# shockless/asr-transformer

Measured on AMD Instinct MI355X. Metric: encoder+decoder frames/sec/GPU at d_model=512 T=1000; 1->8 GPU scaling, higher is better.
Workload: dtype bf16; 1 GPU; c3: 12+12 layers d_model=512 h=8 ff=2048, B=64/GPU, T=1000 (T'=249), L=64, V=250; bf16 train step fwd+CE+bwd+AdamW, dropout 0.1; model=speech-transformer, global_batch=64, seq_len=1000, parallelism=dp1

## Files before the change

### asr-transformer_amd/asrx/blocks.py

```python
import bisect
import math

import torch

from . import kernels as K
from .kernels import MaskSpec


class FreshGrads:

    def __init__(self, store, params):
        self.grad = store.grad
        self.base = store.grad.data_ptr()
        ent = sorted((store.offset(p), p.numel()) for p in params)
        self.offs = [o for o, _ in ent]
        self.live = dict(ent)

    def take(self, gw):
        if not self.live:
            return False
        a = (gw.data_ptr() - self.base) // 4
        rows, cols = (gw.shape[0], gw.shape[1]) if gw.dim() == 2 else (1, gw.numel())
        ld = gw.stride(0) if gw.dim() == 2 else cols
        b = a + (rows - 1) * ld + cols
        i = bisect.bisect_left(self.offs, a)
        if i > 0 and self.offs[i - 1] + self.live.get(self.offs[i - 1], 0) > a:
            i -= 1
        hit = []
        while i < len(self.offs) and self.offs[i] < b:
            o = self.offs[i]
            if o in self.live:
                hit.append(o)
            i += 1
        if not hit:
            return False
        full = (ld == cols and (gw.dim() < 2 or gw.stride(1) == 1) and hit[0] == a
                and sum(self.live[o] for o in hit) == b - a)
        for o in hit:
            n = self.live.pop(o)
            if not full:
                self.grad[o:o + n].zero_()
        return full

    def drain(self, params=None, store=None):
        offs = list(self.live) if params is None else [store.offset(p) for p in params if store.offset(p) in self.live]
        for o in offs:
            self.grad[o:o + self.live.pop(o)].zero_()


class Ctx:

    def __init__(self, store, cd, train, p_drop, seeds, attn_impl="fused"):
        self.store = store
        self.cd = cd
        self.train = train
        self.p = p_drop if train else 0.0
        self.seeds = seeds
        self.attn_impl = attn_impl
        self.wq = None
        self.lnq = None
        self.fresh = None
        self.adam = None
        self.adam_cover = []
        self._gwritten = set()

    def W(self, p):
        return self.store.w16(p) if self.cd == torch.bfloat16 else self.store.w32(p)

    def G(self, p):
        return self.store.g(p)

    def seed(self):
        return self.seeds.next() if self.p > 0 else 0

    def wgrad(self, dy, x, gw, gb=None):
        if self.wq is not None and K.wgrad_groupable(dy, x, gw):
            self.wq.append((dy, x, gw, gb))
        else:
            first = self.fresh is not None and self.fresh.take(gw)
            self._note_writes(gw, gb)
            K.linear_wgrad(dy, x, gw, bias_grad=gb, beta=0.0 if first else 1.0)

    def _note_writes(self, *ts):
        cov = {o for o, _ in self.adam_cover}
        base = self.store.grad.data_ptr()
        for t in ts:
            if t is not None:
                assert (t.data_ptr() - base) // 4 not in cov, "asrx: write to a gradient after its fused AdamW"
                self._gwritten.add(t.data_ptr())

    def _adam_safe(self, q0):
        seen = set()
        for _, _, gw, gb in q0:
            for t in (gw, gb):
                if t is None:
                    continue
                if t.data_ptr() in seen or t.data_ptr() in self._gwritten:
                    return False
                seen.add(t.data_ptr())
        return True

    def _issue_wgrads(self, q):
        if self.fresh is None:
            for _, _, gw, gb in q:
                self._note_writes(gw, gb)
            K.linear_wgrad_grouped(q)
            return
        q0, q1 = [], []
        for it in q:
            (q0 if self.fresh.take(it[2]) else q1).append(it)
        adam = self.adam if not q1 and self._adam_safe(q0) else None
        for _, _, gw, gb in q0 + q1:
            self._note_writes(gw, gb)
        kname = K.linear_wgrad_grouped(q0, beta=0.0, adam=adam)
        if adam is not None and kname in K.GROUPED_FUSED_KERNELS:
            base = self.store.grad.data_ptr()
            for _, _, gw, gb in q0:
                for t in (gw, gb):
                    if t is not None:
                        self.adam_cover.append(((t.data_ptr() - base) // 4, t.numel()))
        K.linear_wgrad_grouped(q1)

    def defer_wgrad(self):
        if self.cd == torch.bfloat16 and self.wq is None:
            self.wq, self.lnq = [], []
            return True
        return False

    def flush_wgrad(self):
        q, self.wq = self.wq, None
        lq, self.lnq = self.lnq, None
        self._issue_wgrads(q or [])
        K.reduce_rows_grouped(lq or [])


class Seeds:
    def __init__(self, base):
        self.base = base
        self.i = 0

    def next(self):
        self.i += 1
        x = (self.base * 0x9E3779B97F4A7C15 + self.i * 0xBF58476D1CE4E5B9) & ((1 << 64) - 1)
        return x ^ (x >> 31)




def _empty(shape, dtype, like):
    return torch.empty(shape, dtype=dtype, device=like.device)


def as_dtype(t, dtype):
    if t.dtype == dtype:
        return t.contiguous()
    out = _empty(t.shape, dtype, t)
    K.cast(t.contiguous(), out)
    return out


def drop_bwd_c(C, g, seed):
    dy_c = _empty(g.shape, C.cd, g)
    if C.p > 0:
        K.ewise(K.EW_DROPOUT, g, dy_c, p=C.p, seed=seed)
    else:
        K.cast(g, dy_c)
    return dy_c



def ln_fwd(C, x, ln, out_dtype=None):
    y = _empty(x.shape, out_dtype or C.cd, x)
    mean, rstd = K.layernorm_fwd(x, ln.weight.data, ln.bias.data, y)
    return y, mean, rstd


def ln_grad_buf(C, ln):
    gw, gb = C.G(ln.weight), C.G(ln.bias)
    if gb.data_ptr() == gw.data_ptr() + 4 * gw.numel():
        return C.store.grad[C.store.offset(ln.weight):C.store.offset(ln.weight) + 2 * gw.numel()], None
    tmp = torch.zeros(2 * gw.numel(), device=gw.device, dtype=torch.float32)
    return tmp, (gw, gb)


def ln_bwd(C, x, dy, ln, mean, rstd, dres=None, drop_out=None, drop_seed=0, drop_p=0.0):
    buf, split = ln_grad_buf(C, ln)
# ... 261 lines not shown
    d = dy.shape[1]
    dmid_c = _empty(dy.shape, C.cd, dy)
    dmid = ffn_bwd(C, Sf, dy, dy_c, dx_c_out=dmid_c, dx_c_p=C.p, dx_c_seed=Sa["sd"])
    return self_attn_bwd(C, Sa, dmid, dmid_c, dx_c_out=dx_c_out, dx_c_p=dx_c_p, dx_c_seed=dx_c_seed)


def dec_layer_fwd(C, x, layer, B, L, H, spec, kv, kv_ld, Te, group=1, xspec=None):
    x1, Sa = self_attn_fwd(C, x, layer._norm1, layer._mask_attention, B, L, H, spec)
    x2, Sc = cross_attn_fwd(C, x1, layer._norm2, layer._cross_attention, kv, kv_ld, B, L, Te, H, group, xspec)
    x3, Sf = ffn_fwd(C, x2, layer._norm3, layer._feedforward)
    return x3, (Sa, Sc, Sf)


def dec_layer_bwd(C, S, dy, dy_c, dkv, dx_c_out, dx_c_p=0.0, dx_c_seed=0):
    Sa, Sc, Sf = S
    d2_c = _empty(dy.shape, C.cd, dy)
    d2 = ffn_bwd(C, Sf, dy, dy_c, dx_c_out=d2_c, dx_c_p=C.p, dx_c_seed=Sc["sd"])
    d1_c = _empty(dy.shape, C.cd, dy)
    d1 = cross_attn_bwd(C, Sc, d2, d2_c, dkv, dx_c_out=d1_c, dx_c_p=C.p, dx_c_seed=Sa["sd"])
    return self_attn_bwd(C, Sa, d1, d1_c, dx_c_out=dx_c_out, dx_c_p=dx_c_p, dx_c_seed=dx_c_seed)



def frontend_fwd(C, spectrum, conv1, conv2):
    B, _, F, T = spectrum.shape
    F1, T1 = (F - 3) // 2 + 1, (T - 3) // 2 + 1
    F2, T2 = (F1 - 3) // 2 + 1, (T1 - 3) // 2 + 1
    x = spectrum.contiguous().float()
    y1 = _empty((B, F1, T1, 64), C.cd, x)
    y1m = torch.empty((B, F1, T1, 8), dtype=torch.uint8, device=x.device) if C.cd == torch.bfloat16 else None
    K.conv1_fwd(x, conv1.weight.data.reshape(64, 9).contiguous(), conv1.bias.data, y1, mask=y1m)
    feats = _empty((B * T2, F2 * 64), C.cd, x)
    if C.cd == torch.bfloat16:
        K.conv2_fwd(y1, C.W(conv2.weight), conv2.bias.data, feats)
        cols = None
    else:
        cols = _empty((B * T2 * F2, 576), C.cd, x)
        K.im2col_conv2(y1, cols)
        K.gemm(cols, C.W(conv2.weight), feats, B * T2 * F2, 64, 576, lda=576, ldb=576, ldc=64,
               bias=conv2.bias.data, relu=True)
    return feats, dict(x=x, y1=y1, y1m=y1m, cols=cols, feats=feats, dims=(B, F, T, F1, T1, F2, T2))


def frontend_bwd(C, S, dfeats_c, conv1, conv2):
    B, F, T, F1, T1, F2, T2 = S["dims"]
    M2 = B * T2 * F2
    dy2 = dfeats_c.view(M2, 64)
    cols = S["cols"]
    G = C.G
    if cols is None:
        gw = G(conv2.weight)
        if C.fresh is not None:
            C.fresh.take(gw)
        K.conv2_wgrad(dy2, S["y1"], gw, G(conv2.bias))
    else:
        C.wgrad(dy2, cols, G(conv2.weight), G(conv2.bias))
    if cols is None and K.conv_bwd_implicit_fits(T):
        K.conv_bwd_implicit(dy2, C.W(conv2.weight), S["y1m"], S["x"], G(conv1.weight).view(64, 9), G(conv1.bias))
        return
    dcols = _empty((M2, 576), C.cd, dy2)
    K.linear_dgrad(dy2, C.W(conv2.weight), dcols)
    K.conv1_bwd_fused(dcols, S["y1"], S["x"], G(conv1.weight).view(64, 9), G(conv1.bias))
```

### asr-transformer_amd/asrx/kernels.py

```python
import ctypes
import os
import math
from typing import NamedTuple, Optional

import torch

from ._lib import (BF16, BITS, CONSTS, CTC_MAX_TARGET, CTC_MEAN, CTC_SUM, ED_CROSS, ED_GROUP, ED_PAIRS, F32,
                   MAX_ROWSUM_GROUPS, AttnDesc, GemmDesc, GemmGroupDev, RowsumGroup, call)

_U64 = (1 << 64) - 1


_raw_stream = torch._C._cuda_getCurrentRawStream
_cur_dev = torch._C._cuda_getDevice


def stream():
    return _raw_stream(_cur_dev())


def code(t):
    if t.dtype == torch.bfloat16:
        return BF16
    if t.dtype == torch.float32:
# ... 367 lines not shown
        seen, nb = set(), 0
        for dy, x, gw, gb in items:
            for t in (dy, x):
                if t.data_ptr() not in seen:
                    seen.add(t.data_ptr())
                    nb += t.shape[0] * t.shape[1] * t.element_size()
            for t in (gw, gb):
                if t is not None:
                    nb += t.numel() * 4 * (2 if beta == 1.0 else 1) + (26 * t.numel() if fused else 0)
        probe.alg_bytes[kname] = nb
    if probe is not None and probe.active and probe.log is not None:
        probe.log.append((kname, len(items), 0,
                          sum(it[0].shape[0] * it[0].shape[1] * it[1].shape[1] for it in items), 1, 1))
    if probe is not None and probe.active:
        timed_launch(kname, flops, launch)
    else:
        launch()
    return kname


def colsum(x, out, *, accumulate=True, rows=None, cols=None, ld=None):
    _cuda(x, out)
    rows = x.shape[0] if rows is None else rows
    cols = x.shape[1] if cols is None else cols
    ld = x.stride(0) if ld is None else ld
    nblocks = max(1, min(512, (rows + 63) // 64))
    part = torch.empty(nblocks * cols, device=x.device, dtype=torch.float32)
    call("asrx_reduce_rows", code(x), x.data_ptr(), rows, cols, ld, out.data_ptr(), int(accumulate),
         part.data_ptr(), nblocks, stream())



def layernorm_fwd(x, gamma, beta, y, eps=1e-5):
    _cuda(x, gamma, beta, y)
    rows, d = x.shape
    mean = torch.empty(rows, device=x.device, dtype=torch.float32)
    rstd = torch.empty(rows, device=x.device, dtype=torch.float32)
    call("asrx_layernorm_fwd", code(x), x.data_ptr(), code(y), y.data_ptr(), gamma.data_ptr(), beta.data_ptr(),
         mean.data_ptr(), rstd.data_ptr(), rows, d, eps, stream())
    return mean, rstd


def reduce_rows_grouped(items):
    for c0 in range(0, len(items), MAX_ROWSUM_GROUPS):
        chunk = items[c0:c0 + MAX_ROWSUM_GROUPS]
        arr = (RowsumGroup * len(chunk))()
        for gr, (src, out, acc) in zip(arr, chunk):
            _cuda(src, out)
            gr.in_, gr.rows, gr.cols = src.data_ptr(), src.shape[0], src.shape[1]
            gr.out, gr.accumulate = out.data_ptr(), int(acc)
        call("asrx_reduce_rows_grouped", arr, len(chunk), stream())


LN_BWD_BLOCKS = 512
LN_BWD512_WAVES = 8


def layernorm_bwd(x, dy, gamma, mean, rstd, dgb, *, dres=None, dx_drop=None, dropout_p=0.0, seed=0, defer=None):
    _cuda(x, dy, gamma, mean, rstd, dgb)
    rows, d = x.shape
    dx = torch.empty(rows, d, device=x.device, dtype=torch.float32)
    wpb = LN_BWD512_WAVES if d == 512 else 4
    nblocks = max(1, min(LN_BWD_BLOCKS * 4 // wpb, (rows + 2 * wpb - 1) // (2 * wpb)))
    part = torch.empty(nblocks * 2 * d, device=x.device, dtype=torch.float32)
    call("asrx_layernorm_bwd", code(x), x.data_ptr(), code(dy), dy.data_ptr(), gamma.data_ptr(), mean.data_ptr(),
         rstd.data_ptr(), _p(dres), dx.data_ptr(), _p(dx_drop), code(dx_drop) if dx_drop is not None else 0,
         dropout_p, seed & _U64, part.data_ptr(), nblocks, rows, d, stream())
    if defer is not None:
        defer.append((part.view(nblocks, 2 * d), dgb, True))
        return dx
    part2 = torch.empty(max(1, (nblocks + 63) // 64) * 2 * d, device=x.device, dtype=torch.float32)
    call("asrx_reduce_rows", F32, part.data_ptr(), nblocks, 2 * d, 2 * d, dgb.data_ptr(), 1, part2.data_ptr(),
         max(1, (nblocks + 63) // 64), stream())
    return dx



class MaskSpec:

    def __init__(self, mode=0, causal=False, kvalid=None, qvalid=None, valid_bstride=0, dense=None,
                 strides=(0, 0, 0)):
        self.mode, self.causal = mode, causal
        self.kvalid, self.qvalid, self.valid_bstride = kvalid, qvalid, valid_bstride
        self.dense, self.strides = dense, strides

    @staticmethod
    def decoder(mask):
        valid = (mask >= 1).to(torch.uint8).contiguous()
        return MaskSpec(1, True, valid, valid, valid.stride(0))

    @staticmethod
    def keys(valid):
        assert valid.dtype == torch.uint8 and valid.dim() == 2 and valid.stride(1) == 1
        return MaskSpec(1, False, valid, None, valid.stride(0))

    @staticmethod
    def from_attention_mask(m, B, Lq, Lk):
        if m is None:
            return MaskSpec()
        mb = m.gt(0).to(torch.uint8)
        while mb.dim() < 3:
            mb = mb.unsqueeze(0)
        mb = mb.expand(B, Lq, Lk)
        return MaskSpec(2, dense=mb, strides=tuple(mb.stride()))


# ... 447 lines not shown

def conv1_fwd(x, w, b, y1, mask=None):
    _cuda(x, w, b, y1, mask)
    B, _, F, T = x.shape
    call("asrx_conv1_fwd", x.data_ptr(), B, F, T, w.data_ptr(), b.data_ptr(), y1.data_ptr(), code(y1), _p(mask),
         stream())


def im2col_conv2(y1, cols):
    _cuda(y1, cols)
    B, F1, T1, _ = y1.shape
    assert y1.dtype == cols.dtype
    call("asrx_im2col_conv2", code(y1), y1.data_ptr(), B, F1, T1, cols.data_ptr(), stream())


def col2im_conv2(dcols, y1, dy1):
    _cuda(dcols, y1, dy1)
    B, F1, T1, _ = y1.shape
    call("asrx_col2im_conv2", code(dcols), dcols.data_ptr(), code(y1), y1.data_ptr(), B, F1, T1, dy1.data_ptr(),
         stream())


def conv2_fwd(y1, w2, bias, out):
    _cuda(y1, w2, bias, out)
    B, F1, T1, _ = y1.shape
    call("asrx_conv2_fwd", y1.data_ptr(), w2.data_ptr(), bias.data_ptr(), out.data_ptr(), B, F1, T1, stream())


def conv2_wgrad(dy2, y1, dw, db, splitk=256):
    _cuda(dy2, y1, dw, db)
    B, F1, T1, _ = y1.shape
    ws = torch.empty(splitk * 64 * 576, device=dy2.device, dtype=torch.float32)
    rws = torch.empty(splitk * 64, device=dy2.device, dtype=torch.float32) if db is not None else None
    call("asrx_conv2_wgrad", dy2.data_ptr(), y1.data_ptr(), B, F1, T1, dw.data_ptr(), _p(db), ws.data_ptr(),
         ws.numel(), _p(rws), splitk, stream())


CONV_BWD_MAXT1 = 1024
CONV_BWD_MAXLDS = 80 * 1024


def conv_bwd_implicit_fits(T):
    T1 = (T - 3) // 2 + 1
    return T1 <= CONV_BWD_MAXT1 and 6 * 64 * 64 * 2 + ((T1 * 8 + 15) & ~15) + 12 * T <= CONV_BWD_MAXLDS


def conv_bwd_implicit(dy2, w2, y1_mask, x, dw, db):
    _cuda(dy2, w2, y1_mask, x, dw, db)
    B, _, F, T = x.shape
    nblocks = max(2, min(512, B * y1_mask.shape[1]))
    part = torch.empty((nblocks + 128) * 640, device=x.device, dtype=torch.float32)
    call("asrx_conv_bwd_implicit", dy2.data_ptr(), w2.data_ptr(), y1_mask.data_ptr(), x.data_ptr(), B, F, T,
         part.data_ptr(), nblocks, dw.data_ptr(), db.data_ptr(), stream())


def conv1_bwd_w(x, dy1, dw, db):
    _cuda(x, dy1, dw, db)
    B, _, F, T = x.shape
    nblocks = 512
    part = torch.empty((nblocks + 128) * 640, device=x.device, dtype=torch.float32)
    call("asrx_conv1_bwd_w", x.data_ptr(), dy1.data_ptr(), B, F, T, part.data_ptr(), nblocks, dw.data_ptr(),
         db.data_ptr(), stream())


def conv1_bwd_fused(dcols, y1, x, dw, db):
    _cuda(dcols, y1, x, dw, db)
    B, _, F, T = x.shape
    nblocks = (B * y1.shape[1] * 8 + 3) // 4
    part = torch.empty((nblocks + 128) * 640, device=x.device, dtype=torch.float32)
    call("asrx_conv1_bwd_fused", code(dcols), dcols.data_ptr(), code(y1), y1.data_ptr(), x.data_ptr(), B, F, T,
         part.data_ptr(), nblocks, dw.data_ptr(), db.data_ptr(), stream())


def embed_fwd(tok, table, pe, out, L, dropout_p=0.0, seed=0):
    _cuda(tok, table, pe, out)
    call("asrx_embed_fwd", tok.data_ptr(), tok.numel(), L, table.data_ptr(), table.shape[1], pe.data_ptr(),
         dropout_p, seed & _U64, out.data_ptr(), stream())


def embed_bwd(tok, dout, dtable, L, pad_id, dropout_p=0.0, seed=0):
    _cuda(tok, dout, dtable)
    call("asrx_embed_bwd", tok.data_ptr(), tok.numel(), L, dout.data_ptr(), dtable.shape[1], dtable.shape[0],
         pad_id, dropout_p, seed & _U64, dtable.data_ptr(), stream())


CE_OLD_MAXLD = 1024


def xent_workspace_elems(rows):
    from ._lib import lib
    n = lib().asrx_xent_workspace_elems(rows)
    if n < 0:
        raise RuntimeError(f"asrx: no cross-entropy workspace for {rows} rows")
    return n


def cross_entropy(logits, V, target, ignore_index=-100, grad_scale=1.0, want_grad=True, want_argmax=False,
                  label_smoothing=0.0, grad_dtype=torch.bfloat16, want_stats=False, strided=False):
    _cuda(logits, target)
    rows, ld = logits.shape
    if strided:
        assert logits.dtype == torch.float32 and logits.stride(1) == 1 and V <= ld, \
            "asrx: cross_entropy(strided=True) needs fp32 rows of unit column stride"
        if rows > 1:
            ld = logits.stride(0)
            assert ld >= logits.shape[1], "asrx: cross_entropy(strided=True): overlapping rows"
# ... 239 lines not shown
    cross = mode == "cross"
    call("asrx_edit_distance", hyp.data_ptr(), hyp.stride(0), hyp.shape[1], _p(hyp_lengths),
         None if cross else ref.data_ptr(), 0 if cross else ref.stride(0), 0 if cross else ref.shape[1],
         None if cross else _p(ref_lengths), N, code, W, None if mode == "pairs" else _p(n_hyp), *_drop_ids(drop),
         -1 if stop is None else int(stop), dist.data_ptr(), _p(cnt), stream())
    return dist, cnt


def mbr_rank(dist, score, B, W, scale=1.0, n_hyp=None):
    _cuda(dist, score, n_hyp)
    assert dist.dtype == torch.int32 and dist.numel() == B * W * W and dist.is_contiguous()
    assert score.dtype == torch.float32 and score.numel() == B * W and score.is_contiguous()
    _check_n_hyp(n_hyp, B)
    risk = torch.empty(B, W, dtype=torch.float32, device=dist.device)
    order = torch.empty(B, W, dtype=torch.int32, device=dist.device)
    call("asrx_mbr_rank", dist.data_ptr(), score.data_ptr(), _p(n_hyp), B, W, float(scale), risk.data_ptr(),
         order.data_ptr(), stream())
    return risk, order


def adam(p, g, m, v, p_bf16, lr, beta1, beta2, eps, weight_decay, step, grad_scale=1.0, decoupled=False, hyp=None):
    _cuda(p, g, m, v, p_bf16, hyp)
    bc1 = 1.0 - beta1 ** step
    bc2 = 1.0 - beta2 ** step
    call("asrx_adam", p.data_ptr(), g.data_ptr(), m.data_ptr(), v.data_ptr(), _p(p_bf16), p.numel(), lr, beta1,
         beta2, eps, weight_decay, bc1, bc2, grad_scale, int(decoupled), _p(hyp), stream())


def adam_desc(p, m, v, p_bf16, g, lr, beta1, beta2, eps, weight_decay, step, grad_scale=1.0, decoupled=False,
              hyp=None):
    from ._lib import AdamDesc
    _cuda(p, m, v, p_bf16, g, hyp)
    d = AdamDesc()
    d.p, d.m, d.v, d.p_bf16, d.g_base, d.hyp = p.data_ptr(), m.data_ptr(), v.data_ptr(), _p(p_bf16), g.data_ptr(), _p(hyp)
    d.lr, d.beta1, d.beta2, d.eps, d.weight_decay = lr, beta1, beta2, eps, weight_decay
    d.bias_corr1, d.bias_corr2 = 1.0 - beta1 ** step, 1.0 - beta2 ** step
    d.grad_scale, d.decoupled = grad_scale, int(decoupled)
    return d


def adam_spans(p, g, m, v, p_bf16, spans, lr, beta1, beta2, eps, weight_decay, step, grad_scale=1.0, decoupled=False,
               hyp=None):
    _cuda(p, g, m, v, p_bf16, spans, hyp)
    call("asrx_adam_spans", p.data_ptr(), g.data_ptr(), m.data_ptr(), v.data_ptr(), _p(p_bf16), spans.data_ptr(),
         spans.shape[0], lr, beta1, beta2, eps, weight_decay, 1.0 - beta1 ** step, 1.0 - beta2 ** step, grad_scale,
         int(decoupled), _p(hyp), stream())


def adam_hyper(hyp, lr, beta1, beta2, step):
    import numpy as np
    upload(hyp, np.array([lr, 1.0 - beta1 ** step, 1.0 - beta2 ** step], dtype=np.float32))


TUNE_KEYS = {k: CONSTS["ASRX_TUNE_" + k.upper()] for k in ("softmax_u", "ln_rw", "ln_pf", "ln_bpc")}


def set_tuning(name, value):
    call("asrx_set_tuning", TUNE_KEYS[name], int(value))


def set_seed_offset(offset):
    call("asrx_set_seed_offset", int(offset) & _U64, stream())
```

### asr-transformer_amd/asrx/train.py

```python
import os

import torch

from . import kernels as K
from .augment import rank_seed
from .blocks import FreshGrads
from .dist import GradAllReduce
from .functions import get_store, key_spec, make_ctx, model_backward, model_forward, pad_lengths

FRESH_GRADS = os.environ.get("ASRX_FRESH_GRADS", "1") == "1"
GRAPH = os.environ.get("ASRX_GRAPH", "1") == "1"
GRAPH_WARMUP = 2
EARLY_ADAM = os.environ.get("ASRX_DP_EARLY_ADAM", "0") == "1"
FUSED_ADAM = os.environ.get("ASRX_FUSED_ADAM", "1") == "1"
ADAM_SPAN = 8192
ZERO_SPAN = 16384


def _aligned_spans(spans, n, q=4):
    out = []
    for a, b in sorted(spans):
        a, b = -(-a // q) * q, min(n, b) // q * q
        if b <= a:
            continue
# ... 199 lines not shown
                                                                   logits[i].shape[1]), device=logits[i].device)),
                                          dim=0)
            logits = torch.stack(logits, dim=0)
            preds.append(pred.to("cpu"))
            targets.append(text.to("cpu"))
            loss = loss_function(logits.transpose(1, 2), text)
            total += loss.item()
    return {"Val Loss": total / max(1, len(data_loader))}, preds[-1][-1]


class Trainer:

    def __init__(self, model, lr=1e-4, betas=(0.9, 0.98), eps=1e-9, weight_decay=0.0, decoupled=True,
                 ignore_index=-100, group=None, bucket_mb=64, allreduce_fn=None, graph=None, wire=None, preds=False,
                 ctc_weight=0.0, bos_token_id=1, spec_augment=None, label_smoothing=0.0):
        self.model = model
        self.label_smoothing = float(label_smoothing)
        if not 0.0 <= self.label_smoothing < 1.0:
            raise ValueError(f"label_smoothing {label_smoothing} outside [0, 1)")
        self.last_stats = None
        self.spec_augment = spec_augment
        self._aug_buf = None
        self.ctc_weight = float(ctc_weight)
        if not 0.0 <= self.ctc_weight < 1.0:
            raise ValueError(f"ctc_weight {ctc_weight} outside [0, 1)")
        head = getattr(model, "ctc_head", None)
        if self.ctc_weight > 0 and head is None:
            raise ValueError("ctc_weight > 0 needs a model with a CTC head: Transformer(..., ctc=True)")
        self._ctc_drop = [int(bos_token_id), int(model.decoder._eos_token_id)]
        if model.decoder.pad_token_id is not None:
            self._ctc_drop.append(int(model.decoder.pad_token_id))
        idle_head = list(head.parameters()) if head is not None and self.ctc_weight == 0 else []
        self.store = get_store(model)
        self.m = torch.zeros_like(self.store.flat)
        self.v = torch.zeros_like(self.store.flat)
        self.lr, self.betas, self.eps, self.wd, self.decoupled = lr, betas, eps, weight_decay, decoupled
        self.ignore_index = ignore_index
        self.step_count = 0
        self.reducer = GradAllReduce(self.store.grad, group=group, bucket_mb=bucket_mb, allreduce_fn=allreduce_fn,
                                     wire=wire)
        self.store.refresh_shadow(force=True)
        self._wonly = [p for p in wgrad_only_params(model) if not any(p is q for q in idle_head)] if FRESH_GRADS else []
        self.graph = GRAPH if graph is None else bool(graph)
        self._cap = None
        self._caps = {}
        self._eager_keys = set()
        self._hyp = torch.zeros(3, dtype=torch.float32, device=self.store.flat.device)
        self.ar_events = None
        self._adam_side = None
        self.want_preds = bool(preds)
        self.last_preds = None
        self._cover = None
        self._rspans = {}
        self._fuse_next = False
        self._frozen = sorted((self.store.offset(p), p.numel()) for p in unused_params(model) + idle_head
                              if self.store.owns(p))
        if self._wonly:
            n, spans, pos = self.store.grad.numel(), [], 0
            for o, k in sorted((self.store.offset(p), p.numel()) for p in self._wonly):
                if o > pos:
                    spans.append((pos, o))
                pos = max(pos, o + k)
            if pos < n:
                spans.append((pos, n))
            spans = [(c, min(c + ZERO_SPAN, b)) for a, b in spans for c in range(a, b, ZERO_SPAN)]
            self._zero_spans = torch.tensor(spans, dtype=torch.int64).reshape(-1, 2).to(self.store.grad.device)

    def _fused_adam_ok(self):
        return FUSED_ADAM and not self.reducer.active and self.model.precision == "bf16" and bool(self._wonly)

    def _residual_spans(self, cover):
        key = tuple(sorted(cover))
        tab = self._rspans.get(key)
        if tab is None:
            pieces = residual_pieces(self.store.flat.numel(), sorted(key + tuple(self._frozen)))
            tab = torch.tensor(pieces, dtype=torch.int64).reshape(-1, 2).to(self.store.flat.device)
            self._rspans[key] = tab
        return tab

    def forward_backward(self, spectrum, text, mask, ready=None, capture=False, input_text=None, input_lengths=None):
        model = self.model
        C = make_ctx(model, model.decoder.p)
        inp = text if input_text is None else input_text
        lam = self.ctc_weight
        from .model import subsampled
        enc_len, enc_spec = key_spec(pad_lengths(model, input_lengths), spectrum.shape[0],
                                     subsampled(spectrum.shape[-1]), self.store.flat.device, 2)
        if (text.is_cuda and text.dtype == torch.int64 and inp.dtype == torch.int64 and mask.dtype == torch.float32
                and text.stride(1) == 1 and inp.stride(1) == 1 and mask.stride(1) == 1):
            B, L = text.shape[0], text.shape[1] - 1
            dec_in, tgt, valid = K.step_tokens(text, inp, mask)
            spec = K.MaskSpec(1, True, valid, valid, valid.stride(0))
            logits, S = model_forward(C, model, spectrum, dec_in.view(B, L), None, spec=spec, ctc=lam > 0,
                                      enc_spec=enc_spec)
        else:
            logits, S = model_forward(C, model, spectrum, inp[:, :-1], mask[:, :-1], ctc=lam > 0, enc_spec=enc_spec)
            tgt = text[:, 1:].reshape(-1).contiguous()
        V = model.decoder._classifier.V
        if self.label_smoothing > 0 or logits.shape[1] > K.CE_OLD_MAXLD:
            loss, dl, am, self.last_stats = K.cross_entropy(
                logits, V, tgt, ignore_index=self.ignore_index, grad_scale=1.0 - lam, want_argmax=self.want_preds,
                label_smoothing=self.label_smoothing, grad_dtype=C.cd, want_stats=True)
        else:
            loss, dl, am = K.cross_entropy(logits, V, tgt, ignore_index=self.ignore_index, grad_scale=1.0 - lam,
                                           want_argmax=self.want_preds)
            self.last_stats = None
        self.last_preds = am
        dctc = None
        if lam > 0:
            dev = logits.device
            tt = text.to(device=dev, dtype=torch.int64)
            ctc_tgt, ctc_len = K.ctc_targets(tt if tt.stride(1) == 1 else tt.contiguous(),
                                             mask.to(device=dev, dtype=torch.float32).contiguous(), self._ctc_drop,
                                             model.ctc_blank)
            cl = S["ctc_logits"]
            Tp = cl.shape[0] // text.shape[0]
            loss, _, dctc = K.ctc_loss(cl, model.ctc_head.V, Tp, ctc_tgt, ctc_len, input_lengths=enc_len,
                                       max_target_len=min(ctc_tgt.shape[1], 255), blank=model.ctc_blank,
                                       reduction="mean", zero_infinity=True, grad_scale=lam, grad_dtype=C.cd,
                                       loss_add=loss, loss_add_scale=1.0 - lam, loss_scale=lam)
        if self._wonly and C.cd == torch.bfloat16 and all(p.grad is not None for p in self.store.params):
            K.zero_spans(self.store.grad, self._zero_spans)
            C.fresh = FreshGrads(self.store, self._wonly)
        else:
            self.store.grad.zero_()
        self._cover = None
        if self._fuse_next and C.fresh is not None:
            sh = self.store.shadow
            C.adam = K.adam_desc(self.store.flat, self.m, self.v, sh, self.store.grad, self.lr, self.betas[0],
                                 self.betas[1], self.eps, self.wd, max(1, self.step_count + 1),
                                 grad_scale=1.0 / self.reducer.world, decoupled=self.decoupled, hyp=self._hyp)
        if ready is None and not capture and self.reducer.active:
            ready = self.reducer.ready
        model_backward(C, model, S, dl.to(C.cd) if dl.dtype != C.cd else dl, ready=ready, dctc_c=dctc)
        if C.fresh is not None:
            C.fresh.drain()
            C.fresh = None
        if C.adam is not None and C.adam_cover:
            self._cover = list(C.adam_cover)
        return loss

    def _adam(self, hyp=None, span=None):
        if span is None and self._cover is not None:
            sh = self.store.shadow
            K.adam_spans(self.store.flat, self.store.grad, self.m, self.v, sh, self._residual_spans(self._cover),
                         self.lr, self.betas[0], self.betas[1], self.eps, self.wd, max(1, self.step_count),
                         grad_scale=1.0 / self.reducer.world, decoupled=self.decoupled, hyp=hyp)
            return
        a0, b0 = span if span is not None else (0, self.store.flat.numel())
        for a, b in _minus(a0, b0, self._frozen, align=4):
            sh = self.store.shadow[a:b] if self.store.shadow is not None else None
            K.adam(self.store.flat[a:b], self.store.grad[a:b], self.m[a:b], self.v[a:b], sh, self.lr, self.betas[0],
                   self.betas[1], self.eps, self.wd, max(1, self.step_count), grad_scale=1.0 / self.reducer.world,
                   decoupled=self.decoupled, hyp=hyp)

    def _reduce_and_adam(self, hyp=None):
        red = self.reducer
        n = self.store.flat.numel()
        early = []
        if EARLY_ADAM and red.active and red.allreduce_fn is None and red.wire == "fp32" and red._issued:
            early = _aligned_spans(red._issued, n)
        if not early:
            self._finish()
            self._adam(hyp)
            return
        dev = self.store.flat.device
        if self._adam_side is None:
            self._adam_side = torch.cuda.Stream(device=dev)
        side, main = self._adam_side, torch.cuda.current_stream(dev)
        works = list(red._works)
        with torch.cuda.stream(side):
            for w in works:
                w.wait()
            for sp in early:
                self._adam(hyp, sp)
        self._finish()
        for sp in _complement(early, n):
            self._adam(hyp, sp)
        main.wait_stream(side)

    def _aug_seed(self):
        return rank_seed(self.spec_augment.seed, reducer_rank(self.reducer))

    def _augment(self, spectrum, out, input_lengths, n):
        if out is None:
            out = self._aug_buf
            if out is None or out.shape != spectrum.shape or out.device != spectrum.device:
                out = self._aug_buf = torch.empty(tuple(spectrum.shape), dtype=torch.float32, device=spectrum.device)
        return self.spec_augment.augment(spectrum, out=out, lengths=input_lengths, step=n, seed=self._aug_seed())

    def step(self, spectrum, text, mask, input_text=None, input_lengths=None):
        if input_text is None:
            input_text = text
        lens = pad_lengths(self.model, input_lengths, self.store.flat.device)
        if self.graph and self.model.precision == "bf16":
# ... 16 lines not shown
        self.step_count += 1
        self._reduce_and_adam(self._hyp)
        self.store.mark_shadow_fresh()
        return loss

    def _finish(self):
        if self.ar_events is not None and self.reducer.active:
            e0, e1 = torch.cuda.Event(enable_timing=True), torch.cuda.Event(enable_timing=True)
            e0.record()
            self.reducer.finish()
            e1.record()
            self.ar_events.append((e0, e1))
        else:
            self.reducer.finish()

    @staticmethod
    def _key(*xs):
        return tuple((tuple(x.shape), x.dtype) for x in xs)

    def _capture(self, spectrum, text, mask, input_text, lens=None):
        dev = self.store.flat.device
        ins = tuple(x.to(dev).clone() for x in (spectrum, text, mask, input_text))
        if lens is not None:
            ins += (lens.clone(),)
        torch.cuda.synchronize(dev)
        pool = torch.cuda.graph_pool_handle()
        side = torch.cuda.Stream(device=dev)
        side.wait_stream(torch.cuda.current_stream(dev))
        with torch.cuda.stream(side):
            seg = _Segments(pool)
            K.CAPTURE = seg
            self._fuse_next = self._fused_adam_ok()
            try:
                loss = self.forward_backward(*ins[:3], ready=seg if self.reducer.active else None, capture=True,
                                             input_text=ins[3], input_lengths=ins[4] if lens is not None else None)
                if not self.reducer.active:
                    self._adam(self._hyp)
            finally:
                self._fuse_next = False
                K.CAPTURE = None
                seg.close()
        torch.cuda.current_stream(dev).wait_stream(side)
        torch.cuda.synchronize(dev)
        self._cap = (seg, ins, loss, self.last_preds, self.last_stats)

    def _replay(self, spectrum, text, mask, input_text, input_lengths=None, lens=None):
        seg, ins, loss, preds, stats = self._cap
        aug = self.spec_augment is not None
        if aug and ins[0].data_ptr() == spectrum.data_ptr():
            raise ValueError("Trainer.step: the spectrogram is the captured input buffer itself; the augmenter does not "
                             "work in place, pass a tensor of your own")
        self.last_preds, self.last_stats = preds, stats
        srcs = (spectrum, text, mask, input_text) + ((lens,) if lens is not None else ())
        for i, (dst, src) in enumerate(zip(ins, srcs)):
            if i == 0 and aug:
                self._augment(src, dst, input_lengths, self.step_count + 1)
            elif dst.data_ptr() != src.data_ptr():
                dst.copy_(src, non_blocking=True)
        self.step_count += 1
        K.set_seed_offset(self.step_count)
        K.adam_hyper(self._hyp, self.lr, self.betas[0], self.betas[1], self.step_count)
        seg.replay(self.reducer)
        if self.reducer.active:
            self._reduce_and_adam(self._hyp)
        self.store.mark_shadow_fresh()
        return loss
```

### asr-transformer_amd/csrc/common.h

```cpp
#pragma once
#include <hip/hip_runtime.h>
#include <stdint.h>

#include "../../include/asrx.h"

typedef uint16_t bf16_t;
typedef short s4_t __attribute__((ext_vector_type(4)));
typedef short s8_t __attribute__((ext_vector_type(8)));
typedef float f4_t __attribute__((ext_vector_type(4)));
typedef unsigned int v2u_t __attribute__((ext_vector_type(2)));
typedef unsigned int v4u_t __attribute__((ext_vector_type(4)));

#define ASRX_DEV __device__ __forceinline__

ASRX_DEV float bf2f(bf16_t v) { return __uint_as_float(((uint32_t)v) << 16); }

typedef float f2_t __attribute__((ext_vector_type(2)));
typedef __bf16 bf2_t __attribute__((ext_vector_type(2)));
ASRX_DEV bf16_t f2bf(float f) { return __builtin_bit_cast(bf16_t, (__bf16)f); }
ASRX_DEV uint32_t pack2bf(float a, float b) {
  return __builtin_bit_cast(uint32_t, __builtin_convertvector((f2_t){a, b}, bf2_t));
}

ASRX_DEV float adam_pin(float x) {
// ... 4 lines not shown
                         float bc1, float rbc2, float gs, int decoupled) {
  float gr = adam_pin(g * gs);
  float pv = p;
  if (decoupled) pv = adam_pin(pv * __builtin_fmaf(-lr, wd, 1.f));
  else gr = __builtin_fmaf(wd, pv, gr);
  m = __builtin_fmaf(b1, m, adam_pin((1.f - b1) * gr));
  v = __builtin_fmaf(b2, v, adam_pin(adam_pin((1.f - b2) * gr) * gr));
  const float denom = __builtin_fmaf(sqrtf(v), rbc2, eps);
  pv -= adam_pin(adam_pin(lr / bc1) * m) / denom;
  p = pv;
  return pv;
}

struct AdamFused {
  float* p; float* m; float* v; bf16_t* pb; const float* g0; const float* hyp;
  float lr, b1, b2, eps, wd, bc1, rbc2, gs; int decoupled;
};
ASRX_DEV void adam_hyp(const AdamFused& a, float& lr, float& bc1, float& rbc2) {
  lr = a.lr; bc1 = a.bc1; rbc2 = a.rbc2;
  if (a.hyp) { lr = a.hyp[0]; bc1 = a.hyp[1]; rbc2 = 1.f / sqrtf(a.hyp[2]); }
}
ASRX_DEV void adam_apply4(const AdamFused& a, const float* ga, f4_t g4, float lr, float bc1, float rbc2) {
  const int64_t off = ga - a.g0;
  f4_t p4 = *(const f4_t*)(a.p + off), m4 = *(const f4_t*)(a.m + off), v4 = *(const f4_t*)(a.v + off);
#pragma unroll
  for (int k = 0; k < 4; ++k) {
    float pe = p4[k], me = m4[k], ve = v4[k];
    adam_elem(g4[k], pe, me, ve, lr, a.b1, a.b2, a.eps, a.wd, bc1, rbc2, a.gs, a.decoupled);
    p4[k] = pe;
    m4[k] = me;
    v4[k] = ve;
  }
  *(f4_t*)(a.p + off) = p4;
  *(f4_t*)(a.m + off) = m4;
  *(f4_t*)(a.v + off) = v4;
  if (a.pb) {
    typedef uint32_t au2_t __attribute__((ext_vector_type(2)));
    au2_t u;
    u.x = pack2bf(p4[0], p4[1]);
    u.y = pack2bf(p4[2], p4[3]);
    *(au2_t*)(a.pb + off) = u;
  }
}
ASRX_DEV void adam_apply1(const AdamFused& a, const float* ga, float g, float lr, float bc1, float rbc2) {
  const int64_t off = ga - a.g0;
  float p = a.p[off], m = a.m[off], v = a.v[off];
  adam_elem(g, p, m, v, lr, a.b1, a.b2, a.eps, a.wd, bc1, rbc2, a.gs, a.decoupled);
  a.p[off] = p;
  a.m[off] = m;
  a.v[off] = v;
  if (a.pb) a.pb[off] = f2bf(p);
}

ASRX_DEV float exp2_raw(float x) { return __builtin_amdgcn_exp2f(x); }

ASRX_DEV uint32_t rng_hash(uint64_t seed, uint32_t pidx) {
  uint32_t x = pidx ^ (uint32_t)seed;
  x ^= x >> 16;
  x *= 0x7feb352dU;
  x ^= x >> 15;
  x = x * 0x846ca68bU + (uint32_t)(seed >> 32);
  x ^= x >> 16;
  return x;
}

static __device__ uint64_t g_seed_offset;
ASRX_DEV uint64_t seed_at(uint64_t seed, uint64_t o) {
  if (o == 0) return seed;
  uint64_t z = o * 0x9E3779B97F4A7C15ull;
  z = (z ^ (z >> 30)) * 0xBF58476D1CE4E5B9ull;
  z = (z ^ (z >> 27)) * 0x94D049BB133111EBull;
  return seed ^ z ^ (z >> 31);
}
ASRX_DEV uint64_t seed_eff(uint64_t seed) { return seed_at(seed, g_seed_offset); }
#define ASRX_SEED_OFFSET_SETTER(tu)                                                                 \
  uint64_t* asrx_seed_offset_addr_##tu() {                                                          \
    void* p = nullptr;                                                                              \
    return hipGetSymbolAddress(&p, HIP_SYMBOL(g_seed_offset)) == hipSuccess ? (uint64_t*)p : nullptr; \
  }
uint64_t* asrx_seed_offset_addr_gemm();
uint64_t* asrx_seed_offset_addr_attention();
uint64_t* asrx_seed_offset_addr_norm();
uint64_t* asrx_seed_offset_addr_softmax();
uint64_t* asrx_seed_offset_addr_frontend();
uint64_t* asrx_seed_offset_addr_gemm_ws();

ASRX_DEV uint32_t rng_half(uint32_t h, uint32_t which) { return which ? (h >> 16) : (h & 0xffffu); }

ASRX_DEV bool rng_keep(uint64_t seed, uint32_t idx, uint32_t threshold) {
  return rng_half(rng_hash(seed, idx >> 1), idx & 1u) >= threshold;
}

ASRX_DEV uint32_t attn_pair(int64_t bh, int lq, int lk, int q, int key) {
  return (uint32_t)((bh * ((lq + 1) >> 1) + (q >> 1)) * (int64_t)lk + key);
}

ASRX_DEV bool attn_keep(uint64_t seed, int64_t bh, int lq, int lk, int q, int key, uint32_t threshold) {
  return rng_half(rng_hash(seed, attn_pair(bh, lq, lk, q, key)), q & 1) >= threshold;
}

static inline uint32_t drop_threshold(float p) {
  if (p <= 0.f) return 0u;
  if (p >= 1.f) return 65536u;
  return (uint32_t)((double)p * 65536.0 + 0.5);
}

// ... 62 lines not shown
```

### asr-transformer_amd/csrc/frontend.hip

```cpp
#include <algorithm>
#include <cstring>

#include "common.h"
#include "gemm_common.h"

namespace {

constexpr int C1 = 64;

template <typename OT>
__global__ __launch_bounds__(256) void conv1_fwd_row_kernel(const float* __restrict__ x, int F, int T, int F1,
                                                            int T1, const float* __restrict__ w,
                                                            const float* __restrict__ bias, OT* __restrict__ y,
                                                            uint8_t* __restrict__ mask) {
  __shared__ __attribute__((aligned(16))) float sw[C1 * 9 + C1];
  for (int i = threadIdx.x; i < C1 * 10; i += 256) sw[i] = i < C1 * 9 ? w[i] : bias[i - C1 * 9];
  __syncthreads();
  const int cg = threadIdx.x & 7, ps = threadIdx.x >> 3;
  const int row = blockIdx.x, b = row / F1, f1 = row % F1;
  float wr[8][9], br[8];
#pragma unroll
  for (int q = 0; q < 18; ++q) {
    const f4_t v = *(const f4_t*)(sw + cg * 72 + 4 * q);
#pragma unroll
    for (int e = 0; e < 4; ++e) wr[(4 * q + e) / 9][(4 * q + e) % 9] = v[e];
  }
#pragma unroll
  for (int i = 0; i < 8; ++i) br[i] = sw[C1 * 9 + cg * 8 + i];
  extern __shared__ float sx[];
  const float* xr = x + ((int64_t)b * F + 2 * f1) * T;
  for (int i = threadIdx.x; i < 3 * T; i += 256) sx[i] = xr[(int64_t)(i / T) * T + i % T];
  __syncthreads();
  OT* yr = y + (int64_t)row * T1 * C1 + cg * 8;
  for (int t1 = ps; t1 < T1; t1 += 32) {
    float in[9];
#pragma unroll
    for (int kh = 0; kh < 3; ++kh)
#pragma unroll
      for (int kw = 0; kw < 3; ++kw) in[kh * 3 + kw] = sx[kh * T + 2 * t1 + kw];
    float o[8];
#pragma unroll
    for (int i = 0; i < 8; ++i) {
      float s = br[i];
#pragma unroll
      for (int k = 0; k < 9; ++k) s = fmaf(wr[i][k], in[k], s);
      o[i] = fmaxf(s, 0.f);
    }
    uint32_t m = 0;
    if constexpr (sizeof(OT) == 2) {
      uint4 u;
      u.x = pack2bf(o[0], o[1]); u.y = pack2bf(o[2], o[3]); u.z = pack2bf(o[4], o[5]); u.w = pack2bf(o[6], o[7]);
      *(uint4*)(yr + (int64_t)t1 * C1) = u;
      const uint32_t uu[4] = {u.x, u.y, u.z, u.w};
// ... 477 lines not shown
        const s8_t b1 = *(const s8_t*)(wr + 8 * ((4 + g) ^ (ci & 7)));
        acc[c] = __builtin_amdgcn_mfma_f32_16x16x32_bf16(cur0, b0, acc[c], 0, 0, 0);
        acc[c] = __builtin_amdgcn_mfma_f32_16x16x32_bf16(cur1, b1, acc[c], 0, 0, 0);
      }
      if (nch_ != ch) {
        const int j0 = 16 * (pt ? ch - c0 : ch), np = pt ? n1 : n0;
        uint2 mw[4];
        float xq[4];
#pragma unroll
        for (int r = 0; r < 4; ++r) {
          const int j = j0 + 4 * g + r;
          const bool ok = j < np;
          const int t1 = pt + 2 * (ok ? j : 0);
          mw[r] = ok ? *(const uint2*)(sM + t1 * 8) : make_uint2(0u, 0u);
          xq[r] = !ok ? 0.f : li < 9 ? sX[qkh * T + 2 * t1 + qkw] : (li == 9 ? 1.f : 0.f);
        }
        const s4_t bx = __builtin_bit_cast(s4_t, make_uint2(pack2bf(xq[0], xq[1]), pack2bf(xq[2], xq[3])));
#pragma unroll
        for (int c = 0; c < 4; ++c) {
          const int ci = 16 * c + li;
          float gv[4];
#pragma unroll
          for (int r = 0; r < 4; ++r) {
            const uint32_t wb = (ci >> 5) ? mw[r].y : mw[r].x;
            gv[r] = ((wb >> (ci & 31)) & 1u) ? acc[c][r] : 0.f;
          }
          const s4_t ga = __builtin_bit_cast(s4_t, make_uint2(pack2bf(gv[0], gv[1]), pack2bf(gv[2], gv[3])));
          aw[c] = __builtin_amdgcn_mfma_f32_16x16x16bf16_1k(ga, bx, aw[c], 0, 0, 0);
          acc[c] = f4_t{0.f, 0.f, 0.f, 0.f};
        }
      }
      if (!more) break;
      ch = nch_; ih = nih; iw = niw;
      cur0 = nx0; cur1 = nx1; cok = nok;
    }
  }
  __syncthreads();
  float (*red)[640] = (float (*)[640])smem;
  if (li < 10) {
#pragma unroll
    for (int c = 0; c < 4; ++c)
#pragma unroll
      for (int r = 0; r < 4; ++r) red[w][(16 * c + 4 * g + r) * 10 + li] = aw[c][r];
  }
  __syncthreads();
  for (int i = tid; i < 640; i += 512) {
    float s = 0.f;
#pragma unroll
    for (int q = 0; q < 8; ++q) s += red[q][i];
    part[(int64_t)blockIdx.x * 640 + i] = s;
  }
}

constexpr int CF_G1 = 128;
constexpr int CF_R1 = 48;

__global__ __launch_bounds__(256) void conv1_bwd_reduce1(const float* __restrict__ part, int nblocks,
                                                         float* __restrict__ part2) {
  const int per = (nblocks + CF_G1 - 1) / CF_G1;
  const int r0 = blockIdx.x * per, r1 = min(nblocks, r0 + per);
  for (int c = threadIdx.x; c < 640; c += 256) {
    float s = 0.f;
    for (int base = r0; base < r1; base += CF_R1) {
      float v[CF_R1];
#pragma unroll
      for (int j = 0; j < CF_R1; ++j) v[j] = base + j < r1 ? part[(int64_t)(base + j) * 640 + c] : 0.f;
#pragma unroll
      for (int j = 0; j < CF_R1; ++j) s += v[j];
    }
    part2[blockIdx.x * 640 + c] = s;
  }
}

__global__ __launch_bounds__(256) void conv1_bwd_reduce2(const float* __restrict__ part2, float* dw, float* db) {
  __shared__ float red[16][16];
  const int c = blockIdx.x * 16 + (threadIdx.x & 15), rg = threadIdx.x >> 4;
  float v[CF_G1 / 16];
#pragma unroll
  for (int j = 0; j < CF_G1 / 16; ++j) v[j] = part2[(rg + 16 * j) * 640 + c];
  float s = 0.f;
#pragma unroll
  for (int j = 0; j < CF_G1 / 16; ++j) s += v[j];
  red[rg][threadIdx.x & 15] = s;
  __syncthreads();
  if (rg == 0) {
    s = 0.f;
#pragma unroll
    for (int i = 0; i < 16; ++i) s += red[i][threadIdx.x];
    const int ch = c / 10, k = c % 10;
    if (k < 9) dw[ch * 9 + k] += s;
    else db[ch] += s;
  }
}

void conv1_bwd_finish(const float* part, int nblocks, float* dw, float* db, hipStream_t st) {
  float* part2 = const_cast<float*>(part) + (int64_t)nblocks * 640;
  hipLaunchKernelGGL(conv1_bwd_reduce1, dim3(CF_G1), dim3(256), 0, st, part, nblocks, part2);
  hipLaunchKernelGGL(conv1_bwd_reduce2, dim3(40), dim3(256), 0, st, part2, dw, db);
}

__global__ __launch_bounds__(256) void embed_fwd_kernel(const int64_t* __restrict__ tok, int64_t ntok, int L,
                                                        const float* __restrict__ table, int d,
                                                        const float* __restrict__ pe, uint32_t thr, float sc,
                                                        uint64_t seed, float* __restrict__ out) {
  seed = seed_eff(seed);
  const int dq = d / 4;
  const int64_t total = ntok * dq;
  for (int64_t t = (int64_t)blockIdx.x * 256 + threadIdx.x; t < total; t += (int64_t)gridDim.x * 256) {
    const int64_t row = t / dq;
    const int c = (int)(t % dq) * 4;
    const int64_t v = tok[row];
    const f4_t e = *(const f4_t*)(table + v * d + c);
    const f4_t p = *(const f4_t*)(pe + (int64_t)(row % L) * d + c);
    f4_t o;
#pragma unroll
    for (int i = 0; i < 4; ++i) {
      o[i] = e[i] + p[i];
      if (thr) o[i] = rng_keep(seed, (uint32_t)(row * d + c + i), thr) ? o[i] * sc : 0.f;
    }
    *(f4_t*)(out + row * d + c) = o;
  }
}

__global__ __launch_bounds__(256) void embed_bwd_kernel(const int64_t* __restrict__ tok, int64_t ntok, int d,
                                                        const float* __restrict__ dout, int pad_id, uint32_t thr,
                                                        float sc, uint64_t seed, float* __restrict__ dtable) {
  seed = seed_eff(seed);
  const int v = blockIdx.x;
  if (v == pad_id) return;
  const int lane = threadIdx.x & 63, w = threadIdx.x >> 6;
  constexpr int EB_WIN = 16, EB_CHUNK = 4 * 64 * EB_WIN;
  __shared__ int rows_[EB_CHUNK];
  __shared__ int wcnt[4 * EB_WIN];
  float acc[8];
#pragma unroll
  for (int j = 0; j < 8; ++j) acc[j] = 0.f;
  for (int64_t base = 0; base < ntok; base += EB_CHUNK) {
    unsigned long long mk[EB_WIN];
#pragma unroll
    for (int q = 0; q < EB_WIN; ++q) {
      const int64_t i = base + 64 * (EB_WIN * w + q) + lane;
      mk[q] = __ballot(i < ntok && tok[i] == v);
    }
    if (lane < EB_WIN) {
      int c = 0;
#pragma unroll
      for (int q = 0; q < EB_WIN; ++q) c = q == lane ? __popcll(mk[q]) : c;
      wcnt[EB_WIN * w + lane] = c;
    }
    __syncthreads();
    int off = 0, n = 0;
// ... 112 lines not shown
          }
        }
#pragma unroll
        for (int k = 0; k < 4; ++k) {
          if (e + k >= e1) break;
          if (thr) {
            const uint32_t pb = (uint32_t)(r[k] * d + c) >> 1;
#pragma unroll
            for (int hq = 0; hq < 2; ++hq)
#pragma unroll
              for (int pp = 0; pp < 2; ++pp) {
                const uint32_t h = rng_hash(seed, pb + 2 * hq + pp);
                g[k][hq][2 * pp] = rng_half(h, 0) >= thr ? g[k][hq][2 * pp] * sc : 0.f;
                g[k][hq][2 * pp + 1] = rng_half(h, 1) >= thr ? g[k][hq][2 * pp + 1] * sc : 0.f;
              }
          }
          acc[j][0] += g[k][0];
          acc[j][1] += g[k][1];
        }
      }
    }
    __syncthreads();
  }
  if (w > 0) {
#pragma unroll
    for (int j = 0; j < NJ; ++j) {
      const int c = 512 * j + 8 * lane;
      if (j < nj && c < d) {
        *(f4_t*)(&red[w - 1][c]) = acc[j][0];
        *(f4_t*)(&red[w - 1][c + 4]) = acc[j][1];
      }
    }
  }
  __syncthreads();
  if (w == 0) {
#pragma unroll
    for (int j = 0; j < NJ; ++j) {
      const int c = 512 * j + 8 * lane;
      if (j < nj && c < d) {
        f4_t s0 = acc[j][0], s1 = acc[j][1];
#pragma unroll
        for (int u = 0; u < 3; ++u) {
          s0 += *(const f4_t*)(&red[u][c]);
          s1 += *(const f4_t*)(&red[u][c + 4]);
        }
        float* o = dtable + (int64_t)v * d + c;
        *(f4_t*)o += s0;
        *(f4_t*)(o + 4) += s1;
      }
    }
  }
}

__global__ __launch_bounds__(256) void ce_count_kernel(const int64_t* tgt, int64_t rows, int64_t ignore, float* ws) {
  __shared__ float red[256];
  float c = 0.f;
  for (int64_t r = threadIdx.x; r < rows; r += 256) c += tgt[r] != ignore ? 1.f : 0.f;
  red[threadIdx.x] = c;
  __syncthreads();
  for (int s = 128; s > 0; s >>= 1) {
    if (threadIdx.x < s) red[threadIdx.x] += red[threadIdx.x + s];
    __syncthreads();
  }
  if (threadIdx.x == 0) ws[rows] = red[0];
}

template <int NJ>
__global__ __launch_bounds__(256) void ce_rows_kernel(const float* __restrict__ logits, int64_t rows, int V,
                                                      int64_t ld, const int64_t* __restrict__ tgt, int64_t ignore,
                                                      float gscale, bf16_t* __restrict__ dlog, int64_t* argmax,
                                                      float* ws) {
  const int l = threadIdx.x & 63;
  const int64_t r = (int64_t)blockIdx.x * 4 + (threadIdx.x >> 6);
  if (r >= rows) return;
  const float* x = logits + r * ld;
  float v[NJ];
  float mx = -INFINITY;
  int am = 0;
#pragma unroll
  for (int j = 0; j < NJ; ++j) {
    const int c = j * 64 + l;
    v[j] = c < V ? x[c] : -INFINITY;
    if (v[j] > mx) { mx = v[j]; am = c; }
  }
#pragma unroll
  for (int o = 32; o > 0; o >>= 1) {
    const float om = __shfl_xor(mx, o, 64);
    const int oa = __shfl_xor(am, o, 64);
    if (om > mx || (om == mx && oa < am)) { mx = om; am = oa; }
  }
  float s = 0.f;
#pragma unroll
  for (int j = 0; j < NJ; ++j) s += __expf(v[j] - mx);
  s = wave_sum(s);
  const float lse = mx + __logf(s);
  const int64_t t = tgt[r];
  const bool valid = t != ignore;
  const float cnt = ws[rows];
  const float k = valid && cnt > 0.f ? gscale / cnt : 0.f;
#pragma unroll
  for (int j = 0; j < NJ; ++j) {
    const int c = j * 64 + l;
    if (c < ld) {
      float gr = 0.f;
      if (c < V) gr = (__expf(v[j] - lse) - (c == t ? 1.f : 0.f)) * k;
      if (dlog) dlog[r * ld + c] = f2bf(gr);
    }
  }
  if (l == 0) {
    ws[r] = valid ? lse - x[t] : 0.f;
    if (argmax) argmax[r] = am;
  }
}

__global__ __launch_bounds__(256) void ce_final_kernel(const float* ws, int64_t rows, float* loss) {
  __shared__ float red[256];
  float s = 0.f;
  for (int64_t r = threadIdx.x; r < rows; r += 256) s += ws[r];
  red[threadIdx.x] = s;
  __syncthreads();
  for (int k = 128; k > 0; k >>= 1) {
    if (threadIdx.x < k) red[threadIdx.x] += red[threadIdx.x + k];
    __syncthreads();
  }
  if (threadIdx.x == 0) loss[0] = ws[rows] > 0.f ? red[0] / ws[rows] : 0.f;
}

__global__ __launch_bounds__(256) void cast_kernel(int sd, const void* __restrict__ src, int dd, void* __restrict__ dst,
                                                   int64_t n) {
  for (int64_t i = (int64_t)blockIdx.x * 256 + threadIdx.x; i < n; i += (int64_t)gridDim.x * 256) {
    const float v = sd == ASRX_F32 ? ((const float*)src)[i] : bf2f(((const bf16_t*)src)[i]);
    if (dd == ASRX_F32) ((float*)dst)[i] = v;
    else ((bf16_t*)dst)[i] = f2bf(v);
  }
}

ASRX_DEV void adam_f4(f4_t& pp, const f4_t gg, f4_t& mm, f4_t& vv, float lr, float b1, float b2, float eps,
                      float wd, float bc1, float rbc2, float gs, int decoupled) {
#pragma unroll
  for (int k = 0; k < 4; ++k) {
    float pe = pp[k], me = mm[k], ve = vv[k];
    adam_elem(gg[k], pe, me, ve, lr, b1, b2, eps, wd, bc1, rbc2, gs, decoupled);
    pp[k] = pe;
    mm[k] = me;
    vv[k] = ve;
  }
}

ASRX_DEV void adam_store(float* p, float* m, float* v, bf16_t* pb, int64_t i, const f4_t& pp, const f4_t& mm,
                         const f4_t& vv) {
  __builtin_nontemporal_store(pp, (f4_t*)p + i);
  __builtin_nontemporal_store(mm, (f4_t*)m + i);
  __builtin_nontemporal_store(vv, (f4_t*)v + i);
  if (pb) {
    typedef uint32_t u2_t __attribute__((ext_vector_type(2)));
    u2_t u;
    u.x = pack2bf(pp[0], pp[1]);
    u.y = pack2bf(pp[2], pp[3]);
    __builtin_nontemporal_store(u, (u2_t*)pb + i);
  }
}

__global__ __launch_bounds__(256) void adam_kernel(float* __restrict__ p, const float* __restrict__ g,
                                                   float* __restrict__ m, float* __restrict__ v,
                                                   bf16_t* __restrict__ pb, int64_t n, float lr, float b1, float b2,
                                                   float eps, float wd, float bc1, float rbc2, float gs,
                                                   int decoupled, const float* __restrict__ hyp) {
  if (hyp) {
    lr = hyp[0];
    bc1 = hyp[1];
    rbc2 = 1.f / sqrtf(hyp[2]);
  }
  const int64_t n4 = n / 4, stride = (int64_t)gridDim.x * 256;
  int64_t i = (int64_t)blockIdx.x * 256 + threadIdx.x;
  for (; i + stride < n4; i += 2 * stride) {
    const int64_t j = i + stride;
    f4_t p0 = __builtin_nontemporal_load((const f4_t*)p + i), p1 = __builtin_nontemporal_load((const f4_t*)p + j);
    const f4_t g0 = __builtin_nontemporal_load((const f4_t*)g + i), g1 = __builtin_nontemporal_load((const f4_t*)g + j);
    f4_t m0 = __builtin_nontemporal_load((const f4_t*)m + i), m1 = __builtin_nontemporal_load((const f4_t*)m + j);
    f4_t v0 = __builtin_nontemporal_load((const f4_t*)v + i), v1 = __builtin_nontemporal_load((const f4_t*)v + j);
    adam_f4(p0, g0, m0, v0, lr, b1, b2, eps, wd, bc1, rbc2, gs, decoupled);
    adam_f4(p1, g1, m1, v1, lr, b1, b2, eps, wd, bc1, rbc2, gs, decoupled);
    adam_store(p, m, v, pb, i, p0, m0, v0);
    adam_store(p, m, v, pb, j, p1, m1, v1);
  }
  if (i < n4) {
    f4_t pp = ((f4_t*)p)[i], mm = ((f4_t*)m)[i], vv = ((f4_t*)v)[i];
    adam_f4(pp, ((const f4_t*)g)[i], mm, vv, lr, b1, b2, eps, wd, bc1, rbc2, gs, decoupled);
    adam_store(p, m, v, pb, i, pp, mm, vv);
  }
  if (blockIdx.x == 0) {
    for (int64_t i = n4 * 4 + threadIdx.x; i < n; i += 256) {
      float pv = p[i], mv = m[i], vv = v[i];
      adam_elem(g[i], pv, mv, vv, lr, b1, b2, eps, wd, bc1, rbc2, gs, decoupled);
      p[i] = pv;
      m[i] = mv;
      v[i] = vv;
      if (pb) pb[i] = f2bf(pv);
    }
  }
}

__global__ __launch_bounds__(256) void adam_spans_kernel(float* __restrict__ p, const float* __restrict__ g,
                                                         float* __restrict__ m, float* __restrict__ v,
                                                         bf16_t* __restrict__ pb, const int64_t* __restrict__ spans,
                                                         float lr, float b1, float b2, float eps, float wd, float bc1,
                                                         float rbc2, float gs, int decoupled,
                                                         const float* __restrict__ hyp) {
  if (hyp) {
    lr = hyp[0];
    bc1 = hyp[1];
    rbc2 = 1.f / sqrtf(hyp[2]);
  }
  const int64_t a0 = spans[2 * blockIdx.x], e0 = spans[2 * blockIdx.x + 1];
  const int64_t a = (a0 + 3) / 4, e = e0 / 4;
  for (int64_t i = a + threadIdx.x; i < e; i += 256) {
    f4_t pp = ((const f4_t*)p)[i], mm = ((const f4_t*)m)[i], vv = ((const f4_t*)v)[i];
    adam_f4(pp, ((const f4_t*)g)[i], mm, vv, lr, b1, b2, eps, wd, bc1, rbc2, gs, decoupled);
    adam_store(p, m, v, pb, i, pp, mm, vv);
  }
  const int64_t hb = min(4 * a, e0), tb = max(4 * e, hb);
  const int64_t j = threadIdx.x < 3 ? a0 + threadIdx.x : tb + (threadIdx.x - 3);
  if ((threadIdx.x < 3 && j < hb) || (threadIdx.x >= 3 && threadIdx.x < 6 && j >= tb && j < e0)) {
    float pe = p[j], me = m[j], ve = v[j];
    adam_elem(g[j], pe, me, ve, lr, b1, b2, eps, wd, bc1, rbc2, gs, decoupled);
    p[j] = pe;
    m[j] = me;
    v[j] = ve;
    if (pb) pb[j] = f2bf(pe);
  }
}

ASRX_DEV float ld_any(int dt, const void* p, int64_t i) {
  return dt == ASRX_F32 ? ((const float*)p)[i] : bf2f(((const bf16_t*)p)[i]);
}
__global__ __launch_bounds__(256) void ewise_kernel(int op, int da, const void* a, int db, const void* b, int dout,
                                                    void* out, int64_t n, uint32_t thr, float dscale, uint64_t seed) {
  if (op == ASRX_EW_DROPOUT) seed = seed_eff(seed);
  for (int64_t i = (int64_t)blockIdx.x * 256 + threadIdx.x; i < n; i += (int64_t)gridDim.x * 256) {
    const float x = ld_any(da, a, i);
    float r;
    if (op == ASRX_EW_RELU_GRAD) r = ld_any(db, b, i) > 0.f ? x : 0.f;
    else if (op == ASRX_EW_DROPOUT) r = (thr == 0u || rng_keep(seed, (uint32_t)i, thr)) ? x * dscale : 0.f;
    else r = x + ld_any(db, b, i);
    if (dout == ASRX_F32) ((float*)out)[i] = r;
    else ((bf16_t*)out)[i] = f2bf(r);
  }
}

__global__ __launch_bounds__(256) void dropout_mask_kernel(uint8_t* keep, int64_t n, uint32_t thr, uint64_t seed) {
  seed = seed_eff(seed);
  for (int64_t i = (int64_t)blockIdx.x * 256 + threadIdx.x; i < n; i += (int64_t)gridDim.x * 256)
    keep[i] = rng_keep(seed, (uint32_t)i, thr) ? 1 : 0;
}

inline unsigned grid_for(int64_t work, int cap = 8192) {
  int64_t b = (work + 255) / 256;
  if (b < 1) b = 1;
  if (b > cap) b = cap;
  return (unsigned)b;
}

}

ASRX_SEED_OFFSET_SETTER(frontend)

extern "C" int asrx_version(void) { return 14; }

extern "C" int asrx_struct_sizes(int64_t* out, int32_t n) {
  if (!out || n < 0) return ASRX_ERR_ARG;
  const int64_t s[5] = {(int64_t)sizeof(asrx_gemm_desc), (int64_t)sizeof(asrx_attn_desc),
                        (int64_t)sizeof(asrx_gemm_group_dev), (int64_t)sizeof(asrx_rowsum_group),
                        (int64_t)sizeof(asrx_adam_desc)};
  const int k = n < 5 ? n : 5;
  for (int i = 0; i < k; ++i) out[i] = s[i];
  return k;
}

extern "C" int asrx_conv1_fwd(const float* x, int32_t B, int32_t F, int32_t T, const float* w, const float* b,
                              void* y1, int32_t y_dtype, uint8_t* y1_mask, void* stream) {
  if (!x || !w || !b || !y1 || B <= 0 || F < 3 || T < 3) return ASRX_ERR_ARG;
  const int F1 = (F - 3) / 2 + 1, T1 = (T - 3) / 2 + 1;
  if (T > 5120) return ASRX_ERR_UNSUPPORTED;
  const dim3 grid((unsigned)(B * F1));
  const size_t shm = sizeof(float) * 3 * T;
  if (y_dtype == ASRX_F32)
    hipLaunchKernelGGL(conv1_fwd_row_kernel<float>, grid, dim3(256), shm, (hipStream_t)stream, x, F, T, F1, T1, w,
                       b, (float*)y1, y1_mask);
  else
    hipLaunchKernelGGL(conv1_fwd_row_kernel<bf16_t>, grid, dim3(256), shm, (hipStream_t)stream, x, F, T, F1, T1, w,
                       b, (bf16_t*)y1, y1_mask);
  ASRX_CHECK_LAUNCH();
  return ASRX_OK;
}

extern "C" int asrx_conv2_fwd(const void* y1, const void* w2, const float* bias, void* out, int32_t B, int32_t F1,
                              int32_t T1, void* stream) {
  if (!y1 || !w2 || !bias || !out || B <= 0 || F1 < 3 || T1 < 3) return ASRX_ERR_ARG;
  if (((uintptr_t)y1 | (uintptr_t)w2 | (uintptr_t)out) % 16) return ASRX_ERR_ARG;
  const int F2 = (F1 - 3) / 2 + 1, T2 = (T1 - 3) / 2 + 1;
  const int64_t y1_bytes = (int64_t)B * F1 * T1 * 64 * 2;
  const int64_t M = (int64_t)B * T2 * F2;
  if (y1_bytes >= 0x80000000LL || M >= 0x7fffffffLL) return ASRX_ERR_UNSUPPORTED;
  const int ntiles = (int)((M + C2_ROWS - 1) / C2_ROWS);
  hipLaunchKernelGGL(conv2_fwd_kernel, dim3(std::min(ntiles, 256)), dim3(512), 0, (hipStream_t)stream,
                     (const bf16_t*)y1, (const bf16_t*)w2, bias, (bf16_t*)out, (int)M, F1, T1, F2, T2, ntiles,
                     y1_bytes);
  ASRX_CHECK_LAUNCH();
  return ASRX_OK;
}

extern "C" int asrx_im2col_conv2(int32_t dtype, const void* y1, int32_t B, int32_t F1, int32_t T1, void* cols,
                                 void* stream) {
  if (!y1 || !cols || B <= 0 || F1 < 3 || T1 < 3) return ASRX_ERR_ARG;
  const int F2 = (F1 - 3) / 2 + 1, T2 = (T1 - 3) / 2 + 1;
  if (dtype == ASRX_F32)
    hipLaunchKernelGGL(im2col_kernel<float>, dim3(grid_for((int64_t)B * T2 * F2 * 144)), dim3(256), 0,
                       (hipStream_t)stream, (const float*)y1, B, F1, T1, F2, T2, (float*)cols);
  else
    hipLaunchKernelGGL(im2col_kernel<bf16_t>, dim3(grid_for((int64_t)B * T2 * F2 * 72)), dim3(256), 0,
// ... 11 lines not shown
  ASRX_CHECK_LAUNCH();
  return ASRX_OK;
}

extern "C" int asrx_conv1_bwd_w(const float* x, const float* dy1, int32_t B, int32_t F, int32_t T, float* part,
                                int32_t nblocks, float* dw, float* db, void* stream) {
  if (!x || !dy1 || !part || !dw || !db || nblocks <= 0) return ASRX_ERR_ARG;
  const int F1 = (F - 3) / 2 + 1, T1 = (T - 3) / 2 + 1;
  const int64_t npos = (int64_t)B * F1 * T1;
  const int64_t per = (npos + nblocks - 1) / nblocks;
  hipStream_t st = (hipStream_t)stream;
  hipLaunchKernelGGL(conv1_bwd_w_kernel, dim3(nblocks), dim3(256), 0, st, x, dy1, B, F, T, F1, T1, part, per);
  ASRX_CHECK_LAUNCH();
  conv1_bwd_finish(part, nblocks, dw, db, st);
  ASRX_CHECK_LAUNCH();
  return ASRX_OK;
}

extern "C" int asrx_embed_fwd(const int64_t* tok, int64_t ntok, int32_t L, const float* table, int32_t d,
                              const float* pe, float dropout_p, uint64_t seed, float* out, void* stream) {
  if (!tok || !table || !pe || !out || d % 4 || L <= 0) return ASRX_ERR_ARG;
  if (ntok == 0) return ASRX_OK;
  const uint32_t thr = drop_threshold(dropout_p);
  const float sc = (dropout_p > 0.f && dropout_p < 1.f) ? 1.f / (1.f - dropout_p) : 1.f;
  hipLaunchKernelGGL(embed_fwd_kernel, dim3(grid_for(ntok * (d / 4))), dim3(256), 0, (hipStream_t)stream, tok, ntok, L,
                     table, d, pe, thr, sc, seed, out);
  ASRX_CHECK_LAUNCH();
  return ASRX_OK;
}

extern "C" int asrx_embed_bwd(const int64_t* tok, int64_t ntok, int32_t L, const float* dout, int32_t d,
                              int32_t vocab, int32_t pad_id, float dropout_p, uint64_t seed, float* dtable,
                              void* stream) {
  (void)L;
  if (!tok || !dout || !dtable || vocab <= 0 || d > 2048) return ASRX_ERR_ARG;
  const uint32_t thr = drop_threshold(dropout_p);
  const float sc = (dropout_p > 0.f && dropout_p < 1.f) ? 1.f / (1.f - dropout_p) : 1.f;
  if (d % 8 == 0 && (uintptr_t)dout % 16 == 0 && (uintptr_t)dtable % 16 == 0)
    hipLaunchKernelGGL(embed_bwd_v8_kernel, dim3(vocab), dim3(256), 0, (hipStream_t)stream, tok, ntok, d, dout, pad_id,
                       thr, sc, seed, dtable);
  else
    hipLaunchKernelGGL(embed_bwd_kernel, dim3(vocab), dim3(256), 0, (hipStream_t)stream, tok, ntok, d, dout, pad_id,
                       thr, sc, seed, dtable);
  ASRX_CHECK_LAUNCH();
  return ASRX_OK;
}

extern "C" int asrx_cross_entropy(const float* logits, int64_t rows, int32_t V, int64_t ld, const int64_t* target,
                                  int64_t ignore_index, float grad_scale, float* loss, void* dlogits,
                                  int64_t* argmax, float* ws, void* stream) {
  if (!logits || !target || !loss || !ws || V <= 0 || ld < V || rows < 0) return ASRX_ERR_ARG;
  if (ld > 1024) return ASRX_ERR_UNSUPPORTED;
  hipStream_t st = (hipStream_t)stream;
  hipLaunchKernelGGL(ce_count_kernel, dim3(1), dim3(256), 0, st, target, rows, ignore_index, ws);
  ASRX_CHECK_LAUNCH();
  if (rows > 0) {
    const dim3 grid((unsigned)((rows + 3) / 4));
    const int nj = (int)((ld + 63) / 64);
    if (nj <= 4) hipLaunchKernelGGL((ce_rows_kernel<4>), grid, dim3(256), 0, st, logits, rows, V, ld, target, ignore_index, grad_scale, (bf16_t*)dlogits, argmax, ws);
    else if (nj <= 8) hipLaunchKernelGGL((ce_rows_kernel<8>), grid, dim3(256), 0, st, logits, rows, V, ld, target, ignore_index, grad_scale, (bf16_t*)dlogits, argmax, ws);
    else hipLaunchKernelGGL((ce_rows_kernel<16>), grid, dim3(256), 0, st, logits, rows, V, ld, target, ignore_index, grad_scale, (bf16_t*)dlogits, argmax, ws);
    ASRX_CHECK_LAUNCH();
  }
  hipLaunchKernelGGL(ce_final_kernel, dim3(1), dim3(256), 0, st, ws, rows, loss);
  ASRX_CHECK_LAUNCH();
  return ASRX_OK;
}

__global__ __launch_bounds__(256) void greedy_argmax_kernel(const float* __restrict__ logits, int64_t rows, int V,
                                                            int64_t ld, int64_t* __restrict__ tok,
                                                            int64_t tok_stride, int64_t* __restrict__ cur) {
  const int l = threadIdx.x & 63;
  const int64_t r = (int64_t)blockIdx.x * 4 + (threadIdx.x >> 6);
  if (r >= rows) return;
  const float* x = logits + r * ld;
  float mx = -INFINITY;
  int am = V;
  for (int c = l; c < V; c += 64) {
    const float v = x[c];
    if (v > mx || (am == V && !(v < mx))) { mx = v; am = c; }
  }
#pragma unroll
  for (int o = 32; o > 0; o >>= 1) {
    const float om = __shfl_xor(mx, o, 64);
    const int oa = __shfl_xor(am, o, 64);
    if (om > mx || (om == mx && oa < am)) { mx = om; am = oa; }
  }
  if (l == 0) {
    const int64_t t = am < V ? am : 0;
    tok[r * tok_stride] = t;
    if (cur) cur[r] = t;
  }
}

extern "C" int asrx_greedy_argmax(const float* logits, int64_t rows, int32_t V, int64_t ld, int64_t* tok,
                                  int64_t tok_stride, int64_t* cur, void* stream) {
  if (!logits || !tok || V <= 0 || ld < V || rows < 0) return ASRX_ERR_ARG;
  if (rows == 0) return ASRX_OK;
  hipLaunchKernelGGL(greedy_argmax_kernel, dim3((unsigned)((rows + 3) / 4)), dim3(256), 0, (hipStream_t)stream,
                     logits, rows, (int)V, ld, tok, tok_stride, cur);
  ASRX_CHECK_LAUNCH();
  return ASRX_OK;
}

__global__ __launch_bounds__(256) void sum_chunks_bf16_kernel(const bf16_t* __restrict__ in, int W, int64_t c,
                                                               bf16_t* __restrict__ out) {
  for (int64_t i = (int64_t)blockIdx.x * 256 + threadIdx.x; i < c; i += (int64_t)gridDim.x * 256) {
    float acc = 0.f;
    for (int w = 0; w < W; ++w) acc += bf2f(in[(int64_t)w * c + i]);
    out[i] = f2bf(acc);
  }
}

int g_tune_softmax_u = 0;
int g_tune_ln_rw = 0;
int g_tune_ln_pf = 0;
int g_tune_ln_bpc = 0;
// ... 30 lines not shown
  if (!src || !dst || n < 0) return ASRX_ERR_ARG;
  if (n == 0) return ASRX_OK;
  hipLaunchKernelGGL(cast_kernel, dim3(grid_for(n)), dim3(256), 0, (hipStream_t)stream, src_dtype, src, dst_dtype, dst,
                     n);
  ASRX_CHECK_LAUNCH();
  return ASRX_OK;
}

extern "C" int asrx_ewise(int32_t op, int32_t dtype_a, const void* a, int32_t dtype_b, const void* b,
                          int32_t dtype_out, void* out, int64_t n, float p, uint64_t seed, void* stream) {
  if (op < ASRX_EW_RELU_GRAD || op > ASRX_EW_ADD || n < 0) return ASRX_ERR_ARG;
  const auto okdt = [](int32_t t) { return t == ASRX_F32 || t == ASRX_BF16; };
  if (!okdt(dtype_a) || !okdt(dtype_out) || (op != ASRX_EW_DROPOUT && !okdt(dtype_b))) return ASRX_ERR_ARG;
  if (n == 0) return ASRX_OK;
  if (!a || !out || (op != ASRX_EW_DROPOUT && !b) || (op == ASRX_EW_DROPOUT && !(p >= 0.f && p < 1.f)))
    return ASRX_ERR_ARG;
  const uint32_t thr = op == ASRX_EW_DROPOUT ? drop_threshold(p) : 0u;
  const float dscale = op == ASRX_EW_DROPOUT && p > 0.f ? 1.f / (1.f - p) : 1.f;
  hipLaunchKernelGGL(ewise_kernel, dim3(grid_for(n)), dim3(256), 0, (hipStream_t)stream, (int)op, (int)dtype_a, a,
                     (int)dtype_b, b, (int)dtype_out, out, n, thr, dscale, seed);
  ASRX_CHECK_LAUNCH();
  return ASRX_OK;
}

extern "C" int asrx_adam(float* p, const float* g, float* m, float* v, void* p_bf16, int64_t n, float lr, float beta1,
                         float beta2, float eps, float weight_decay, float bias_corr1, float bias_corr2,
                         float grad_scale, int32_t decoupled, const float* hyp, void* stream) {
  if (!p || !g || !m || !v || n < 0 || (!hyp && (bias_corr1 <= 0.f || bias_corr2 <= 0.f))) return ASRX_ERR_ARG;
  if (((uintptr_t)p | (uintptr_t)g | (uintptr_t)m | (uintptr_t)v) % 16) return ASRX_ERR_ARG;
  if (p_bf16 && (uintptr_t)p_bf16 % 8) return ASRX_ERR_ARG;
  if (n == 0) return ASRX_OK;
  hipLaunchKernelGGL(adam_kernel, dim3(grid_for(n / 4 + 1, 16384)), dim3(256), 0, (hipStream_t)stream, p, g, m, v,
                     (bf16_t*)p_bf16, n, lr, beta1, beta2, eps, weight_decay, bias_corr1, 1.f / sqrtf(bias_corr2),
                     grad_scale, decoupled, hyp);
  ASRX_CHECK_LAUNCH();
  return ASRX_OK;
}

extern "C" int asrx_adam_spans(float* p, const float* g, float* m, float* v, void* p_bf16, const int64_t* spans,
                               int32_t nspans, float lr, float beta1, float beta2, float eps, float weight_decay,
                               float bias_corr1, float bias_corr2, float grad_scale, int32_t decoupled,
                               const float* hyp, void* stream) {
  if (!p || !g || !m || !v || nspans < 0 || (nspans > 0 && !spans)) return ASRX_ERR_ARG;
  if (((uintptr_t)p | (uintptr_t)g | (uintptr_t)m | (uintptr_t)v) % 16) return ASRX_ERR_ARG;
  if (p_bf16 && (uintptr_t)p_bf16 % 8) return ASRX_ERR_ARG;
  if (nspans == 0) return ASRX_OK;
  hipLaunchKernelGGL(adam_spans_kernel, dim3(nspans), dim3(256), 0, (hipStream_t)stream, p, g, m, v, (bf16_t*)p_bf16,
                     spans, lr, beta1, beta2, eps, weight_decay, bias_corr1, 1.f / sqrtf(bias_corr2), grad_scale,
                     decoupled, hyp);
  ASRX_CHECK_LAUNCH();
  return ASRX_OK;
}

extern "C" int asrx_dropout_mask(uint8_t* keep, int64_t n, float p, uint64_t seed, void* stream) {
  if (!keep || n < 0) return ASRX_ERR_ARG;
  if (n == 0) return ASRX_OK;
  hipLaunchKernelGGL(dropout_mask_kernel, dim3(grid_for(n)), dim3(256), 0, (hipStream_t)stream, keep, n,
                     drop_threshold(p), seed);
  ASRX_CHECK_LAUNCH();
  return ASRX_OK;
}

extern "C" int asrx_conv_bwd_implicit(const void* dy2, const void* w2, const uint8_t* y1m, const float* x, int32_t B,
                                      int32_t F, int32_t T, float* part, int32_t nblocks, float* dw, float* db,
                                      void* stream) {
  if (!dy2 || !w2 || !y1m || !x || !part || !dw || !db || B <= 0 || F < 7 || T < 7 || nblocks < 2)
    return ASRX_ERR_ARG;
  if (((uintptr_t)dy2 | (uintptr_t)y1m) % 16) return ASRX_ERR_ARG;
  const int F1 = (F - 3) / 2 + 1, T1 = (T - 3) / 2 + 1;
  const int F2 = (F1 - 3) / 2 + 1, T2 = (T1 - 3) / 2 + 1;
  if (T1 > CB_MAXT1) return ASRX_ERR_UNSUPPORTED;
  const int g_even = std::max(1, std::min(nblocks - 1, (2 * nblocks + 2) / 3));
  const size_t shm = (size_t)6 * 64 * 64 * 2 + ((T1 * 8 + 15) & ~15) + sizeof(float) * 3 * T;
  if (shm > 80 * 1024 || shm < 8 * 640 * 4) return ASRX_ERR_UNSUPPORTED;
  hipStream_t st = (hipStream_t)stream;
  hipLaunchKernelGGL(conv_bwd_implicit_kernel, dim3(nblocks), dim3(512), shm, st, (const bf16_t*)dy2,
                     (const bf16_t*)w2, y1m, x, B, F, T, F1, T1, F2, T2, g_even, part);
  ASRX_CHECK_LAUNCH();
  conv1_bwd_finish(part, nblocks, dw, db, st);
  return ASRX_OK;
}

extern "C" int asrx_conv1_bwd_fused(int32_t dcols_dtype, const void* dcols, int32_t y1_dtype, const void* y1,
                                    const float* x, int32_t B, int32_t F, int32_t T, float* part, int32_t nblocks,
                                    float* dw, float* db, void* stream) {
  if (!dcols || !y1 || !x || !part || !dw || !db || B <= 0) return ASRX_ERR_ARG;
  const int F1 = (F - 3) / 2 + 1, T1 = (T - 3) / 2 + 1;
  const int F2 = (F1 - 3) / 2 + 1, T2 = (T1 - 3) / 2 + 1;
  if (F1 <= 0 || T1 <= 0 || F2 <= 0 || T2 <= 0) return ASRX_ERR_ARG;
  if (nblocks != (B * F1 * CB_SEG + 3) / 4) return ASRX_ERR_ARG;
  hipStream_t st = (hipStream_t)stream;
#define ASRX_FUSED(DT, YT) hipLaunchKernelGGL((conv1_bwd_fused_kernel<DT, YT>), dim3(nblocks), dim3(256), 0, st, \
      (const DT*)dcols, (const YT*)y1, x, B, F, T, F1, T1, F2, T2, part)
  if (dcols_dtype == ASRX_BF16 && y1_dtype == ASRX_BF16)
    hipLaunchKernelGGL(conv1_bwd_fused_v8_kernel, dim3(nblocks), dim3(256), 0, st, (const bf16_t*)dcols,
                       (const bf16_t*)y1, x, B, F, T, F1, T1, F2, T2, part);
  else if (dcols_dtype == ASRX_F32 && y1_dtype == ASRX_F32) ASRX_FUSED(float, float);
  else if (dcols_dtype == ASRX_BF16 && y1_dtype == ASRX_F32) ASRX_FUSED(bf16_t, float);
  else ASRX_FUSED(float, bf16_t);
#undef ASRX_FUSED
  ASRX_CHECK_LAUNCH();
  conv1_bwd_finish(part, nblocks, dw, db, st);
  ASRX_CHECK_LAUNCH();
  return ASRX_OK;
}

namespace {
constexpr int UPLOAD_CHUNK = 3968;
struct UploadChunk {
  uint32_t w[UPLOAD_CHUNK / 4];
};
__global__ __launch_bounds__(256) void upload_kernel(UploadChunk c, uint32_t* __restrict__ dst, int nwords) {
  for (int i = threadIdx.x; i < nwords; i += 256) dst[i] = c.w[i];
}
}

extern "C" int asrx_upload(void* dst, const void* src, int64_t nbytes, void* stream) {
  if (!dst || (!src && nbytes > 0) || nbytes < 0 || nbytes % 4 || (uintptr_t)dst % 4) return ASRX_ERR_ARG;
  const unsigned char* s = (const unsigned char*)src;
  for (int64_t off = 0; off < nbytes; off += UPLOAD_CHUNK) {
    const int n = (int)std::min<int64_t>(UPLOAD_CHUNK, nbytes - off);
    UploadChunk c;
    std::memcpy(c.w, s + off, n);
    hipLaunchKernelGGL(upload_kernel, dim3(1), dim3(256), 0, (hipStream_t)stream, c, (uint32_t*)((char*)dst + off),
                       n / 4);
    ASRX_CHECK_LAUNCH();
  }
  return ASRX_OK;
}

namespace {
struct SeedAddrs { uint64_t* p[6]; };
__global__ void seed_offset_set_all_kernel(uint64_t v, SeedAddrs a) {
  if (threadIdx.x < 6) *a.p[threadIdx.x] = v;
}
}

extern "C" int asrx_set_seed_offset(uint64_t offset, void* stream) {
  static const SeedAddrs addrs = [] {
    return SeedAddrs{{asrx_seed_offset_addr_gemm(), asrx_seed_offset_addr_attention(), asrx_seed_offset_addr_norm(),
                      asrx_seed_offset_addr_softmax(), asrx_seed_offset_addr_frontend(),
                      asrx_seed_offset_addr_gemm_ws()}};
  }();
  for (uint64_t* q : addrs.p)
    if (!q) return ASRX_ERR_LAUNCH;
  hipLaunchKernelGGL(seed_offset_set_all_kernel, dim3(1), dim3(64), 0, (hipStream_t)stream, offset, addrs);
  ASRX_CHECK_LAUNCH();
  return ASRX_OK;
}

__global__ __launch_bounds__(256) void zero_spans_kernel(float* __restrict__ base, const int64_t* __restrict__ spans) {
  const int64_t a = spans[2 * blockIdx.x], b = spans[2 * blockIdx.x + 1];
  const int64_t a4 = (a + 3) & ~(int64_t)3, b4 = b & ~(int64_t)3;
  if (a4 >= b4) {
    for (int64_t i = a + threadIdx.x; i < b; i += 256) base[i] = 0.f;
    return;
  }
  for (int64_t i = a + threadIdx.x; i < a4; i += 256) base[i] = 0.f;
  for (int64_t i = b4 + threadIdx.x; i < b; i += 256) base[i] = 0.f;
  for (int64_t i = a4 + 4 * (int64_t)threadIdx.x; i < b4; i += 1024) *(f4_t*)(base + i) = f4_t{0.f, 0.f, 0.f, 0.f};
}

namespace {
constexpr int CLIP_CHUNK = 4096;

ASRX_DEV float block_sum256(float v, float* red) {
  v = wave_sum(v);
  if ((threadIdx.x & 63) == 0) red[threadIdx.x >> 6] = v;
  __syncthreads();
  const float t = (red[0] + red[1]) + (red[2] + red[3]);
  __syncthreads();
  return t;
}

template <bool SCALE>
__global__ __launch_bounds__(256) void clip_spans_kernel(const int64_t* __restrict__ spans, int count, float max_norm,
                                                         float* __restrict__ part, int nparts, float* __restrict__ out) {
  __shared__ float red[4];
  float coef = 1.f;
  if constexpr (SCALE) {
    float t = 0.f;
    for (int i = threadIdx.x; i < nparts; i += 256) t += part[i];
    const float total = sqrtf(block_sum256(t, red));
    coef = fminf(max_norm / (total + 1e-6f), 1.f);
    if (blockIdx.x == 0 && threadIdx.x == 0) { out[0] = total; out[1] = coef; }
  }
  float acc = 0.f;
  int64_t pre = 0;
  for (int s = 0; s < count; ++s) {
    float* g = (float*)(uintptr_t)spans[2 * s];
    const int64_t n = spans[2 * s + 1];
    const bool vec = ((uintptr_t)g & 15) == 0;
    const int64_t nck = (n + CLIP_CHUNK - 1) / CLIP_CHUNK;
    const int64_t first = ((int64_t)blockIdx.x - pre % nparts + nparts) % nparts;
    pre += nck;
    for (int64_t c0 = first * CLIP_CHUNK; c0 < n; c0 += (int64_t)nparts * CLIP_CHUNK) {
      const int64_t c1 = min(n, c0 + CLIP_CHUNK);
      if (vec && c1 - c0 == CLIP_CHUNK) {
        for (int64_t i = c0 + 4 * threadIdx.x; i < c1; i += 1024) {
// ... 139 lines not shown
```

### asr-transformer_amd/csrc/gemm.hip

```cpp
#include <algorithm>
#include <cstdio>
#include <cstdlib>
#include <cstring>
#include <optional>
#include <type_traits>

#include "gemm_common.h"

namespace {
using namespace asrxg;


template <int R, bool KSTRIDED>
struct TileBF16 {
  static constexpr int ELEMS = KSTRIDED ? BK * R : R * KC_STRIDE;
  static constexpr int CHUNKS = R * BK / 8;
  static constexpr int PER_THREAD = CHUNKS / 256;

  template <bool VEC>
  ASRX_DEV static void load(s8_t* regs, const bf16_t* base, int64_t ld, int r0, int rmax, int k0, int kmax) {
    const int t = threadIdx.x;
#pragma unroll
    for (int i = 0; i < PER_THREAD; ++i) {
      const int c = t + 256 * i;
// ... 1171 lines not shown
        const s4_t lo = __builtin_amdgcn_ds_read_tr16_b64_v4i16((__attribute__((address_space(3))) s4_t*)p);
        const s4_t hi = __builtin_amdgcn_ds_read_tr16_b64_v4i16((__attribute__((address_space(3))) s4_t*)(p + 16 * N));
        const s8_t fb = s8_t{lo[0], lo[1], lo[2], lo[3], hi[0], hi[1], hi[2], hi[3]};
#pragma unroll
        for (int i = 0; i < 2; ++i) acc[i][j] = __builtin_amdgcn_mfma_f32_16x16x32_bf16(fa[i], fb, acc[i][j], 0, 0, 0);
      }
    }
    if (nq == 0 && g.rowsum) {
#pragma unroll
      for (int i = 0; i < 2; ++i) rs[i] = __builtin_amdgcn_mfma_f32_16x16x32_bf16(fa[i], ones, rs[i], 0, 0, 0);
    }
  }
  float* ws = g.ws + (int64_t)z * g.M * N;
#pragma unroll
  for (int i = 0; i < 2; ++i) {
    const int m0 = 16 * (2 * mh + i) + 4 * g4;
#pragma unroll
    for (int j = 0; j < 9; ++j) {
      const int nt = 9 * nq + j;
      if (nt < ntt) {
#pragma unroll
        for (int r = 0; r < 4; ++r) ws[(int64_t)(m0 + r) * N + 16 * nt + li] = acc[i][j][r];
      }
    }
    if (nq == 0 && g.rowsum && li == 0) {
#pragma unroll
      for (int r = 0; r < 4; ++r) g.rowsum_ws[(int64_t)z * g.M + m0 + r] = rs[i][r];
    }
  }
}

__global__ __launch_bounds__(256) void tallk_reduce_kernel(GemmArgs g) {
  __shared__ f4_t red[8][32];
  const int nq = g.N / 4;
  const int q = blockIdx.x * 32 + (threadIdx.x & 31), sg = threadIdx.x >> 5;
  const int quads = g.M * nq;
  f4_t s = f4_t{0.f, 0.f, 0.f, 0.f};
  if (q < quads) {
    const int m = q / nq, n0 = (q % nq) * 4;
    for (int sp = sg; sp < g.splitk; sp += 8) s += *(const f4_t*)(g.ws + ((int64_t)sp * g.M + m) * g.N + n0);
  }
  red[sg][threadIdx.x & 31] = s;
  __syncthreads();
  if (sg == 0 && q < quads) {
#pragma unroll
    for (int i = 1; i < 8; ++i) s += red[i][threadIdx.x];
    float v[4] = {s[0], s[1], s[2], s[3]};
    epilogue4(g, 0, q / nq, (q % nq) * 4, v);
  }
}

__global__ __launch_bounds__(256) void rowsum_finish_kernel(const float* ws, int splitk, int M, float* out) {
  __shared__ float red[4][64];
  const int m = blockIdx.x * 64 + (threadIdx.x & 63), sg = threadIdx.x >> 6;
  float s = 0.f;
  if (m < M) {
    for (int sp0 = sg; sp0 < splitk; sp0 += 64) {
      float v[16];
#pragma unroll
      for (int j = 0; j < 16; ++j) {
        const int sp = sp0 + 4 * j;
        v[j] = sp < splitk ? ws[(int64_t)sp * M + m] : 0.f;
      }
#pragma unroll
      for (int j = 0; j < 16; ++j) s += v[j];
    }
  }
  red[sg][threadIdx.x & 63] = s;
  __syncthreads();
  if (sg == 0 && m < M) out[m] += red[0][threadIdx.x] + red[1][threadIdx.x] + red[2][threadIdx.x] + red[3][threadIdx.x];
}

template <class F>
void with_layout(bool at, bool bt, F&& f) {
  using T = std::true_type;
  using N = std::false_type;
  at ? (bt ? f(T{}, T{}) : f(T{}, N{})) : (bt ? f(N{}, T{}) : f(N{}, N{}));
}
template <class F>
void with_layout(bool at, bool bt, bool vec, F&& f) {
  with_layout(at, bt, [&](auto AT, auto BT) { vec ? f(AT, BT, std::true_type{}) : f(AT, BT, std::false_type{}); });
}

enum class Family { Reg128, Reg64, P3, P4, Ring64, Ring128, TallK, Ws256, Ws64 };
enum class Reduce { None, SplitK, TallK };

struct GemmPlan {
  Family family;
  bool at, bt;
  bool vec, cvec;
  int epi;
  bool drop_keeps_all;
  int ntiles;
  bool bias_chunks;
  Reduce reduce;
};

bool epi_instantiated(bool at, bool bt, int epi) {
#define ASRX_HAS(E) if (epi == (E)) return true;
  if (!at && !bt) { ASRX_EPI_NT(ASRX_HAS) }
  else if (!at && bt) { ASRX_EPI_NN(ASRX_HAS) }
  else if (at && bt) { ASRX_EPI_TT(ASRX_HAS) }
#undef ASRX_HAS
  return false;
}

std::optional<Family> forced_family(int code, Family reg) {
  switch (code) {
    case ASRX_GEMM_P3: return Family::P3;
    case ASRX_GEMM_REG: return reg;
    case ASRX_GEMM_RING: return Family::Ring64;
    case ASRX_GEMM_RING128: return Family::Ring128;
    case ASRX_GEMM_P4: return Family::P4;
    case ASRX_GEMM_WS: return Family::Ws256;
    case ASRX_GEMM_WS64: return Family::Ws64;
    default: return std::nullopt;
  }
}

bool c_quads_aligned(const asrx_gemm_desc* d) {
  const int esz = d->c_dtype == ASRX_F32 ? 16 : 8;
  return (d->ldc % 4 == 0) && ((uintptr_t)d->c % esz == 0) && (d->sc_outer % 4 == 0) && (d->sc_inner % 4 == 0);
}
// ... 156 lines not shown
      });
      break;
    case Family::TallK:
      hipLaunchKernelGGL(gemm_bf16_tallk_kernel, dim3(g.splitk), dim3(512), 0, st, g, TallkConv{0, 0, 0, 0, 0, 0});
      break;
    case Family::Ws256:
    case Family::Ws64:
      launch_ws(g, pl.bt, pl.epi, pl.ntiles, pl.family == Family::Ws64 ? 64 : 256, st);
      break;
  }
  return ASRX_OK;
}

int fill_args(const asrx_gemm_desc* d, GemmArgs& g, int& batch) {
  g = GemmArgs{};
  if (!d || d->m < 0 || d->n < 0 || d->k < 0 || !d->a || !d->b || !d->c) return ASRX_ERR_ARG;
  if (d->in_dtype != ASRX_BF16 && d->in_dtype != ASRX_F32) return ASRX_ERR_ARG;
  if (d->c_dtype != ASRX_BF16 && d->c_dtype != ASRX_F32) return ASRX_ERR_ARG;
  if (d->m == 0 || d->n == 0) return ASRX_OK;
  batch = d->batch > 0 ? d->batch : 1;
  const int splitk = d->splitk > 1 ? d->splitk : 1;
  if (splitk > 1 && (batch != 1 || !d->workspace || d->workspace_elems < (int64_t)splitk * d->m * d->n))
    return ASRX_ERR_ARG;
  if (batch > 65535 || splitk > 65535) return ASRX_ERR_ARG;
  if (((d->gate && d->gate_dtype == ASRX_BITS) || d->mask_out) && d->in_dtype != ASRX_BF16) return ASRX_ERR_UNSUPPORTED;
  if (d->rowsum_a && (!d->a_trans || d->in_dtype != ASRX_BF16 || batch != 1)) return ASRX_ERR_UNSUPPORTED;
  if (d->rowsum_a && splitk > 1 && !d->rowsum_ws) return ASRX_ERR_ARG;
  g.M = d->m; g.N = d->n; g.K = d->k;
  g.a = d->a; g.lda = d->lda; g.b = d->b; g.ldb = d->ldb;
  g.c = d->c; g.ldc = d->ldc; g.c_dtype = d->c_dtype;
  g.batch_inner = d->batch_inner > 0 ? d->batch_inner : 1;
  g.sa_o = d->sa_outer; g.sa_i = d->sa_inner; g.sb_o = d->sb_outer; g.sb_i = d->sb_inner;
  g.sc_o = d->sc_outer; g.sc_i = d->sc_inner;
  g.alpha = d->alpha; g.beta = d->beta;
  g.bias = d->bias;
  g.rowadd = d->rowadd; g.ld_rowadd = d->ld_rowadd; g.rowadd_mod = d->rowadd_mod > 0 ? d->rowadd_mod : 1;
  g.relu = d->relu;
  g.drop_thr = drop_threshold(d->dropout_p);
  g.drop_scale = d->dropout_p > 0.f && d->dropout_p < 1.f ? 1.f / (1.f - d->dropout_p) : 0.f;
  g.seed = d->seed;
  g.gate = d->gate; g.ld_gate = d->ld_gate; g.gate_dtype = d->gate_dtype;
  g.mask_out = d->mask_out; g.ld_mask = d->ld_mask;
  g.resid = d->resid; g.ld_resid = d->ld_resid; g.resid_dtype = d->resid_dtype;
  g.ws = d->workspace;
  g.rowsum = d->rowsum_a;
  g.rowsum_ws = d->rowsum_ws;
  g.dbg = gemm_dbg();
  const int bk = d->in_dtype == ASRX_BF16 ? BK : FBK;
  g.splitk = splitk;
  g.k_per_split = ((((int)d->k + bk - 1) / bk + splitk - 1) / splitk) * bk;
  return ASRX_OK;
}

int launch_reduce(const GemmArgs& g, Reduce reduce, hipStream_t st) {
  const int64_t quads = (int64_t)g.M * ((g.N + 3) / 4);
  if (reduce == Reduce::TallK)
    hipLaunchKernelGGL(tallk_reduce_kernel, dim3((unsigned)((quads + 31) / 32)), dim3(256), 0, st, g);
  else
    hipLaunchKernelGGL(splitk_reduce_kernel, dim3((int)std::min<int64_t>((quads + 255) / 256, 4096)), dim3(256), 0, st, g);
  ASRX_CHECK_LAUNCH();
  if (g.rowsum) {
    hipLaunchKernelGGL(rowsum_finish_kernel, dim3((g.M + 63) / 64), dim3(256), 0, st, g.rowsum_ws, g.splitk, g.M, g.rowsum);
    ASRX_CHECK_LAUNCH();
  }
  return ASRX_OK;
}

}

ASRX_SEED_OFFSET_SETTER(gemm)

extern "C" int asrx_gemm_set_debug(int32_t flags) {
  g_gemm_dbg = flags < 0 ? 0 : flags;
  return ASRX_OK;
}

extern "C" int asrx_gemm_kernel_name(const asrx_gemm_desc* d, char* buf, int len) {
  if (!d || !buf || len < 8) return ASRX_ERR_ARG;
  if (d->in_dtype == ASRX_F32)
    snprintf(buf, len, "gemm_f32_kernel<%s, %s>", d->a_trans ? "true" : "false", d->b_trans ? "true" : "false");
  else
    plan_name(plan_bf16(d, d->batch > 0 ? d->batch : 1, d->splitk > 1 ? d->splitk : 1), buf, len);
  return ASRX_OK;
}

static_assert(sizeof(GroupEnt) == sizeof(asrx_gemm_group_dev), "device group table layout");

extern "C" int asrx_gemm(const asrx_gemm_desc* d, void* stream) {
  GemmArgs g;
  int batch = 1;
  int rc = fill_args(d, g, batch);
  if (rc != ASRX_OK) return rc;
  if (g.M == 0) return ASRX_OK;
  hipStream_t st = (hipStream_t)stream;
  Reduce reduce = g.splitk > 1 ? Reduce::SplitK : Reduce::None;
  if (d->in_dtype == ASRX_BF16) {
    const GemmPlan pl = plan_bf16(d, batch, g.splitk);
    g.cvec = pl.cvec;
    reduce = pl.reduce;
    rc = launch_plan(d, g, pl, batch, st);
    if (rc != ASRX_OK) return rc;
  } else {
    g.cvec = c_quads_aligned(d);
    const int vec = (d->lda % 4 == 0) && (d->ldb % 4 == 0) && ((uintptr_t)d->a % 16 == 0) &&
                    ((uintptr_t)d->b % 16 == 0) && (d->sa_outer % 4 == 0) && (d->sa_inner % 4 == 0) &&
                    (d->sb_outer % 4 == 0) && (d->sb_inner % 4 == 0);
    const dim3 grid(((d->m + FBM - 1) / FBM) * ((d->n + FBN - 1) / FBN), g.splitk, batch);
    with_layout(d->a_trans, d->b_trans, [&](auto AT, auto BT) {
      hipLaunchKernelGGL((gemm_f32_kernel<AT, BT>), grid, dim3(256), 0, st, g, vec);
    });
  }
  ASRX_CHECK_LAUNCH();
  return reduce == Reduce::None ? ASRX_OK : launch_reduce(g, reduce, st);
}
// ... 5 lines not shown
      blocks < 0 || tiles > 65535)
    return ASRX_ERR_ARG;
  if (!adam->p || !adam->m || !adam->v || !adam->g_base || (((uintptr_t)adam->p | (uintptr_t)adam->m |
      (uintptr_t)adam->v | (uintptr_t)adam->g_base) % 16) || (adam->p_bf16 && (uintptr_t)adam->p_bf16 % 8))
    return ASRX_ERR_ARG;
  if (tiles == 0 || blocks == 0) return ASRX_OK;
  if (common->in_dtype != ASRX_BF16 || !common->a_trans || !common->b_trans || common->tile != ASRX_GROUP_TILE_WS ||
      common->c_dtype != ASRX_F32 || common->alpha != 1.f || common->beta != 0.f || !common->workspace ||
      common->workspace_elems < 16 || !common->rowsum_ws)
    return ASRX_ERR_UNSUPPORTED;
  AdamFused ad;
  ad.p = adam->p; ad.m = adam->m; ad.v = adam->v; ad.pb = (bf16_t*)adam->p_bf16; ad.g0 = adam->g_base;
  ad.hyp = adam->hyp; ad.lr = adam->lr; ad.b1 = adam->beta1; ad.b2 = adam->beta2; ad.eps = adam->eps;
  ad.wd = adam->weight_decay; ad.bc1 = adam->bias_corr1; ad.rbc2 = 1.f / sqrtf(adam->bias_corr2);
  ad.gs = adam->grad_scale; ad.decoupled = adam->decoupled;
  if (launch_ws_grouped_adam((const GroupEnt*)groups, tile_group, block_tile, tiles, blocks, gemm_dbg(),
                             (int*)common->workspace, common->rowsum_ws, ad, (hipStream_t)stream) != 0)
    return ASRX_ERR_UNSUPPORTED;
  ASRX_CHECK_LAUNCH();
  return ASRX_OK;
}

extern "C" int asrx_gemm_grouped_xcd(const asrx_gemm_desc* common, const asrx_gemm_group_dev* groups,
                                     const uint16_t* tile_group, const uint16_t* block_tile, int32_t count,
                                     int32_t tiles, int32_t blocks, void* stream) {
  if (!common || !groups || !tile_group || !block_tile || count <= 0 || count > 65535 || tiles < 0 || blocks < 0 ||
      tiles > 65535)
    return ASRX_ERR_ARG;
  if (tiles == 0 || blocks == 0) return ASRX_OK;
  if (common->in_dtype != ASRX_BF16 || !common->a_trans || !common->b_trans) return ASRX_ERR_UNSUPPORTED;
  if (common->c_dtype != ASRX_BF16 && common->c_dtype != ASRX_F32) return ASRX_ERR_ARG;
  if (common->tile == ASRX_GROUP_TILE_WS) {
    if (common->c_dtype != ASRX_F32 || common->alpha != 1.f ||
        launch_ws_grouped((const GroupEnt*)groups, tile_group, block_tile, tiles, blocks, common->beta, gemm_dbg(),
                          common->workspace && common->workspace_elems >= 16 ? (int*)common->workspace : nullptr,
                          common->workspace && common->workspace_elems >= 16 ? common->rowsum_ws : nullptr,
                          (hipStream_t)stream) != 0)
      return ASRX_ERR_UNSUPPORTED;
  } else if (common->tile == ASRX_GROUP_TILE_P3 || common->tile == ASRX_GROUP_TILE_P4) {
    if (launch_p3_grouped(common, (const GroupEnt*)groups, tile_group, block_tile, tiles, blocks,
                          common->tile == ASRX_GROUP_TILE_P4, (hipStream_t)stream) != 0)
      return ASRX_ERR_UNSUPPORTED;
  } else if (common->tile == ASRX_GROUP_TILE_REG) {
    hipLaunchKernelGGL((gemm_bf16_grouped_dev_kernel<true, true>), dim3(blocks), dim3(256), 0, (hipStream_t)stream,
                       common->alpha, common->beta, common->c_dtype, common->relu ? 1 : 0, (const GroupEnt*)groups,
                       tile_group, (int)tiles, 0, block_tile);
  } else {
    return ASRX_ERR_ARG;
  }
  ASRX_CHECK_LAUNCH();
  return ASRX_OK;
}

extern "C" int asrx_conv2_wgrad(const void* dy2, const void* y1, int32_t B, int32_t F1, int32_t T1, float* dw,
                                float* db, float* ws, int64_t ws_elems, float* rws, int32_t splitk, void* stream) {
  if (!dy2 || !y1 || !dw || !ws || B <= 0 || F1 < 3 || T1 < 3 || splitk < 1 || splitk > 65535) return ASRX_ERR_ARG;
  if (((uintptr_t)dy2 | (uintptr_t)y1) % 16 || (db && !rws)) return ASRX_ERR_ARG;
  if (ws_elems < (int64_t)splitk * 64 * 576) return ASRX_ERR_ARG;
  const int F2 = (F1 - 3) / 2 + 1, T2 = (T1 - 3) / 2 + 1;
  const int64_t y1_bytes = (int64_t)B * F1 * T1 * 64 * 2;
  const int64_t rows = (int64_t)B * T2 * F2;
  if (y1_bytes >= 0x80000000LL || rows * 128 >= 0x80000000LL) return ASRX_ERR_UNSUPPORTED;
  GemmArgs g = {};
  g.M = 64; g.N = 576; g.K = (int)rows;
  g.a = dy2; g.lda = 64; g.b = y1; g.ldb = 576;
  g.c = dw; g.ldc = 576; g.c_dtype = ASRX_F32;
  g.batch_inner = 1; g.alpha = 1.f; g.beta = 1.f; g.rowadd_mod = 1; g.cvec = 1;
  g.splitk = splitk;
  g.k_per_split = (int)(((rows + BK - 1) / BK + splitk - 1) / splitk) * BK;
  g.ws = ws; g.rowsum = db; g.rowsum_ws = rws;
  g.dbg = gemm_dbg();
  hipStream_t st = (hipStream_t)stream;
  hipLaunchKernelGGL(gemm_bf16_tallk_kernel, dim3(splitk), dim3(512), 0, st, g,
                     TallkConv{1, F1, T1, F2, T2, y1_bytes});
  ASRX_CHECK_LAUNCH();
  return launch_reduce(g, Reduce::TallK, st);
}
```

### asr-transformer_amd/csrc/gemm_common.h

```cpp
#pragma once
#include <type_traits>

#include "common.h"

namespace asrxg {

struct GemmArgs {
  int M, N, K;
  const void* a; int64_t lda;
  const void* b; int64_t ldb;
  void* c; int64_t ldc; int c_dtype;
  int batch_inner;
  int64_t sa_o, sa_i, sb_o, sb_i, sc_o, sc_i;
  float alpha, beta;
  const float* bias;
  const float* rowadd; int64_t ld_rowadd; int rowadd_mod;
  int relu;
  uint32_t drop_thr; float drop_scale; uint64_t seed;
  const void* gate; int64_t ld_gate; int gate_dtype;
  const void* resid; int64_t ld_resid; int resid_dtype;
  int splitk; int k_per_split;
  float* ws;
  int cvec;
  float* rowsum;
// ... 450 lines not shown
  g.splitk = 1; g.k_per_split = e.k; g.cvec = 1;
  g.rowsum = e.rowsum;
  g.dbg = dbg;
  return g;
}

template <int TN, int TM>
ASRX_DEV void keep_live(f4_t (&acc)[TN][TM]) {
#pragma unroll
  for (int i = 0; i < TN; ++i)
#pragma unroll
    for (int j = 0; j < TM; ++j) asm volatile("" ::"v"(acc[i][j]));
}

template <int R, bool KSTRIDED>
ASRX_DEV s8_t p_frag(const unsigned char* img, int i0, int ks) {
  const int l = threadIdx.x & 63, g = l >> 4;
  if constexpr (!KSTRIDED) {
    const int r = i0 + (l & 15);
    const int c = (ks * 4 + g) ^ ((r >> 1) & 7);
    return *(const s8_t*)(img + r * 128 + c * 16);
  } else {
    const bf16_t* t = (const bf16_t*)img;
    const int i = l & 15, q = i >> 2, p = i & 3;
    const int k1 = ks * 32 + 8 * g + q;
    const int k2 = k1 + 4;
    const bf16_t* a1 = t + k1 * R + (((i0 >> 4) ^ ks_swz<128>(k1)) << 4) + 4 * p;
    const bf16_t* a2 = t + k2 * R + (((i0 >> 4) ^ ks_swz<128>(k2)) << 4) + 4 * p;
    s4_t v1 = __builtin_amdgcn_ds_read_tr16_b64_v4i16((__attribute__((address_space(3))) s4_t*)a1);
    s4_t v2 = __builtin_amdgcn_ds_read_tr16_b64_v4i16((__attribute__((address_space(3))) s4_t*)a2);
    return s8_t{v1[0], v1[1], v1[2], v1[3], v2[0], v2[1], v2[2], v2[3]};
  }
}

ASRX_DEV uint32_t p4_swz_bytes() {
  const int l = threadIdx.x & 63;
  return (uint32_t)(ks_swz<128>(8 * (l >> 4) + ((l & 15) >> 2)) * 32);
}
template <int R, bool KSTRIDED>
ASRX_DEV s8_t p4_frag(const unsigned char* img, int i0, int ks, uint32_t S) {
  if constexpr (!KSTRIDED) {
    return p_frag<R, false>(img, i0, ks);
  } else {
    const int l = threadIdx.x & 63, g = l >> 4, i = l & 15, q = i >> 2, p = i & 3;
    const int k1 = ks * 32 + 8 * g + q;
    const unsigned char* a1 = img + k1 * R * 2 + 8 * p + (i0 & ~127) * 2 + (((uint32_t)(i0 & 127) * 2) ^ S);
    const unsigned char* a2 = a1 + 4 * R * 2;
    s4_t v1 = __builtin_amdgcn_ds_read_tr16_b64_v4i16((__attribute__((address_space(3))) s4_t*)a1);
    s4_t v2 = __builtin_amdgcn_ds_read_tr16_b64_v4i16((__attribute__((address_space(3))) s4_t*)a2);
    return s8_t{v1[0], v1[1], v1[2], v1[3], v2[0], v2[1], v2[2], v2[3]};
  }
}

constexpr int WS_BM = 256, WS_BN = 128;
bool ws_instantiated(bool bt, int epi);
void launch_ws(const GemmArgs& g, bool bt, int epi, int ntiles, int bm, hipStream_t st);
int launch_ws_grouped(const GroupEnt* ents, const uint16_t* tile_group, const uint16_t* block_tile, int ntiles,
                      int blocks, float beta, int dbg, int* queue, float* part, hipStream_t st);
int launch_ws_grouped_adam(const GroupEnt* ents, const uint16_t* tile_group, const uint16_t* block_tile, int ntiles,
                           int blocks, int dbg, int* queue, float* part, const AdamFused& ad, hipStream_t st);

}
```

### asr-transformer_amd/csrc/norm.hip

```cpp
#include <algorithm>
#include <cstdlib>

#include "common.h"
#include "ln512.h"

namespace {
using namespace asrxln;

template <int CH>
ASRX_DEV void load_ch(const void* p, int dtype, int64_t off, float* v) {
  if (dtype == ASRX_F32) {
    const float* f = (const float*)p + off;
    if constexpr (CH == 4) { f4_t x = *(const f4_t*)f; v[0] = x[0]; v[1] = x[1]; v[2] = x[2]; v[3] = x[3]; }
    else if constexpr (CH == 2) { float2 x = *(const float2*)f; v[0] = x.x; v[1] = x.y; }
    else v[0] = f[0];
  } else {
    const bf16_t* b = (const bf16_t*)p + off;
    if constexpr (CH == 4) { uint2 u = *(const uint2*)b; v[0] = bf2f(u.x & 0xffff); v[1] = bf2f(u.x >> 16); v[2] = bf2f(u.y & 0xffff); v[3] = bf2f(u.y >> 16); }
    else if constexpr (CH == 2) { uint32_t u = *(const uint32_t*)b; v[0] = bf2f(u & 0xffff); v[1] = bf2f(u >> 16); }
    else v[0] = bf2f(b[0]);
  }
}

template <int CH>
// ... 216 lines not shown
    }
  }
#pragma unroll
  for (int i = 0; i < 8; ++i) {
    red[w][8 * l + i] = pg[i];
    red[w][D + 8 * l + i] = pb[i];
  }
  __syncthreads();
  for (int c = threadIdx.x; c < 2 * D; c += 64 * LNB_W) {
    float t = red[0][c];
#pragma unroll
    for (int i = 1; i < LNB_W; ++i) t += red[i][c];
    part[(int64_t)blockIdx.x * 2 * D + c] = t;
  }
}

int ln_pf() { return g_tune_ln_pf == 8 ? 0 : g_tune_ln_pf > 0 ? g_tune_ln_pf : 2; }
int ln_bpc() { return g_tune_ln_bpc > 0 ? g_tune_ln_bpc : 4; }

__global__ __launch_bounds__(256) void colsum_stage1(int dtype, const void* in, int64_t rows, int cols, int64_t ld,
                                                     float* part, int64_t rows_per_block) {
  const int64_t r0 = (int64_t)blockIdx.y * rows_per_block;
  const int64_t r1 = min(rows, r0 + rows_per_block);
  const int c = blockIdx.x * 64 + (threadIdx.x & 63);
  const int sub = threadIdx.x >> 6;
  __shared__ float red[4][64];
  float s = 0.f;
  if (c < cols) {
    for (int64_t r = r0 + sub; r < r1; r += 4) {
      const int64_t o = r * ld + c;
      s += dtype == ASRX_F32 ? ((const float*)in)[o] : bf2f(((const bf16_t*)in)[o]);
    }
  }
  red[sub][threadIdx.x & 63] = s;
  __syncthreads();
  if (sub == 0 && c < cols)
    part[(int64_t)blockIdx.y * cols + c] = red[0][threadIdx.x] + red[1][threadIdx.x] + red[2][threadIdx.x] + red[3][threadIdx.x];
}

__global__ __launch_bounds__(256) void colsum_stage2(const float* part, int nparts, int cols, float* out, int acc) {
  __shared__ float red[4][64];
  const int c = blockIdx.x * 64 + (threadIdx.x & 63), sub = threadIdx.x >> 6;
  float s = 0.f;
  if (c < cols)
    for (int p = sub; p < nparts; p += 4) s += part[(int64_t)p * cols + c];
  red[sub][threadIdx.x & 63] = s;
  __syncthreads();
  if (sub == 0 && c < cols) {
    const float t = red[0][threadIdx.x] + red[1][threadIdx.x] + red[2][threadIdx.x] + red[3][threadIdx.x];
    out[c] = acc ? out[c] + t : t;
  }
}

constexpr int RG_MAX = 64;
struct RowsumGroup { const float* in; float* out; int rows, cols, chunk0, acc; };
struct RowsumTable { int count; RowsumGroup gr[RG_MAX]; };

__global__ __launch_bounds__(256) void reduce_rows_grouped_kernel(RowsumTable t) {
  __shared__ float red[4][64];
  const int bid = blockIdx.x;
  int gi = 0;
  while (gi + 1 < t.count && t.gr[gi + 1].chunk0 <= bid) ++gi;
  const RowsumGroup& G = t.gr[gi];
  const int c = (bid - G.chunk0) * 64 + (threadIdx.x & 63), sub = threadIdx.x >> 6;
  float s[16];
#pragma unroll
  for (int i = 0; i < 16; ++i) s[i] = 0.f;
  if (c < G.cols) {
    const float* p = G.in + c;
    const int64_t ld = G.cols;
    int r = sub;
    for (; r + 60 < G.rows; r += 64) {
#pragma unroll
      for (int i = 0; i < 16; ++i) s[i] += p[(int64_t)(r + 4 * i) * ld];
    }
    for (int i = 0; r < G.rows; r += 4, ++i) s[i & 15] += p[(int64_t)r * ld];
  }
#pragma unroll
  for (int i = 8; i > 0; i >>= 1)
#pragma unroll
    for (int j = 0; j < i; ++j) s[j] += s[j + i];
  red[sub][threadIdx.x & 63] = s[0];
  __syncthreads();
  if (sub == 0 && c < G.cols) {
    const float v = red[0][threadIdx.x] + red[1][threadIdx.x] + red[2][threadIdx.x] + red[3][threadIdx.x];
    G.out[c] = G.acc ? G.out[c] + v : v;
  }
}

template <int CH>
bool ln_aligned(const void* p, int dtype) {
  return (uintptr_t)p % (CH * (dtype == ASRX_F32 ? 4 : 2)) == 0;
}

template <int CH, int NJ>
bool ln_fwd_launch(int x_dtype, const void* x, int y_dtype, void* y, const float* gamma, const float* beta,
                   float* mean, float* rstd, int64_t rows, int d, float eps, hipStream_t st) {
  if (d != CH * NJ * 64) return false;
  if (!ln_aligned<CH>(x, x_dtype) || !ln_aligned<CH>(y, y_dtype) || !ln_aligned<CH>(gamma, ASRX_F32) ||
      !ln_aligned<CH>(beta, ASRX_F32))
    return false;
  const int rw = (g_tune_ln_rw == 1 || g_tune_ln_rw == 4) ? g_tune_ln_rw : 2;
  const unsigned blocks = (unsigned)((rows + 4 * rw - 1) / (4 * rw));
  if (rw == 4)
    hipLaunchKernelGGL((ln_fwd_kernel<CH, NJ, 4>), dim3(blocks), dim3(256), 0, st, x_dtype, x, y_dtype, y, gamma, beta,
                       mean, rstd, rows, eps);
  else if (rw == 2)
    hipLaunchKernelGGL((ln_fwd_kernel<CH, NJ, 2>), dim3(blocks), dim3(256), 0, st, x_dtype, x, y_dtype, y, gamma, beta,
                       mean, rstd, rows, eps);
  else
    hipLaunchKernelGGL((ln_fwd_kernel<CH, NJ, 1>), dim3(blocks), dim3(256), 0, st, x_dtype, x, y_dtype, y, gamma, beta,
                       mean, rstd, rows, eps);
  return true;
}

template <int CH, int NJ>
bool ln_bwd_launch(int x_dtype, const void* x, int dy_dtype, const void* dy, const float* gamma, const float* mean,
                   const float* rstd, const float* dres, float* dx_out, void* dx_drop, int drop_dtype, float p,
                   uint64_t seed, float* part, int nblocks, int64_t rows, int d, hipStream_t st) {
  if (d != CH * NJ * 64) return false;
  if (!ln_aligned<CH>(x, x_dtype) || !ln_aligned<CH>(dy, dy_dtype) || !ln_aligned<CH>(dres, ASRX_F32) ||
      !ln_aligned<CH>(dx_out, ASRX_F32) || !ln_aligned<CH>(dx_drop, drop_dtype))
    return false;
  const uint32_t thr = drop_threshold(p);
  const float sc = (p > 0.f && p < 1.f) ? 1.f / (1.f - p) : 1.f;
  hipLaunchKernelGGL((ln_bwd_kernel<CH, NJ>), dim3(nblocks), dim3(256), 0, st, x_dtype, x, dy_dtype, dy, gamma, mean,
                     rstd, dres, dx_out, dx_drop, drop_dtype, thr, sc, seed, part, rows);
  return true;
}

constexpr int LNA_K = 32, LNA_MAXD = 64 * LNA_K;
ASRX_DEV float lna_ld(const void* p, int dtype, int64_t i) {
  return dtype == ASRX_BF16 ? bf2f(((const bf16_t*)p)[i]) : ((const float*)p)[i];
}

__global__ __launch_bounds__(256) void ln_fwd_any_kernel(int x_dtype, const void* __restrict__ x, int y_dtype,
                                                         void* __restrict__ y, const float* __restrict__ gamma,
                                                         const float* __restrict__ beta, float* __restrict__ mean,
                                                         float* __restrict__ rstd, int64_t rows, int d, float eps) {
  const int l = threadIdx.x & 63;
// ... 137 lines not shown
      (!dx_drop || drop_dtype == ASRX_BF16) &&
      ((uintptr_t)x | (uintptr_t)dy | (uintptr_t)dx_out | (uintptr_t)dres | (uintptr_t)dx_drop |
       (uintptr_t)gamma) % 16 == 0) {
    const uint32_t thr = drop_threshold(dropout_p);
    const float sc = (dropout_p > 0.f && dropout_p < 1.f) ? 1.f / (1.f - dropout_p) : 1.f;
#define ASRX_LNB(PF, DYF) hipLaunchKernelGGL((ln_bwd512_kernel<PF, DYF>), dim3(nblocks), dim3(64 * LNB_W), 0, st, \
                                             (const float*)x, dy, gamma, mean, rstd, dres, dx_out, (bf16_t*)dx_drop, \
                                             thr, sc, seed, part, rows)
    if (dy_dtype == ASRX_F32) ASRX_LNB(2, true);
    else if (pf == 1) ASRX_LNB(1, false);
    else if (pf == 4) ASRX_LNB(4, false);
    else ASRX_LNB(2, false);
#undef ASRX_LNB
    ASRX_CHECK_LAUNCH();
    return ASRX_OK;
  }
  bool ok = ln_bwd_launch<1, 1>(x_dtype, x, dy_dtype, dy, gamma, mean, rstd, dres, dx_out, dx_drop, drop_dtype, dropout_p, seed, part, nblocks, rows, d, st) ||
            ln_bwd_launch<2, 1>(x_dtype, x, dy_dtype, dy, gamma, mean, rstd, dres, dx_out, dx_drop, drop_dtype, dropout_p, seed, part, nblocks, rows, d, st) ||
            ln_bwd_launch<4, 1>(x_dtype, x, dy_dtype, dy, gamma, mean, rstd, dres, dx_out, dx_drop, drop_dtype, dropout_p, seed, part, nblocks, rows, d, st) ||
            ln_bwd_launch<4, 2>(x_dtype, x, dy_dtype, dy, gamma, mean, rstd, dres, dx_out, dx_drop, drop_dtype, dropout_p, seed, part, nblocks, rows, d, st) ||
            ln_bwd_launch<4, 3>(x_dtype, x, dy_dtype, dy, gamma, mean, rstd, dres, dx_out, dx_drop, drop_dtype, dropout_p, seed, part, nblocks, rows, d, st) ||
            ln_bwd_launch<4, 4>(x_dtype, x, dy_dtype, dy, gamma, mean, rstd, dres, dx_out, dx_drop, drop_dtype, dropout_p, seed, part, nblocks, rows, d, st);
  if (!ok) {
    if (d <= 0 || d > LNA_MAXD) return ASRX_ERR_UNSUPPORTED;
    const uint32_t thr = drop_threshold(dropout_p);
    const float sc = (dropout_p > 0.f && dropout_p < 1.f) ? 1.f / (1.f - dropout_p) : 1.f;
    hipLaunchKernelGGL(ln_bwd_any_kernel, dim3(nblocks), dim3(256), (size_t)8 * d * sizeof(float), st, x_dtype, x,
                       dy_dtype, dy, gamma, mean, rstd, dres, dx_out, dx_drop, drop_dtype, thr, sc, seed, part, rows, d);
  }
  ASRX_CHECK_LAUNCH();
  return ASRX_OK;
}

extern "C" int asrx_reduce_rows(int32_t dtype, const void* in, int64_t rows, int32_t cols, int64_t ld, float* out,
                                int32_t accumulate, float* part, int32_t nblocks, void* stream) {
  if (!in || !out || !part || cols <= 0 || rows < 0 || nblocks <= 0) return ASRX_ERR_ARG;
  hipStream_t st = (hipStream_t)stream;
  const int64_t rpb = (rows + nblocks - 1) / nblocks;
  const int nparts = rows > 0 ? (int)((rows + rpb - 1) / rpb) : 0;
  if (nparts > 0) {
    hipLaunchKernelGGL(colsum_stage1, dim3((cols + 63) / 64, nparts), dim3(256), 0, st, dtype, in, rows, cols, ld,
                       part, rpb);
    ASRX_CHECK_LAUNCH();
  }
  hipLaunchKernelGGL(colsum_stage2, dim3((cols + 63) / 64), dim3(256), 0, st, part, nparts, cols, out, accumulate);
  ASRX_CHECK_LAUNCH();
  return ASRX_OK;
}

extern "C" int asrx_reduce_rows_grouped(const asrx_rowsum_group* groups, int32_t count, void* stream) {
  if (!groups || count < 0 || count > RG_MAX) return ASRX_ERR_ARG;
  if (count == 0) return ASRX_OK;
  RowsumTable t;
  t.count = count;
  int chunks = 0;
  for (int i = 0; i < count; ++i) {
    const asrx_rowsum_group& q = groups[i];
    if (!q.in || !q.out || q.rows < 0 || q.cols <= 0 || q.rows > INT32_MAX) return ASRX_ERR_ARG;
    t.gr[i].in = q.in; t.gr[i].out = q.out; t.gr[i].rows = (int)q.rows; t.gr[i].cols = q.cols;
    t.gr[i].acc = q.accumulate; t.gr[i].chunk0 = chunks;
    chunks += (q.cols + 63) / 64;
  }
  hipLaunchKernelGGL(reduce_rows_grouped_kernel, dim3(chunks), dim3(256), 0, (hipStream_t)stream, t);
  ASRX_CHECK_LAUNCH();
  return ASRX_OK;
}
```

### include/asrx.h

```cpp
#ifndef ASRX_H
#define ASRX_H

#include <stdint.h>

#ifdef __cplusplus
extern "C" {
#endif

#define ASRX_OK 0
#define ASRX_ERR_ARG (-1)
#define ASRX_ERR_LAUNCH (-2)
#define ASRX_ERR_UNSUPPORTED (-3)

#define ASRX_BF16 0
#define ASRX_F32 1
#define ASRX_BITS 2

int asrx_version(void);

int asrx_struct_sizes(int64_t* out, int32_t n);

typedef struct asrx_gemm_desc {
  int32_t m, n, k;
  int32_t in_dtype;
// ... 67 lines not shown
  const void* k; int64_t k_rstride, k_bstride;
  const void* v; int64_t v_rstride, v_bstride;
  void* o; int64_t o_rstride, o_bstride;
  float* lse;
  float scale;
  int32_t mask_mode, causal;
  const uint8_t* kvalid; const uint8_t* qvalid; int64_t valid_bstride;
  const uint8_t* mask; int64_t mask_sb, mask_sq, mask_sk;
  float dropout_p; uint64_t seed;
  const void* dout; int64_t do_rstride, do_bstride;
  void* dq; int64_t dq_rstride, dq_bstride;
  void* dk; int64_t dk_rstride, dk_bstride;
  void* dv; int64_t dv_rstride, dv_bstride;
  float* delta;
  float* dq_acc;
  uint32_t* dropmask;
  int32_t dropmask_ready;
  void* o_lo;
} asrx_attn_desc;

int asrx_attention_fwd(const asrx_attn_desc* d, void* stream);
int64_t asrx_attn_dropmask_words(int32_t batch, int32_t heads, int32_t lq, int32_t lk);
int64_t asrx_attn_dq_acc_elems(int32_t batch, int32_t heads, int32_t lq, int32_t lk, int32_t dh);
int asrx_attn_dropgen(const asrx_attn_desc* d, void* stream);
int asrx_layernorm_fwd_attn_dropgen(const float* x, void* y, const float* gamma, const float* beta, float* mean,
                                    float* rstd, int64_t rows, int32_t d_model, float eps, const asrx_attn_desc* d,
                                    void* stream);
int asrx_attention_bwd(const asrx_attn_desc* d, void* stream);

int asrx_softmax_fwd(int32_t dtype, const void* s, void* p, void* pd, int64_t nbh, int32_t heads, int32_t lq,
                     int32_t lk, int64_t ld, float scale, int32_t mask_mode, int32_t causal,
                     const uint8_t* kvalid, const uint8_t* qvalid, int64_t valid_bstride, const uint8_t* mask,
                     int64_t mask_sb, int64_t mask_sq, int64_t mask_sk, float dropout_p, uint64_t seed,
                     void* stream);
int asrx_softmax_bwd(int32_t dtype, const void* p, const void* dpd, void* ds, int64_t nbh, int32_t lq, int32_t lk,
                     int64_t ld, float scale, float dropout_p, uint64_t seed, void* stream);

int asrx_layernorm_fwd(int32_t x_dtype, const void* x, int32_t y_dtype, void* y, const float* gamma,
                       const float* beta, float* mean, float* rstd, int64_t rows, int32_t d, float eps,
                       void* stream);
int asrx_layernorm_bwd(int32_t x_dtype, const void* x, int32_t dy_dtype, const void* dy, const float* gamma,
                       const float* mean, const float* rstd, const float* dres, float* dx_out, void* dx_drop,
                       int32_t drop_dtype, float dropout_p, uint64_t seed, float* part, int32_t nblocks,
                       int64_t rows, int32_t d, void* stream);

int asrx_reduce_rows(int32_t dtype, const void* in, int64_t rows, int32_t cols, int64_t ld, float* out,
                     int32_t accumulate, float* part, int32_t nblocks, void* stream);

typedef struct asrx_rowsum_group {
  const float* in; int64_t rows; int32_t cols; float* out; int32_t accumulate;
} asrx_rowsum_group;

int asrx_reduce_rows_grouped(const asrx_rowsum_group* groups, int32_t count, void* stream);

int asrx_conv1_fwd(const float* x, int32_t B, int32_t F, int32_t T, const float* w, const float* b, void* y1,
                   int32_t y_dtype, uint8_t* y1_mask, void* stream);
int asrx_conv2_fwd(const void* y1, const void* w2, const float* bias, void* out, int32_t B, int32_t F1, int32_t T1,
                   void* stream);
int asrx_conv2_wgrad(const void* dy2, const void* y1, int32_t B, int32_t F1, int32_t T1, float* dw, float* db,
                     float* ws, int64_t ws_elems, float* rws, int32_t splitk, void* stream);
int asrx_conv_bwd_implicit(const void* dy2, const void* w2, const uint8_t* y1_mask, const float* x, int32_t B, int32_t F,
                           int32_t T, float* part, int32_t nblocks, float* dw, float* db, void* stream);
int asrx_im2col_conv2(int32_t dtype, const void* y1, int32_t B, int32_t F1, int32_t T1, void* cols, void* stream);
int asrx_col2im_conv2(int32_t dcols_dtype, const void* dcols, int32_t y1_dtype, const void* y1, int32_t B,
                      int32_t F1, int32_t T1, float* dy1, void* stream);
int asrx_conv1_bwd_w(const float* x, const float* dy1, int32_t B, int32_t F, int32_t T, float* part,
                     int32_t nblocks, float* dw, float* db, void* stream);

int asrx_conv1_bwd_fused(int32_t dcols_dtype, const void* dcols, int32_t y1_dtype, const void* y1, const float* x,
                         int32_t B, int32_t F, int32_t T, float* part, int32_t nblocks, float* dw, float* db,
                         void* stream);

int asrx_embed_fwd(const int64_t* tok, int64_t ntok, int32_t L, const float* table, int32_t d, const float* pe,
                   float dropout_p, uint64_t seed, float* out, void* stream);
int asrx_embed_bwd(const int64_t* tok, int64_t ntok, int32_t L, const float* dout, int32_t d, int32_t vocab,
                   int32_t pad_id, float dropout_p, uint64_t seed, float* dtable, void* stream);

int asrx_cross_entropy(const float* logits, int64_t rows, int32_t V, int64_t ld, const int64_t* target,
                       int64_t ignore_index, float grad_scale, float* loss, void* dlogits, int64_t* argmax,
                       float* ws, void* stream);

#define ASRX_XENT_MAX_ROWS 715827881
int asrx_xent_workspace_elems(int64_t rows);
int asrx_cross_entropy_ls(const float* logits, int64_t rows, int32_t V, int64_t ld, const int64_t* target,
                          int64_t ignore_index, float label_smoothing, float grad_scale, float* loss, float* stats,
                          int32_t grad_dtype, void* dlogits, int64_t* argmax, float* ws, void* stream);

int asrx_cast(int32_t src_dtype, const void* src, int32_t dst_dtype, void* dst, int64_t n, void* stream);
#define ASRX_EW_RELU_GRAD 0
#define ASRX_EW_DROPOUT 1
#define ASRX_EW_ADD 2
int asrx_ewise(int32_t op, int32_t dtype_a, const void* a, int32_t dtype_b, const void* b, int32_t dtype_out,
               void* out, int64_t n, float p, uint64_t seed, void* stream);

int asrx_spectrogram(const float* audio, int64_t batch, int64_t samples, int64_t batch_stride, const float* basis,
                     int32_t n_fft, int32_t hop, int32_t nbins, int32_t power, float scale, float* ws,
                     int64_t ws_elems, float* out, void* stream);

int asrx_greedy_argmax(const float* logits, int64_t rows, int32_t V, int64_t ld, int64_t* tok, int64_t tok_stride,
                       int64_t* cur, void* stream);

int asrx_beam_step(const float* logits, int32_t B, int32_t W, int32_t V, int64_t ld, const float* score_in,
                   const uint8_t* fin_in, const int32_t* len_in, int64_t eos, float* score_out, int64_t* tok_out,
                   int64_t* cur, int32_t* parent_out, int32_t* src_row_out, uint8_t* fin_out, int32_t* len_out,
                   int32_t* n_live, void* stream);
int asrx_gather_rows(const void* src, void* dst, const int32_t* index, int32_t esize, int32_t outer, int32_t rows,
                     int64_t count, int64_t row_stride, int64_t outer_stride, void* stream);

#define ASRX_CTC_SUM 0
#define ASRX_CTC_MEAN 1

int64_t asrx_ctc_workspace_elems(int32_t B, int32_t T, int32_t max_target_len);

int asrx_ctc_loss(const float* logits, int32_t B, int32_t T, int32_t V, int64_t ld, const int64_t* targets,
                  int64_t tgt_stride, const int32_t* input_lengths, const int32_t* target_lengths,
// ... 75 lines not shown

#define ASRX_SPECAUG_MAX_MASKS 8
#define ASRX_SPECAUG_RUN 1024
int asrx_specaug(const float* src, float* dst, int32_t B, int32_t F, int32_t T, int64_t src_bstride,
                 int64_t dst_bstride, const int32_t* lengths, int32_t freq_masks, int32_t freq_width,
                 int32_t time_masks, int32_t time_width, float time_ratio, int32_t time_warp, float mask_value,
                 uint64_t seed, uint64_t step, int32_t* plan_out, void* stream);

#define ASRX_LOGMEL_MAX_MELS 256
int asrx_logmel(const float* audio, int64_t batch, int64_t samples, int64_t batch_stride, const int32_t* wave_lengths,
                const float* basis, int32_t n_fft, int32_t hop, int32_t nbins, int32_t power, float scale,
                const float* fb, const int32_t* fb_range, int32_t n_mels, int32_t log_mode, float log_mul,
                float log_eps, const float* mean, const float* istd, float pad_value, float* ws, int64_t ws_elems,
                float* out, int32_t* frame_lengths, void* stream);
int asrx_logmel_pass(const float* ws, int64_t batch, int64_t frames, const int32_t* wave_lengths, int32_t n_fft,
                     int32_t hop, int32_t nbins, int32_t power, float scale, const float* fb, const int32_t* fb_range,
                     int32_t n_mels, int32_t log_mode, float log_mul, float log_eps, const float* mean,
                     const float* istd, float pad_value, float* out, int32_t* frame_lengths, void* stream);
int asrx_stft_power(const float* ws, int64_t batch, int64_t frames, int32_t nbins, int32_t power, float scale,
                    float* out, void* stream);
int asrx_cmvn(const float* x, float* out, int32_t B, int32_t F, int32_t T, int64_t x_bstride, int64_t out_bstride,
              const int32_t* lengths, const float* mean, const float* istd, int32_t norm_var, float eps,
              float pad_value, void* stream);
int asrx_feature_stats(const float* x, int32_t B, int32_t F, int32_t T, int64_t x_bstride, const int32_t* lengths,
                       double* sum, double* sumsq, int64_t* count, void* stream);

int asrx_length_mask(const int32_t* lengths, int32_t B, int32_t T, int32_t subsample, int32_t* enc_lengths,
                     uint8_t* valid, int64_t valid_bstride, void* stream);

int asrx_sum_chunks_bf16(const void* in, int32_t world, int64_t chunk, void* out, void* stream);
int asrx_adam(float* p, const float* g, float* m, float* v, void* p_bf16, int64_t n, float lr, float beta1,
              float beta2, float eps, float weight_decay, float bias_corr1, float bias_corr2, float grad_scale,
              int32_t decoupled, const float* hyp, void* stream);
int asrx_adam_spans(float* p, const float* g, float* m, float* v, void* p_bf16, const int64_t* spans, int32_t nspans,
                    float lr, float beta1, float beta2, float eps, float weight_decay, float bias_corr1,
                    float bias_corr2, float grad_scale, int32_t decoupled, const float* hyp, void* stream);
int asrx_zero_spans(float* base, const int64_t* spans, int32_t nspans, void* stream);

int asrx_clip_grad_norm(const int64_t* spans, int32_t count, float max_norm, float* part, int32_t nparts, float* out,
                        void* stream);
int asrx_remove_after_eos(int64_t* pred, int32_t batch, int32_t pred_len, float* logits, int32_t logit_len,
                          int32_t vocab, const int64_t* eoses, int64_t eos_token, void* stream);
int asrx_step_tokens(const int64_t* text, int64_t ld_text, const int64_t* inp, int64_t ld_inp, const float* mask,
                     int64_t ld_mask, int32_t B, int32_t L, int64_t* dec_in, int64_t* tgt, uint8_t* valid,
                     void* stream);
int asrx_rowwise(int32_t op, const float* a, const float* b, float* out, int64_t rows, int32_t d, int64_t period,
                 void* stream);
int asrx_transpose_last2(const float* x, int64_t batch, int32_t R, int32_t C, float* out, void* stream);
int asrx_attn_delta(const asrx_attn_desc* d, void* stream);
int asrx_dropout_mask(uint8_t* keep, int64_t n, float p, uint64_t seed, void* stream);

int asrx_upload(void* dst, const void* src, int64_t nbytes, void* stream);
int asrx_set_seed_offset(uint64_t offset, void* stream);

#ifdef __cplusplus
}
#endif
#endif
```

Before: 5.594 million frames/s.

## Fuse launch-heavy tails: conv bwd finish, LN rowsum+Adam, step-begin, CE

Several kernel-launch reductions at once. The two-kernel conv1 gradient reduction becomes one ticket-based last-block kernel that also finishes the conv2 bias rowsum. Conv2 wgrad and the implicit conv backward are combined into one front_bwd entry. Deferred LayerNorm gamma/beta rowsums are folded into the Adam span update when running on one GPU. Input copies, seed-offset setting and Adam hyperparameter upload are merged into a single step_begin call, and cross-entropy is reworked into a single ticketed kernel. Together these cut launch count and small-kernel tail latency, at the cost of global ticket counters and more complex cross-block synchronisation.

```diff
diff --git a/asr-transformer_amd/asrx/blocks.py b/asr-transformer_amd/asrx/blocks.py
--- a/asr-transformer_amd/asrx/blocks.py
+++ b/asr-transformer_amd/asrx/blocks.py
@@ -59,6 +59,7 @@
         self.attn_impl = attn_impl
         self.wq = None
         self.lnq = None
+        self.ln_sink = None
         self.fresh = None
         self.adam = None
         self.adam_cover = []
@@ -131,7 +132,10 @@
         q, self.wq = self.wq, None
         lq, self.lnq = self.lnq, None
         self._issue_wgrads(q or [])
-        K.reduce_rows_grouped(lq or [])
+        if self.ln_sink is not None:
+            self.ln_sink += lq or []
+        else:
+            K.reduce_rows_grouped(lq or [])
 
 
 class Seeds:
@@ -499,12 +503,13 @@
         gw = G(conv2.weight)
         if C.fresh is not None:
             C.fresh.take(gw)
+        if K.conv_bwd_implicit_fits(T):
+            K.front_bwd(dy2, S["y1"], C.W(conv2.weight), S["y1m"], S["x"], gw, G(conv2.bias),
+                        G(conv1.weight).view(64, 9), G(conv1.bias))
+            return
         K.conv2_wgrad(dy2, S["y1"], gw, G(conv2.bias))
     else:
         C.wgrad(dy2, cols, G(conv2.weight), G(conv2.bias))
-    if cols is None and K.conv_bwd_implicit_fits(T):
-        K.conv_bwd_implicit(dy2, C.W(conv2.weight), S["y1m"], S["x"], G(conv1.weight).view(64, 9), G(conv1.bias))
-        return
     dcols = _empty((M2, 576), C.cd, dy2)
     K.linear_dgrad(dy2, C.W(conv2.weight), dcols)
     K.conv1_bwd_fused(dcols, S["y1"], S["x"], G(conv1.weight).view(64, 9), G(conv1.bias))
diff --git a/asr-transformer_amd/asrx/kernels.py b/asr-transformer_amd/asrx/kernels.py
--- a/asr-transformer_amd/asrx/kernels.py
+++ b/asr-transformer_amd/asrx/kernels.py
@@ -443,6 +443,19 @@
         call("asrx_reduce_rows_grouped", arr, len(chunk), stream())
 
 
+def reduce_rows_adam(items, apply, adam, spans):
+    assert len(items) <= MAX_ROWSUM_GROUPS and len(apply) == len(items)
+    arr = (RowsumGroup * max(1, len(items)))()
+    for gr, (src, out, acc) in zip(arr, items):
+        _cuda(src, out)
+        gr.in_, gr.rows, gr.cols = src.data_ptr(), src.shape[0], src.shape[1]
+        gr.out, gr.accumulate = out.data_ptr(), int(acc)
+    flags = (ctypes.c_int32 * max(1, len(items)))(*[int(bool(a)) for a in apply])
+    _cuda(spans)
+    call("asrx_reduce_rows_adam", arr, flags, len(items), ctypes.byref(adam), _p(spans),
+         0 if spans is None else spans.shape[0], stream())
+
+
 LN_BWD_BLOCKS = 512
 LN_BWD512_WAVES = 8
 
@@ -996,6 +1009,26 @@
     part = torch.empty((nblocks + 128) * 640, device=x.device, dtype=torch.float32)
     call("asrx_conv_bwd_implicit", dy2.data_ptr(), w2.data_ptr(), y1_mask.data_ptr(), x.data_ptr(), B, F, T,
          part.data_ptr(), nblocks, dw.data_ptr(), db.data_ptr(), stream())
+
+
+def front_bwd(dy2, y1, w2, y1_mask, x, dw2, db2, dw1, db1, splitk=256):
+    _cuda(dy2, y1, w2, y1_mask, x, dw2, db2, dw1, db1)
+    B, _, F, T = x.shape
+    ws = torch.empty(splitk * 64 * 576, device=dy2.device, dtype=torch.float32)
+    rws = torch.empty(splitk * 64, device=dy2.device, dtype=torch.float32)
+    nblocks = max(2, min(512, B * y1_mask.shape[1]))
+    part = torch.empty((nblocks + 128) * 640, device=x.device, dtype=torch.float32)
+    call("asrx_front_bwd", dy2.data_ptr(), y1.data_ptr(), w2.data_ptr(), y1_mask.data_ptr(), x.data_ptr(), B, F, T,
+         dw2.data_ptr(), db2.data_ptr(), ws.data_ptr(), ws.numel(), rws.data_ptr(), splitk, part.data_ptr(), nblocks,
+         dw1.data_ptr(), db1.data_ptr(), stream())
+
+
+def conv1_bwd_finish(part, nblocks, dw, db, rowsum_ws=None, rowsum_out=None):
+    _cuda(part, dw, db, rowsum_ws, rowsum_out)
+    assert part.numel() >= (nblocks + 128) * 640
+    sk, m = (rowsum_ws.shape[0], rowsum_ws.shape[1]) if rowsum_ws is not None else (0, 0)
+    call("asrx_conv1_bwd_finish", part.data_ptr(), nblocks, dw.data_ptr(), db.data_ptr(), _p(rowsum_ws), sk, m,
+         _p(rowsum_out), stream())
 
 
 def conv1_bwd_w(x, dy1, dw, db):
@@ -1341,6 +1374,27 @@
     upload(hyp, np.array([lr, 1.0 - beta1 ** step, 1.0 - beta2 ** step], dtype=np.float32))
 
 
+STEP_BEGIN_SPANS = 5
+
+
+def step_begin(copies, seed_offset, hyp, lr, beta1, beta2, step):
+    assert len(copies) <= STEP_BEGIN_SPANS
+    arr = (ctypes.c_int64 * max(1, 3 * len(copies)))()
+    for i, (dst, src) in enumerate(copies):
+        _cuda(dst, src)
+        assert step_begin_takes(dst, src)
+        arr[3 * i], arr[3 * i + 1], arr[3 * i + 2] = dst.data_ptr(), src.data_ptr(), dst.numel() * dst.element_size()
+    _cuda(hyp)
+    call("asrx_step_begin", arr, len(copies), int(seed_offset) & _U64, _p(hyp), lr, 1.0 - beta1 ** step,
+         1.0 - beta2 ** step, stream())
+
+
+def step_begin_takes(dst, src):
+    return (src.is_cuda and dst.is_cuda and src.device == dst.device and src.dtype == dst.dtype
+            and src.shape == dst.shape and src.is_contiguous() and dst.is_contiguous()
+            and (src.data_ptr() | dst.data_ptr()) % 16 == 0)
+
+
 TUNE_KEYS = {k: CONSTS["ASRX_TUNE_" + k.upper()] for k in ("softmax_u", "ln_rw", "ln_pf", "ln_bpc")}
 
 
diff --git a/asr-transformer_amd/asrx/train.py b/asr-transformer_amd/asrx/train.py
--- a/asr-transformer_amd/asrx/train.py
+++ b/asr-transformer_amd/asrx/train.py
@@ -275,6 +275,8 @@
         self.last_preds = None
         self._cover = None
         self._rspans = {}
+        self._ln_pending = None
+        self._ln_adam = None
         self._fuse_next = False
         self._frozen = sorted((self.store.offset(p), p.numel()) for p in unused_params(model) + idle_head
                               if self.store.owns(p))
@@ -353,6 +355,8 @@
             C.adam = K.adam_desc(self.store.flat, self.m, self.v, sh, self.store.grad, self.lr, self.betas[0],
                                  self.betas[1], self.eps, self.wd, max(1, self.step_count + 1),
                                  grad_scale=1.0 / self.reducer.world, decoupled=self.decoupled, hyp=self._hyp)
+            if not self.reducer.active:
+                C.ln_sink = []
         if ready is None and not capture and self.reducer.active:
             ready = self.reducer.ready
         model_backward(C, model, S, dl.to(C.cd) if dl.dtype != C.cd else dl, ready=ready, dctc_c=dctc)
@@ -361,9 +365,42 @@
             C.fresh = None
         if C.adam is not None and C.adam_cover:
             self._cover = list(C.adam_cover)
+        self._ln_pending = None
+        if C.ln_sink:
+            if self._cover is not None and self._ln_fusable(C.ln_sink):
+                self._ln_pending, self._ln_adam = C.ln_sink, C.adam
+            else:
+                K.reduce_rows_grouped(C.ln_sink)
         return loss
 
+    def _ln_fusable(self, items):
+        return len(items) <= K.MAX_ROWSUM_GROUPS and len({out.data_ptr() for _, out, _ in items}) == len(items)
+
+    def _ln_plan(self, cover, items):
+        g = self.store.grad
+        base, n = g.data_ptr(), g.numel()
+        ranges = []
+        for _, out, _ in items:
+            o = (out.data_ptr() - base) // 4
+            ok = (out.dtype == torch.float32 and out.is_contiguous() and (out.data_ptr() - base) % 4 == 0
+                  and 0 <= o and o + out.numel() <= n
+                  and not any(o < fo + fk and fo < o + out.numel() for fo, fk in self._frozen))
+            ranges.append((o, out.numel()) if ok else None)
+        key = (tuple(sorted(cover)), tuple(ranges))
+        plan = self._rspans.get(key)
+        if plan is None:
+            holes = sorted(list(key[0]) + list(self._frozen) + [r for r in ranges if r is not None])
+            pieces = residual_pieces(n, holes)
+            tab = torch.tensor(pieces, dtype=torch.int64).reshape(-1, 2).to(g.device)
+            plan = self._rspans[key] = ([r is not None for r in ranges], tab)
+        return plan
+
     def _adam(self, hyp=None, span=None):
+        if span is None and self._cover is not None and self._ln_pending:
+            items, self._ln_pending = self._ln_pending, None
+            apply, tab = self._ln_plan(self._cover, items)
+            K.reduce_rows_adam(items, apply, self._ln_adam, tab)
+            return
         if span is None and self._cover is not None:
             sh = self.store.shadow
             K.adam_spans(self.store.flat, self.store.grad, self.m, self.v, sh, self._residual_spans(self._cover),
@@ -486,14 +523,17 @@
                              "work in place, pass a tensor of your own")
         self.last_preds, self.last_stats = preds, stats
         srcs = (spectrum, text, mask, input_text) + ((lens,) if lens is not None else ())
+        copies = []
         for i, (dst, src) in enumerate(zip(ins, srcs)):
             if i == 0 and aug:
                 self._augment(src, dst, input_lengths, self.step_count + 1)
             elif dst.data_ptr() != src.data_ptr():
-                dst.copy_(src, non_blocking=True)
+                if len(copies) < K.STEP_BEGIN_SPANS and K.step_begin_takes(dst, src):
+                    copies.append((dst, src))
+                else:
+                    dst.copy_(src, non_blocking=True)
         self.step_count += 1
-        K.set_seed_offset(self.step_count)
-        K.adam_hyper(self._hyp, self.lr, self.betas[0], self.betas[1], self.step_count)
+        K.step_begin(copies, self.step_count, self._hyp, self.lr, self.betas[0], self.betas[1], self.step_count)
         seg.replay(self.reducer)
         if self.reducer.active:
             self._reduce_and_adam(self._hyp)
diff --git a/asr-transformer_amd/csrc/common.h b/asr-transformer_amd/csrc/common.h
--- a/asr-transformer_amd/csrc/common.h
+++ b/asr-transformer_amd/csrc/common.h
@@ -80,6 +80,54 @@
   if (a.pb) a.pb[off] = f2bf(p);
 }
 
+constexpr int RG_MAX = 64;
+struct RowsumGroup { const float* in; float* out; int rows, cols, chunk0, acc; };
+struct RowsumTable { int count; RowsumGroup gr[RG_MAX]; };
+
+ASRX_DEV int rowsum_group_of(const RowsumTable& t, int bid) {
+  int gi = 0;
+  while (gi + 1 < t.count && t.gr[gi + 1].chunk0 <= bid) ++gi;
+  return gi;
+}
+ASRX_DEV bool reduce_rows_chunk(const RowsumGroup& G, int chunk, float (*red)[64], int& c, float& v) {
+  c = chunk * 64 + (threadIdx.x & 63);
+  const int sub = threadIdx.x >> 6;
+  float s[16];
+#pragma unroll
+  for (int i = 0; i < 16; ++i) s[i] = 0.f;
+  if (c < G.cols) {
+    const float* p = G.in + c;
+    const int64_t ld = G.cols;
+    int r = sub;
+    for (; r + 60 < G.rows; r += 64) {
+#pragma unroll
+      for (int i = 0; i < 16; ++i) s[i] += p[(int64_t)(r + 4 * i) * ld];
+    }
+    for (int i = 0; r < G.rows; r += 4, ++i) s[i & 15] += p[(int64_t)r * ld];
+  }
+#pragma unroll
+  for (int i = 8; i > 0; i >>= 1)
+#pragma unroll
+    for (int j = 0; j < i; ++j) s[j] += s[j + i];
+  red[sub][threadIdx.x & 63] = s[0];
+  __syncthreads();
+  if (sub != 0 || c >= G.cols) return false;
+  v = red[0][threadIdx.x] + red[1][threadIdx.x] + red[2][threadIdx.x] + red[3][threadIdx.x];
+  return true;
+}
+static inline int rowsum_table(const asrx_rowsum_group* groups, int32_t count, RowsumTable& t) {
+  t.count = count;
+  int chunks = 0;
+  for (int i = 0; i < count; ++i) {
+    const asrx_rowsum_group& q = groups[i];
+    if (!q.in || !q.out || q.rows < 0 || q.cols <= 0 || q.rows > INT32_MAX) return -1;
+    t.gr[i].in = q.in; t.gr[i].out = q.out; t.gr[i].rows = (int)q.rows; t.gr[i].cols = q.cols;
+    t.gr[i].acc = q.accumulate; t.gr[i].chunk0 = chunks;
+    chunks += (q.cols + 63) / 64;
+  }
+  return chunks;
+}
+
 ASRX_DEV float exp2_raw(float x) { return __builtin_amdgcn_exp2f(x); }
 
 ASRX_DEV uint32_t rng_hash(uint64_t seed, uint32_t pidx) {
diff --git a/asr-transformer_amd/csrc/frontend.hip b/asr-transformer_amd/csrc/frontend.hip
--- a/asr-transformer_amd/csrc/frontend.hip
+++ b/asr-transformer_amd/csrc/frontend.hip
@@ -1,4 +1,5 @@
 #include <algorithm>
+#include <atomic>
 #include <cstring>
 
 #include "common.h"
@@ -582,14 +583,26 @@
   }
 }
 
+constexpr int TICKET_SLOTS = 64;
+__device__ unsigned int g_tickets[TICKET_SLOTS];
+
 constexpr int CF_G1 = 128;
 constexpr int CF_R1 = 48;
 
-__global__ __launch_bounds__(256) void conv1_bwd_reduce1(const float* __restrict__ part, int nblocks,
-                                                         float* __restrict__ part2) {
+__global__ __launch_bounds__(1024) void conv_finish_kernel(const float* __restrict__ part, int nblocks, float* part2,
+                                                           float* dw, float* db, const float* rs_ws, int rs_splitk,
+                                                           int rs_m, float* rs_out, unsigned int* ticket) {
+  __shared__ float red[16][640];
+  __shared__ int s_last;
+  const int tid = threadIdx.x;
+  if (blockIdx.x >= CF_G1) {
+    asrxg::rowsum_finish_block(rs_ws, rs_splitk, rs_m, rs_out, blockIdx.x - CF_G1, (float (*)[64])red);
+    return;
+  }
   const int per = (nblocks + CF_G1 - 1) / CF_G1;
   const int r0 = blockIdx.x * per, r1 = min(nblocks, r0 + per);
-  for (int c = threadIdx.x; c < 640; c += 256) {
+  if (tid < 640) {
+    const int c = tid;
     float s = 0.f;
     for (int base = r0; base < r1; base += CF_R1) {
       float v[CF_R1];
@@ -598,35 +611,59 @@
 #pragma unroll
       for (int j = 0; j < CF_R1; ++j) s += v[j];
     }
-    part2[blockIdx.x * 640 + c] = s;
-  }
-}
-
-__global__ __launch_bounds__(256) void conv1_bwd_reduce2(const float* __restrict__ part2, float* dw, float* db) {
-  __shared__ float red[16][16];
-  const int c = blockIdx.x * 16 + (threadIdx.x & 15), rg = threadIdx.x >> 4;
-  float v[CF_G1 / 16];
-#pragma unroll
-  for (int j = 0; j < CF_G1 / 16; ++j) v[j] = part2[(rg + 16 * j) * 640 + c];
-  float s = 0.f;
-#pragma unroll
-  for (int j = 0; j < CF_G1 / 16; ++j) s += v[j];
-  red[rg][threadIdx.x & 15] = s;
+    __hip_atomic_store(part2 + blockIdx.x * 640 + c, s, __ATOMIC_RELAXED, __HIP_MEMORY_SCOPE_AGENT);
+  }
+  asm volatile("s_waitcnt vmcnt(0)" ::: "memory");
   __syncthreads();
-  if (rg == 0) {
-    s = 0.f;
-#pragma unroll
-    for (int i = 0; i < 16; ++i) s += red[i][threadIdx.x];
+  if (tid == 0) {
+    const bool last = __hip_atomic_fetch_add(ticket, 1u, __ATOMIC_RELAXED, __HIP_MEMORY_SCOPE_AGENT) == CF_G1 - 1;
+    if (last) {
+      __builtin_amdgcn_fence(__ATOMIC_ACQUIRE, "agent");
+      asm volatile("s_waitcnt vmcnt(0)" ::: "memory");
+      __hip_atomic_store(ticket, 0u, __ATOMIC_RELAXED, __HIP_MEMORY_SCOPE_AGENT);
+    }
+    s_last = last;
+  }
+  __syncthreads();
+  if (!s_last) return;
+  const int rg = tid >> 6, l = tid & 63;
+  float v[10][CF_G1 / 16];
+#pragma unroll
+  for (int cc = 0; cc < 10; ++cc)
+#pragma unroll
+    for (int j = 0; j < CF_G1 / 16; ++j)
+      v[cc][j] = __hip_atomic_load(part2 + (rg + 16 * j) * 640 + cc * 64 + l, __ATOMIC_RELAXED,
+                                   __HIP_MEMORY_SCOPE_AGENT);
+#pragma unroll
+  for (int cc = 0; cc < 10; ++cc) {
+    float s = 0.f;
+#pragma unroll
+    for (int j = 0; j < CF_G1 / 16; ++j) s += v[cc][j];
+    red[rg][cc * 64 + l] = s;
+  }
+  __syncthreads();
+  if (tid < 640) {
+    const int c = tid;
+    float s = 0.f;
+#pragma unroll
+    for (int i = 0; i < 16; ++i) s += red[i][c];
     const int ch = c / 10, k = c % 10;
     if (k < 9) dw[ch * 9 + k] += s;
     else db[ch] += s;
   }
 }
 
-void conv1_bwd_finish(const float* part, int nblocks, float* dw, float* db, hipStream_t st) {
+unsigned int* next_ticket();
+
+int conv1_bwd_finish(const float* part, int nblocks, float* dw, float* db, hipStream_t st,
+                     const float* rs_ws = nullptr, int rs_splitk = 0, int rs_m = 0, float* rs_out = nullptr) {
   float* part2 = const_cast<float*>(part) + (int64_t)nblocks * 640;
-  hipLaunchKernelGGL(conv1_bwd_reduce1, dim3(CF_G1), dim3(256), 0, st, part, nblocks, part2);
-  hipLaunchKernelGGL(conv1_bwd_reduce2, dim3(40), dim3(256), 0, st, part2, dw, db);
+  unsigned int* ticket = next_ticket();
+  if (!ticket) return ASRX_ERR_LAUNCH;
+  const int nrs = rs_ws ? (rs_m + 63) / 64 : 0;
+  hipLaunchKernelGGL(conv_finish_kernel, dim3(CF_G1 + nrs), dim3(1024), 0, st, part, nblocks, part2, dw, db, rs_ws,
+                     rs_splitk, rs_m, rs_out, ticket);
+  return ASRX_OK;
 }
 
 __global__ __launch_bounds__(256) void embed_fwd_kernel(const int64_t* __restrict__ tok, int64_t ntok, int L,
@@ -845,78 +882,109 @@
   }
 }
 
-__global__ __launch_bounds__(256) void ce_count_kernel(const int64_t* tgt, int64_t rows, int64_t ignore, float* ws) {
+constexpr int CE_WAVES = 16;
+template <int NJ>
+__global__ __launch_bounds__(64 * CE_WAVES) void ce_kernel(const float* __restrict__ logits, int64_t rows, int V, int64_t ld,
+                                                 const int64_t* __restrict__ tgt, int64_t ignore, float gscale,
+                                                 bf16_t* __restrict__ dlog, int64_t* argmax, float* ws, float* loss,
+                                                 unsigned int* ticket) {
   __shared__ float red[256];
+  __shared__ int s_last;
+  const int l = threadIdx.x & 63;
+  const int64_t r = (int64_t)blockIdx.x * CE_WAVES + (threadIdx.x >> 6);
+  const float* x = logits + (r < rows ? r : 0) * ld;
+  float v[NJ];
+  if (r < rows) {
+#pragma unroll
+    for (int j = 0; j < NJ; ++j) {
+      const int c = j * 64 + l;
+      v[j] = c < V ? x[c] : -INFINITY;
+    }
+  }
+  constexpr int NT = 64 * CE_WAVES;
   float c = 0.f;
-  for (int64_t r = threadIdx.x; r < rows; r += 256) c += tgt[r] != ignore ? 1.f : 0.f;
-  red[threadIdx.x] = c;
+  for (int64_t q0 = threadIdx.x; q0 < rows; q0 += NT * 4) {
+    int64_t t4[4];
+#pragma unroll
+    for (int j = 0; j < 4; ++j) t4[j] = tgt[min(q0 + NT * j, rows - 1)];
+#pragma unroll
+    for (int j = 0; j < 4; ++j) c += q0 + NT * j < rows && t4[j] != ignore ? 1.f : 0.f;
+  }
+  c = wave_sum(c);
+  if (l == 0) red[threadIdx.x >> 6] = c;
   __syncthreads();
-  for (int s = 128; s > 0; s >>= 1) {
-    if (threadIdx.x < s) red[threadIdx.x] += red[threadIdx.x + s];
-    __syncthreads();
-  }
-  if (threadIdx.x == 0) ws[rows] = red[0];
-}
-
-template <int NJ>
-__global__ __launch_bounds__(256) void ce_rows_kernel(const float* __restrict__ logits, int64_t rows, int V,
-                                                      int64_t ld, const int64_t* __restrict__ tgt, int64_t ignore,
-                                                      float gscale, bf16_t* __restrict__ dlog, int64_t* argmax,
-                                                      float* ws) {
-  const int l = threadIdx.x & 63;
-  const int64_t r = (int64_t)blockIdx.x * 4 + (threadIdx.x >> 6);
-  if (r >= rows) return;
-  const float* x = logits + r * ld;
-  float v[NJ];
-  float mx = -INFINITY;
-  int am = 0;
-#pragma unroll
-  for (int j = 0; j < NJ; ++j) {
-    const int c = j * 64 + l;
-    v[j] = c < V ? x[c] : -INFINITY;
-    if (v[j] > mx) { mx = v[j]; am = c; }
-  }
-#pragma unroll
-  for (int o = 32; o > 0; o >>= 1) {
-    const float om = __shfl_xor(mx, o, 64);
-    const int oa = __shfl_xor(am, o, 64);
-    if (om > mx || (om == mx && oa < am)) { mx = om; am = oa; }
-  }
+  float cnt = 0.f;
+#pragma unroll
+  for (int w = 0; w < CE_WAVES; ++w) cnt += red[w];
+  if (r < rows) {
+    float mx = -INFINITY;
+    int am = 0;
+#pragma unroll
+    for (int j = 0; j < NJ; ++j) {
+      const int c = j * 64 + l;
+      if (v[j] > mx) { mx = v[j]; am = c; }
+    }
+#pragma unroll
+    for (int o = 32; o > 0; o >>= 1) {
+      const float om = __shfl_xor(mx, o, 64);
+      const int oa = __shfl_xor(am, o, 64);
+      if (om > mx || (om == mx && oa < am)) { mx = om; am = oa; }
+    }
+    float s = 0.f;
+#pragma unroll
+    for (int j = 0; j < NJ; ++j) s += __expf(v[j] - mx);
+    s = wave_sum(s);
+    const float lse = mx + __logf(s);
+    const int64_t t = tgt[r];
+    const bool valid = t != ignore;
+    const float k = valid && cnt > 0.f ? gscale / cnt : 0.f;
+#pragma unroll
+    for (int j = 0; j < NJ; ++j) {
+      const int c = j * 64 + l;
+      if (c < ld) {
+        float gr = 0.f;
+        if (c < V) gr = (__expf(v[j] - lse) - (c == t ? 1.f : 0.f)) * k;
+        if (dlog) dlog[r * ld + c] = f2bf(gr);
+      }
+    }
+    if (l == 0) {
+      __hip_atomic_store(ws + r, valid ? lse - x[t] : 0.f, __ATOMIC_RELAXED, __HIP_MEMORY_SCOPE_AGENT);
+      if (argmax) argmax[r] = am;
+    }
+  }
+  asm volatile("s_waitcnt vmcnt(0)" ::: "memory");
+  __syncthreads();
+  if (threadIdx.x == 0) {
+    const bool last = __hip_atomic_fetch_add(ticket, 1u, __ATOMIC_RELAXED, __HIP_MEMORY_SCOPE_AGENT) == gridDim.x - 1;
+    if (last) {
+      __builtin_amdgcn_fence(__ATOMIC_ACQUIRE, "agent");
+      asm volatile("s_waitcnt vmcnt(0)" ::: "memory");
+      __hip_atomic_store(ticket, 0u, __ATOMIC_RELAXED, __HIP_MEMORY_SCOPE_AGENT);
+    }
+    s_last = last;
+  }
+  __syncthreads();
+  if (!s_last) return;
+  const bool fin = threadIdx.x < 256;
   float s = 0.f;
-#pragma unroll
-  for (int j = 0; j < NJ; ++j) s += __expf(v[j] - mx);
-  s = wave_sum(s);
-  const float lse = mx + __logf(s);
-  const int64_t t = tgt[r];
-  const bool valid = t != ignore;
-  const float cnt = ws[rows];
-  const float k = valid && cnt > 0.f ? gscale / cnt : 0.f;
-#pragma unroll
-  for (int j = 0; j < NJ; ++j) {
-    const int c = j * 64 + l;
-    if (c < ld) {
-      float gr = 0.f;
-      if (c < V) gr = (__expf(v[j] - lse) - (c == t ? 1.f : 0.f)) * k;
-      if (dlog) dlog[r * ld + c] = f2bf(gr);
-    }
-  }
-  if (l == 0) {
-    ws[r] = valid ? lse - x[t] : 0.f;
-    if (argmax) argmax[r] = am;
-  }
-}
-
-__global__ __launch_bounds__(256) void ce_final_kernel(const float* ws, int64_t rows, float* loss) {
-  __shared__ float red[256];
-  float s = 0.f;
-  for (int64_t r = threadIdx.x; r < rows; r += 256) s += ws[r];
-  red[threadIdx.x] = s;
+  for (int64_t q0 = threadIdx.x; fin && q0 < rows; q0 += 256 * 16) {
+    float w16[16];
+#pragma unroll
+    for (int j = 0; j < 16; ++j)
+      w16[j] = __hip_atomic_load(ws + min(q0 + 256 * j, rows - 1), __ATOMIC_RELAXED, __HIP_MEMORY_SCOPE_AGENT);
+#pragma unroll
+    for (int j = 0; j < 16; ++j) s = q0 + 256 * j < rows ? s + w16[j] : s;
+  }
+  if (fin) red[threadIdx.x] = s;
   __syncthreads();
   for (int k = 128; k > 0; k >>= 1) {
     if (threadIdx.x < k) red[threadIdx.x] += red[threadIdx.x + k];
     __syncthreads();
   }
-  if (threadIdx.x == 0) loss[0] = ws[rows] > 0.f ? red[0] / ws[rows] : 0.f;
+  if (threadIdx.x == 0) {
+    ws[rows] = cnt;
+    loss[0] = cnt > 0.f ? red[0] / cnt : 0.f;
+  }
 }
 
 __global__ __launch_bounds__(256) void cast_kernel(int sd, const void* __restrict__ src, int dd, void* __restrict__ dst,
@@ -994,6 +1062,29 @@
   }
 }
 
+ASRX_DEV void adam_span_block(float* __restrict__ p, const float* __restrict__ g, float* __restrict__ m,
+                              float* __restrict__ v, bf16_t* __restrict__ pb, const int64_t* __restrict__ spans,
+                              int blk, float lr, float b1, float b2, float eps, float wd, float bc1, float rbc2,
+                              float gs, int decoupled) {
+  const int64_t a0 = spans[2 * blk], e0 = spans[2 * blk + 1];
+  const int64_t a = (a0 + 3) / 4, e = e0 / 4;
+  for (int64_t i = a + threadIdx.x; i < e; i += 256) {
+    f4_t pp = ((const f4_t*)p)[i], mm = ((const f4_t*)m)[i], vv = ((const f4_t*)v)[i];
+    adam_f4(pp, ((const f4_t*)g)[i], mm, vv, lr, b1, b2, eps, wd, bc1, rbc2, gs, decoupled);
+    adam_store(p, m, v, pb, i, pp, mm, vv);
+  }
+  const int64_t hb = min(4 * a, e0), tb = max(4 * e, hb);
+  const int64_t j = threadIdx.x < 3 ? a0 + threadIdx.x : tb + (threadIdx.x - 3);
+  if ((threadIdx.x < 3 && j < hb) || (threadIdx.x >= 3 && threadIdx.x < 6 && j >= tb && j < e0)) {
+    float pe = p[j], me = m[j], ve = v[j];
+    adam_elem(g[j], pe, me, ve, lr, b1, b2, eps, wd, bc1, rbc2, gs, decoupled);
+    p[j] = pe;
+    m[j] = me;
+    v[j] = ve;
+    if (pb) pb[j] = f2bf(pe);
+  }
+}
+
 __global__ __launch_bounds__(256) void adam_spans_kernel(float* __restrict__ p, const float* __restrict__ g,
                                                          float* __restrict__ m, float* __restrict__ v,
                                                          bf16_t* __restrict__ pb, const int64_t* __restrict__ spans,
@@ -1005,22 +1096,27 @@
     bc1 = hyp[1];
     rbc2 = 1.f / sqrtf(hyp[2]);
   }
-  const int64_t a0 = spans[2 * blockIdx.x], e0 = spans[2 * blockIdx.x + 1];
-  const int64_t a = (a0 + 3) / 4, e = e0 / 4;
-  for (int64_t i = a + threadIdx.x; i < e; i += 256) {
-    f4_t pp = ((const f4_t*)p)[i], mm = ((const f4_t*)m)[i], vv = ((const f4_t*)v)[i];
-    adam_f4(pp, ((const f4_t*)g)[i], mm, vv, lr, b1, b2, eps, wd, bc1, rbc2, gs, decoupled);
-    adam_store(p, m, v, pb, i, pp, mm, vv);
-  }
-  const int64_t hb = min(4 * a, e0), tb = max(4 * e, hb);
-  const int64_t j = threadIdx.x < 3 ? a0 + threadIdx.x : tb + (threadIdx.x - 3);
-  if ((threadIdx.x < 3 && j < hb) || (threadIdx.x >= 3 && threadIdx.x < 6 && j >= tb && j < e0)) {
-    float pe = p[j], me = m[j], ve = v[j];
-    adam_elem(g[j], pe, me, ve, lr, b1, b2, eps, wd, bc1, rbc2, gs, decoupled);
-    p[j] = pe;
-    m[j] = me;
-    v[j] = ve;
-    if (pb) pb[j] = f2bf(pe);
+  adam_span_block(p, g, m, v, pb, spans, blockIdx.x, lr, b1, b2, eps, wd, bc1, rbc2, gs, decoupled);
+}
+
+__global__ __launch_bounds__(256) void reduce_rows_adam_kernel(RowsumTable t, uint64_t apply, int nred, AdamFused ad,
+                                                               const int64_t* __restrict__ spans) {
+  __shared__ float red[4][64];
+  float lr, bc1, rbc2;
+  adam_hyp(ad, lr, bc1, rbc2);
+  if ((int)blockIdx.x >= nred) {
+    adam_span_block(ad.p, ad.g0, ad.m, ad.v, ad.pb, spans, blockIdx.x - nred, lr, ad.b1, ad.b2, ad.eps, ad.wd, bc1,
+                    rbc2, ad.gs, ad.decoupled);
+    return;
+  }
+  const int gi = rowsum_group_of(t, blockIdx.x);
+  const RowsumGroup& G = t.gr[gi];
+  int c;
+  float v;
+  if (reduce_rows_chunk(G, blockIdx.x - G.chunk0, red, c, v)) {
+    const float gv = G.acc ? G.out[c] + v : v;
+    G.out[c] = gv;
+    if ((apply >> gi) & 1u) adam_apply1(ad, G.out + c, gv, lr, bc1, rbc2);
   }
 }
 
@@ -1054,11 +1150,20 @@
   return (unsigned)b;
 }
 
+unsigned int* next_ticket() {
+  static unsigned int* const base = [] {
+    void* p = nullptr;
+    return hipGetSymbolAddress(&p, HIP_SYMBOL(g_tickets)) == hipSuccess ? (unsigned int*)p : nullptr;
+  }();
+  static std::atomic<unsigned> slot{0};
+  return base ? base + slot.fetch_add(1, std::memory_order_relaxed) % TICKET_SLOTS : nullptr;
+}
+
 }
 
 ASRX_SEED_OFFSET_SETTER(frontend)
 
-extern "C" int asrx_version(void) { return 14; }
+extern "C" int asrx_version(void) { return 15; }
 
 extern "C" int asrx_struct_sizes(int64_t* out, int32_t n) {
   if (!out || n < 0) return ASRX_ERR_ARG;
@@ -1176,17 +1281,13 @@
   if (!logits || !target || !loss || !ws || V <= 0 || ld < V || rows < 0) return ASRX_ERR_ARG;
   if (ld > 1024) return ASRX_ERR_UNSUPPORTED;
   hipStream_t st = (hipStream_t)stream;
-  hipLaunchKernelGGL(ce_count_kernel, dim3(1), dim3(256), 0, st, target, rows, ignore_index, ws);
-  ASRX_CHECK_LAUNCH();
-  if (rows > 0) {
-    const dim3 grid((unsigned)((rows + 3) / 4));
-    const int nj = (int)((ld + 63) / 64);
-    if (nj <= 4) hipLaunchKernelGGL((ce_rows_kernel<4>), grid, dim3(256), 0, st, logits, rows, V, ld, target, ignore_index, grad_scale, (bf16_t*)dlogits, argmax, ws);
-    else if (nj <= 8) hipLaunchKernelGGL((ce_rows_kernel<8>), grid, dim3(256), 0, st, logits, rows, V, ld, target, ignore_index, grad_scale, (bf16_t*)dlogits, argmax, ws);
-    else hipLaunchKernelGGL((ce_rows_kernel<16>), grid, dim3(256), 0, st, logits, rows, V, ld, target, ignore_index, grad_scale, (bf16_t*)dlogits, argmax, ws);
-    ASRX_CHECK_LAUNCH();
-  }
-  hipLaunchKernelGGL(ce_final_kernel, dim3(1), dim3(256), 0, st, ws, rows, loss);
+  const dim3 grid((unsigned)std::max<int64_t>(1, (rows + CE_WAVES - 1) / CE_WAVES));
+  unsigned int* ticket = next_ticket();
+  if (!ticket) return ASRX_ERR_LAUNCH;
+  const int nj = (int)((ld + 63) / 64);
+  if (nj <= 4) hipLaunchKernelGGL((ce_kernel<4>), grid, dim3(64 * CE_WAVES), 0, st, logits, rows, V, ld, target, ignore_index, grad_scale, (bf16_t*)dlogits, argmax, ws, loss, ticket);
+  else if (nj <= 8) hipLaunchKernelGGL((ce_kernel<8>), grid, dim3(64 * CE_WAVES), 0, st, logits, rows, V, ld, target, ignore_index, grad_scale, (bf16_t*)dlogits, argmax, ws, loss, ticket);
+  else hipLaunchKernelGGL((ce_kernel<16>), grid, dim3(64 * CE_WAVES), 0, st, logits, rows, V, ld, target, ignore_index, grad_scale, (bf16_t*)dlogits, argmax, ws, loss, ticket);
   ASRX_CHECK_LAUNCH();
   return ASRX_OK;
 }
@@ -1323,6 +1424,32 @@
   return ASRX_OK;
 }
 
+extern "C" int asrx_reduce_rows_adam(const asrx_rowsum_group* groups, const int32_t* apply, int32_t count,
+                                     const asrx_adam_desc* adam, const int64_t* spans, int32_t nspans, void* stream) {
+  if (count < 0 || count > RG_MAX || (count > 0 && (!groups || !apply)) || !adam || nspans < 0 || (nspans > 0 && !spans))
+    return ASRX_ERR_ARG;
+  if (!adam->p || !adam->m || !adam->v || !adam->g_base || (((uintptr_t)adam->p | (uintptr_t)adam->m |
+      (uintptr_t)adam->v | (uintptr_t)adam->g_base) % 16) || (adam->p_bf16 && (uintptr_t)adam->p_bf16 % 8))
+    return ASRX_ERR_ARG;
+  if (!adam->hyp && (adam->bias_corr1 <= 0.f || adam->bias_corr2 <= 0.f)) return ASRX_ERR_ARG;
+  RowsumTable t;
+  const int nred = rowsum_table(groups, count, t);
+  if (nred < 0) return ASRX_ERR_ARG;
+  if (nred + nspans == 0) return ASRX_OK;
+  uint64_t mask = 0;
+  for (int i = 0; i < count; ++i)
+    if (apply[i]) mask |= 1ull << i;
+  AdamFused ad;
+  ad.p = adam->p; ad.m = adam->m; ad.v = adam->v; ad.pb = (bf16_t*)adam->p_bf16; ad.g0 = adam->g_base;
+  ad.hyp = adam->hyp; ad.lr = adam->lr; ad.b1 = adam->beta1; ad.b2 = adam->beta2; ad.eps = adam->eps;
+  ad.wd = adam->weight_decay; ad.bc1 = adam->bias_corr1; ad.rbc2 = 1.f / sqrtf(adam->bias_corr2);
+  ad.gs = adam->grad_scale; ad.decoupled = adam->decoupled;
+  hipLaunchKernelGGL(reduce_rows_adam_kernel, dim3(nred + nspans), dim3(256), 0, (hipStream_t)stream, t, mask, nred,
+                     ad, spans);
+  ASRX_CHECK_LAUNCH();
+  return ASRX_OK;
+}
+
 extern "C" int asrx_dropout_mask(uint8_t* keep, int64_t n, float p, uint64_t seed, void* stream) {
   if (!keep || n < 0) return ASRX_ERR_ARG;
   if (n == 0) return ASRX_OK;
@@ -1332,9 +1459,22 @@
   return ASRX_OK;
 }
 
+static int conv_bwd_implicit_impl(const void* dy2, const void* w2, const uint8_t* y1m, const float* x, int32_t B,
+                                  int32_t F, int32_t T, float* part, int32_t nblocks, float* dw, float* db,
+                                  const float* rs_ws, int rs_splitk, int rs_m, float* rs_out, bool launch,
+                                  hipStream_t st);
+
 extern "C" int asrx_conv_bwd_implicit(const void* dy2, const void* w2, const uint8_t* y1m, const float* x, int32_t B,
                                       int32_t F, int32_t T, float* part, int32_t nblocks, float* dw, float* db,
                                       void* stream) {
+  return conv_bwd_implicit_impl(dy2, w2, y1m, x, B, F, T, part, nblocks, dw, db, nullptr, 0, 0, nullptr, true,
+                                (hipStream_t)stream);
+}
+
+static int conv_bwd_implicit_impl(const void* dy2, const void* w2, const uint8_t* y1m, const float* x, int32_t B,
+                                  int32_t F, int32_t T, float* part, int32_t nblocks, float* dw, float* db,
+                                  const float* rs_ws, int rs_splitk, int rs_m, float* rs_out, bool launch,
+                                  hipStream_t st) {
   if (!dy2 || !w2 || !y1m || !x || !part || !dw || !db || B <= 0 || F < 7 || T < 7 || nblocks < 2)
     return ASRX_ERR_ARG;
   if (((uintptr_t)dy2 | (uintptr_t)y1m) % 16) return ASRX_ERR_ARG;
@@ -1344,11 +1484,37 @@
   const int g_even = std::max(1, std::min(nblocks - 1, (2 * nblocks + 2) / 3));
   const size_t shm = (size_t)6 * 64 * 64 * 2 + ((T1 * 8 + 15) & ~15) + sizeof(float) * 3 * T;
   if (shm > 80 * 1024 || shm < 8 * 640 * 4) return ASRX_ERR_UNSUPPORTED;
-  hipStream_t st = (hipStream_t)stream;
+  if (!launch) return ASRX_OK;
   hipLaunchKernelGGL(conv_bwd_implicit_kernel, dim3(nblocks), dim3(512), shm, st, (const bf16_t*)dy2,
                      (const bf16_t*)w2, y1m, x, B, F, T, F1, T1, F2, T2, g_even, part);
   ASRX_CHECK_LAUNCH();
-  conv1_bwd_finish(part, nblocks, dw, db, st);
+  const int rc = conv1_bwd_finish(part, nblocks, dw, db, st, rs_ws, rs_splitk, rs_m, rs_out);
+  if (rc != ASRX_OK) return rc;
+  ASRX_CHECK_LAUNCH();
+  return ASRX_OK;
+}
+
+extern "C" int asrx_front_bwd(const void* dy2, const void* y1, const void* w2, const uint8_t* y1m, const float* x,
+                              int32_t B, int32_t F, int32_t T, float* dw2, float* db2, float* ws, int64_t ws_elems,
+                              float* rws, int32_t splitk, float* part, int32_t nblocks, float* dw1, float* db1,
+                              void* stream) {
+  if (!db2 || !rws) return ASRX_ERR_ARG;
+  hipStream_t st = (hipStream_t)stream;
+  int rc = conv_bwd_implicit_impl(dy2, w2, y1m, x, B, F, T, part, nblocks, dw1, db1, rws, splitk, 64, db2, false, st);
+  if (rc != ASRX_OK) return rc;
+  const int F1 = (F - 3) / 2 + 1, T1 = (T - 3) / 2 + 1;
+  rc = asrxg::conv2_wgrad_launch(dy2, y1, B, F1, T1, dw2, db2, ws, ws_elems, rws, splitk, false, st);
+  if (rc != ASRX_OK) return rc;
+  return conv_bwd_implicit_impl(dy2, w2, y1m, x, B, F, T, part, nblocks, dw1, db1, rws, splitk, 64, db2, true, st);
+}
+
+extern "C" int asrx_conv1_bwd_finish(const float* part, int32_t nblocks, float* dw, float* db, const float* rs_ws,
+                                     int32_t rs_splitk, int32_t rs_m, float* rs_out, void* stream) {
+  if (!part || !dw || !db || nblocks <= 0) return ASRX_ERR_ARG;
+  if (rs_ws && (!rs_out || rs_splitk < 1 || rs_m < 1)) return ASRX_ERR_ARG;
+  const int rc = conv1_bwd_finish(part, nblocks, dw, db, (hipStream_t)stream, rs_ws, rs_splitk, rs_m, rs_out);
+  if (rc != ASRX_OK) return rc;
+  ASRX_CHECK_LAUNCH();
   return ASRX_OK;
 }
 
@@ -1407,15 +1573,76 @@
 }
 }
 
-extern "C" int asrx_set_seed_offset(uint64_t offset, void* stream) {
+static const SeedAddrs* seed_addrs() {
   static const SeedAddrs addrs = [] {
     return SeedAddrs{{asrx_seed_offset_addr_gemm(), asrx_seed_offset_addr_attention(), asrx_seed_offset_addr_norm(),
                       asrx_seed_offset_addr_softmax(), asrx_seed_offset_addr_frontend(),
                       asrx_seed_offset_addr_gemm_ws()}};
   }();
   for (uint64_t* q : addrs.p)
-    if (!q) return ASRX_ERR_LAUNCH;
-  hipLaunchKernelGGL(seed_offset_set_all_kernel, dim3(1), dim3(64), 0, (hipStream_t)stream, offset, addrs);
+    if (!q) return nullptr;
+  return &addrs;
+}
+
+extern "C" int asrx_set_seed_offset(uint64_t offset, void* stream) {
+  const SeedAddrs* addrs = seed_addrs();
+  if (!addrs) return ASRX_ERR_LAUNCH;
+  hipLaunchKernelGGL(seed_offset_set_all_kernel, dim3(1), dim3(64), 0, (hipStream_t)stream, offset, *addrs);
+  ASRX_CHECK_LAUNCH();
+  return ASRX_OK;
+}
+
+namespace {
+constexpr int STEP_SPANS = 5;
+constexpr int STEP_SPAN_BLOCKS = 1024;
+struct StepSpans {
+  char* dst[STEP_SPANS];
+  const char* src[STEP_SPANS];
+  int64_t bytes[STEP_SPANS];
+  int blk0[STEP_SPANS + 1];
+};
+__global__ __launch_bounds__(256) void step_begin_kernel(StepSpans sp, int nspans, uint64_t seed_offset, SeedAddrs a,
+                                                         float* hyp, float h0, float h1, float h2) {
+  if (blockIdx.x == 0) {
+    if (threadIdx.x < 6) *a.p[threadIdx.x] = seed_offset;
+    if (hyp && threadIdx.x >= 64 && threadIdx.x < 67)
+      hyp[threadIdx.x - 64] = threadIdx.x == 64 ? h0 : (threadIdx.x == 65 ? h1 : h2);
+  }
+  int i = 0;
+  while (i + 1 < nspans && sp.blk0[i + 1] <= (int)blockIdx.x) ++i;
+  if (i >= nspans || (int)blockIdx.x >= sp.blk0[i + 1]) return;
+  const int b = blockIdx.x - sp.blk0[i], nb = sp.blk0[i + 1] - sp.blk0[i];
+  const int64_t n16 = sp.bytes[i] / 16;
+  const f4_t* s = (const f4_t*)sp.src[i];
+  f4_t* d = (f4_t*)sp.dst[i];
+  for (int64_t q = (int64_t)b * 256 + threadIdx.x; q < n16; q += (int64_t)nb * 256) d[q] = s[q];
+  if (b == 0) {
+    const int64_t t = n16 * 16 + threadIdx.x;
+    if (threadIdx.x < 16 && t < sp.bytes[i]) sp.dst[i][t] = sp.src[i][t];
+  }
+}
+}
+
+extern "C" int asrx_step_begin(const int64_t* spans, int32_t nspans, uint64_t seed_offset, float* hyp, float lr,
+                               float bias_corr1, float bias_corr2, void* stream) {
+  if (nspans < 0 || nspans > STEP_SPANS || (nspans > 0 && !spans)) return ASRX_ERR_ARG;
+  const SeedAddrs* addrs = seed_addrs();
+  if (!addrs) return ASRX_ERR_LAUNCH;
+  StepSpans sp = {};
+  int blocks = 0, n = 0;
+  for (int i = 0; i < nspans; ++i) {
+    const int64_t dst = spans[3 * i], src = spans[3 * i + 1], bytes = spans[3 * i + 2];
+    if (bytes < 0 || (bytes > 0 && (!dst || !src || (dst | src) % 16))) return ASRX_ERR_ARG;
+    if (bytes == 0) continue;
+    sp.dst[n] = (char*)(uintptr_t)dst;
+    sp.src[n] = (const char*)(uintptr_t)src;
+    sp.bytes[n] = bytes;
+    sp.blk0[n] = blocks;
+    blocks += (int)std::min<int64_t>(STEP_SPAN_BLOCKS, (bytes + 4095) / 4096);
+    sp.blk0[++n] = blocks;
+  }
+  hipLaunchKernelGGL(step_begin_kernel, dim3(std::max(1, blocks)), dim3(256), 0, (hipStream_t)stream, sp, n,
+                     seed_offset, *addrs, hyp, lr, bias_corr1, bias_corr2);
   ASRX_CHECK_LAUNCH();
   return ASRX_OK;
 }
diff --git a/asr-transformer_amd/csrc/gemm.hip b/asr-transformer_amd/csrc/gemm.hip
--- a/asr-transformer_amd/csrc/gemm.hip
+++ b/asr-transformer_amd/csrc/gemm.hip
@@ -1247,23 +1247,7 @@
 
 __global__ __launch_bounds__(256) void rowsum_finish_kernel(const float* ws, int splitk, int M, float* out) {
   __shared__ float red[4][64];
-  const int m = blockIdx.x * 64 + (threadIdx.x & 63), sg = threadIdx.x >> 6;
-  float s = 0.f;
-  if (m < M) {
-    for (int sp0 = sg; sp0 < splitk; sp0 += 64) {
-      float v[16];
-#pragma unroll
-      for (int j = 0; j < 16; ++j) {
-        const int sp = sp0 + 4 * j;
-        v[j] = sp < splitk ? ws[(int64_t)sp * M + m] : 0.f;
-      }
-#pragma unroll
-      for (int j = 0; j < 16; ++j) s += v[j];
-    }
-  }
-  red[sg][threadIdx.x & 63] = s;
-  __syncthreads();
-  if (sg == 0 && m < M) out[m] += red[0][threadIdx.x] + red[1][threadIdx.x] + red[2][threadIdx.x] + red[3][threadIdx.x];
+  rowsum_finish_block(ws, splitk, M, out, blockIdx.x, red);
 }
 
 template <class F>
@@ -1526,14 +1510,14 @@
   return ASRX_OK;
 }
 
-int launch_reduce(const GemmArgs& g, Reduce reduce, hipStream_t st) {
+int launch_reduce(const GemmArgs& g, Reduce reduce, hipStream_t st, bool finish_rowsum = true) {
   const int64_t quads = (int64_t)g.M * ((g.N + 3) / 4);
   if (reduce == Reduce::TallK)
     hipLaunchKernelGGL(tallk_reduce_kernel, dim3((unsigned)((quads + 31) / 32)), dim3(256), 0, st, g);
   else
     hipLaunchKernelGGL(splitk_reduce_kernel, dim3((int)std::min<int64_t>((quads + 255) / 256, 4096)), dim3(256), 0, st, g);
   ASRX_CHECK_LAUNCH();
-  if (g.rowsum) {
+  if (g.rowsum && finish_rowsum) {
     hipLaunchKernelGGL(rowsum_finish_kernel, dim3((g.M + 63) / 64), dim3(256), 0, st, g.rowsum_ws, g.splitk, g.M, g.rowsum);
     ASRX_CHECK_LAUNCH();
   }
@@ -1645,8 +1629,8 @@
   return ASRX_OK;
 }
 
-extern "C" int asrx_conv2_wgrad(const void* dy2, const void* y1, int32_t B, int32_t F1, int32_t T1, float* dw,
-                                float* db, float* ws, int64_t ws_elems, float* rws, int32_t splitk, void* stream) {
+int asrxg::conv2_wgrad_launch(const void* dy2, const void* y1, int B, int F1, int T1, float* dw, float* db, float* ws,
+                              int64_t ws_elems, float* rws, int splitk, bool finish_rowsum, hipStream_t st) {
   if (!dy2 || !y1 || !dw || !ws || B <= 0 || F1 < 3 || T1 < 3 || splitk < 1 || splitk > 65535) return ASRX_ERR_ARG;
   if (((uintptr_t)dy2 | (uintptr_t)y1) % 16 || (db && !rws)) return ASRX_ERR_ARG;
   if (ws_elems < (int64_t)splitk * 64 * 576) return ASRX_ERR_ARG;
@@ -1663,9 +1647,13 @@
   g.k_per_split = (int)(((rows + BK - 1) / BK + splitk - 1) / splitk) * BK;
   g.ws = ws; g.rowsum = db; g.rowsum_ws = rws;
   g.dbg = gemm_dbg();
-  hipStream_t st = (hipStream_t)stream;
   hipLaunchKernelGGL(gemm_bf16_tallk_kernel, dim3(splitk), dim3(512), 0, st, g,
                      TallkConv{1, F1, T1, F2, T2, y1_bytes});
   ASRX_CHECK_LAUNCH();
-  return launch_reduce(g, Reduce::TallK, st);
-}
+  return launch_reduce(g, Reduce::TallK, st, finish_rowsum);
+}
+
+extern "C" int asrx_conv2_wgrad(const void* dy2, const void* y1, int32_t B, int32_t F1, int32_t T1, float* dw,
+                                float* db, float* ws, int64_t ws_elems, float* rws, int32_t splitk, void* stream) {
+  return conv2_wgrad_launch(dy2, y1, B, F1, T1, dw, db, ws, ws_elems, rws, splitk, true, (hipStream_t)stream);
+}
diff --git a/asr-transformer_amd/csrc/gemm_common.h b/asr-transformer_amd/csrc/gemm_common.h
--- a/asr-transformer_amd/csrc/gemm_common.h
+++ b/asr-transformer_amd/csrc/gemm_common.h
@@ -526,6 +526,29 @@
   }
 }
 
+ASRX_DEV void rowsum_finish_block(const float* ws, int splitk, int M, float* out, int blk, float (*red)[64]) {
+  const int t = threadIdx.x, m = blk * 64 + (t & 63), sg = t >> 6;
+  float s = 0.f;
+  if (sg < 4 && m < M) {
+    for (int sp0 = sg; sp0 < splitk; sp0 += 64) {
+      float v[16];
+#pragma unroll
+      for (int j = 0; j < 16; ++j) {
+        const int sp = sp0 + 4 * j;
+        v[j] = sp < splitk ? ws[(int64_t)sp * M + m] : 0.f;
+      }
+#pragma unroll
+      for (int j = 0; j < 16; ++j) s += v[j];
+    }
+  }
+  if (sg < 4) red[sg][t & 63] = s;
+  __syncthreads();
+  if (sg == 0 && m < M) out[m] += red[0][t] + red[1][t] + red[2][t] + red[3][t];
+}
+
+int conv2_wgrad_launch(const void* dy2, const void* y1, int B, int F1, int T1, float* dw, float* db, float* ws,
+                       int64_t ws_elems, float* rws, int splitk, bool finish_rowsum, hipStream_t st);
+
 constexpr int WS_BM = 256, WS_BN = 128;
 bool ws_instantiated(bool bt, int epi);
 void launch_ws(const GemmArgs& g, bool bt, int epi, int ntiles, int bm, hipStream_t st);
diff --git a/asr-transformer_amd/csrc/norm.hip b/asr-transformer_amd/csrc/norm.hip
--- a/asr-transformer_amd/csrc/norm.hip
+++ b/asr-transformer_amd/csrc/norm.hip
@@ -292,40 +292,12 @@
   }
 }
 
-constexpr int RG_MAX = 64;
-struct RowsumGroup { const float* in; float* out; int rows, cols, chunk0, acc; };
-struct RowsumTable { int count; RowsumGroup gr[RG_MAX]; };
-
 __global__ __launch_bounds__(256) void reduce_rows_grouped_kernel(RowsumTable t) {
   __shared__ float red[4][64];
-  const int bid = blockIdx.x;
-  int gi = 0;
-  while (gi + 1 < t.count && t.gr[gi + 1].chunk0 <= bid) ++gi;
-  const RowsumGroup& G = t.gr[gi];
-  const int c = (bid - G.chunk0) * 64 + (threadIdx.x & 63), sub = threadIdx.x >> 6;
-  float s[16];
-#pragma unroll
-  for (int i = 0; i < 16; ++i) s[i] = 0.f;
-  if (c < G.cols) {
-    const float* p = G.in + c;
-    const int64_t ld = G.cols;
-    int r = sub;
-    for (; r + 60 < G.rows; r += 64) {
-#pragma unroll
-      for (int i = 0; i < 16; ++i) s[i] += p[(int64_t)(r + 4 * i) * ld];
-    }
-    for (int i = 0; r < G.rows; r += 4, ++i) s[i & 15] += p[(int64_t)r * ld];
-  }
-#pragma unroll
-  for (int i = 8; i > 0; i >>= 1)
-#pragma unroll
-    for (int j = 0; j < i; ++j) s[j] += s[j + i];
-  red[sub][threadIdx.x & 63] = s[0];
-  __syncthreads();
-  if (sub == 0 && c < G.cols) {
-    const float v = red[0][threadIdx.x] + red[1][threadIdx.x] + red[2][threadIdx.x] + red[3][threadIdx.x];
-    G.out[c] = G.acc ? G.out[c] + v : v;
-  }
+  const RowsumGroup& G = t.gr[rowsum_group_of(t, blockIdx.x)];
+  int c;
+  float v;
+  if (reduce_rows_chunk(G, blockIdx.x - G.chunk0, red, c, v)) G.out[c] = G.acc ? G.out[c] + v : v;
 }
 
 template <int CH>
@@ -569,15 +541,8 @@
   if (!groups || count < 0 || count > RG_MAX) return ASRX_ERR_ARG;
   if (count == 0) return ASRX_OK;
   RowsumTable t;
-  t.count = count;
-  int chunks = 0;
-  for (int i = 0; i < count; ++i) {
-    const asrx_rowsum_group& q = groups[i];
-    if (!q.in || !q.out || q.rows < 0 || q.cols <= 0 || q.rows > INT32_MAX) return ASRX_ERR_ARG;
-    t.gr[i].in = q.in; t.gr[i].out = q.out; t.gr[i].rows = (int)q.rows; t.gr[i].cols = q.cols;
-    t.gr[i].acc = q.accumulate; t.gr[i].chunk0 = chunks;
-    chunks += (q.cols + 63) / 64;
-  }
+  const int chunks = rowsum_table(groups, count, t);
+  if (chunks < 0) return ASRX_ERR_ARG;
   hipLaunchKernelGGL(reduce_rows_grouped_kernel, dim3(chunks), dim3(256), 0, (hipStream_t)stream, t);
   ASRX_CHECK_LAUNCH();
   return ASRX_OK;
diff --git a/include/asrx.h b/include/asrx.h
--- a/include/asrx.h
+++ b/include/asrx.h
@@ -143,6 +143,8 @@
 } asrx_rowsum_group;
 
 int asrx_reduce_rows_grouped(const asrx_rowsum_group* groups, int32_t count, void* stream);
+int asrx_reduce_rows_adam(const asrx_rowsum_group* groups, const int32_t* apply, int32_t count,
+                          const asrx_adam_desc* adam, const int64_t* spans, int32_t nspans, void* stream);
 
 int asrx_conv1_fwd(const float* x, int32_t B, int32_t F, int32_t T, const float* w, const float* b, void* y1,
                    int32_t y_dtype, uint8_t* y1_mask, void* stream);
@@ -152,6 +154,11 @@
                      float* ws, int64_t ws_elems, float* rws, int32_t splitk, void* stream);
 int asrx_conv_bwd_implicit(const void* dy2, const void* w2, const uint8_t* y1_mask, const float* x, int32_t B, int32_t F,
                            int32_t T, float* part, int32_t nblocks, float* dw, float* db, void* stream);
+int asrx_conv1_bwd_finish(const float* part, int32_t nblocks, float* dw, float* db, const float* rs_ws,
+                          int32_t rs_splitk, int32_t rs_m, float* rs_out, void* stream);
+int asrx_front_bwd(const void* dy2, const void* y1, const void* w2, const uint8_t* y1_mask, const float* x, int32_t B,
+                   int32_t F, int32_t T, float* dw2, float* db2, float* ws, int64_t ws_elems, float* rws,
+                   int32_t splitk, float* part, int32_t nblocks, float* dw1, float* db1, void* stream);
 int asrx_im2col_conv2(int32_t dtype, const void* y1, int32_t B, int32_t F1, int32_t T1, void* cols, void* stream);
 int asrx_col2im_conv2(int32_t dcols_dtype, const void* dcols, int32_t y1_dtype, const void* y1, int32_t B,
                       int32_t F1, int32_t T1, float* dy1, void* stream);
@@ -333,6 +340,8 @@
 
 int asrx_upload(void* dst, const void* src, int64_t nbytes, void* stream);
 int asrx_set_seed_offset(uint64_t offset, void* stream);
+int asrx_step_begin(const int64_t* spans, int32_t nspans, uint64_t seed_offset, float* hyp, float lr, float bias_corr1,
+                    float bias_corr2, void* stream);
 
 #ifdef __cplusplus
 }
```

Measured after the change: 5.611 million frames/s, median of 4. Within noise of the previous version (+0.3%).
